# samuel-vitorino/sopro

Hardware: AMD Instinct MI355X
Metric: audio_seconds_per_second (higher is better)
Workload: dtype f32; 1 GPU; Sopro-135M synthesize, 32 utterances x 200 frames per GPU (BASELINE configs[1]), S=64 text tokens, 32 distinct 150-frame reference voice(s) per batch prepared outside the timed region, top_p=0.9 T=1.05 anti_loop (reference defaults), synthetic weights with EOS suppressed; batch_per_gpu=32, frames=200, voices_per_batch=32, parallelism=replicas x1 (utterance sharding, no collective), lanes_per_gpu=4

## Files before the change

include/sopro_hip.h:

```cpp
#ifndef SOPRO_HIP_H
#define SOPRO_HIP_H

#include <stdint.h>

#ifdef __cplusplus
extern "C" {
#endif

#define SOPRO_ABI_VERSION 42

const char* sopro_last_error(void);
int sopro_abi_version(void);
int sopro_build_flags(void);
int sopro_set_lds_floor(int bytes);
int sopro_set_host_wait(int blocking);
int sopro_device_info(int device, int* out4);

int sopro_capture_begin(void* stream);
int sopro_capture_end(void* stream, void** graph_exec_out);
int sopro_graph_launch(void* graph_exec, void* stream);
int sopro_graph_launch_n(void* graph_exec, void* stream, int32_t n);
int sopro_graph_destroy(void* graph_exec);
int sopro_stream_create_cu_range(int first_cu, int n_cus, void** stream_out);
int sopro_stream_create_cu_mask(const uint32_t* mask, int32_t words, void** stream_out);
int sopro_stream_destroy(void* stream);
int sopro_host_alloc(int64_t bytes, void** out);
int sopro_host_free(void* p);
int sopro_copy_to_host_async(void* dst_host, const void* src_dev, int64_t bytes, void* stream);

enum { SOPRO_PRO_NONE = 0, SOPRO_PRO_ELU = 1, SOPRO_PRO_ADDVEC = 2 };
enum { SOPRO_EPI_NONE = 0, SOPRO_EPI_GELU = 1, SOPRO_EPI_GLU = 2, SOPRO_EPI_RES = 3, SOPRO_EPI_TANH = 4,
       SOPRO_EPI_GLU_DW = 5 ,
       SOPRO_EPI_ROPE = 6  };

typedef struct sopro_gemm_args {
  const float* A; int64_t lda; int64_t a_seg_stride;
  const float* W; int64_t ldw;
  const float* bias;
  float* C; int64_t ldc; int64_t c_seg_stride;
  const float* R; int64_t ldr; int64_t r_seg_stride;
  const float* scale;
  const float* pro_vec;
  long long* dbg;
  int32_t M, N, K, rows_per_seg;
  int32_t prologue, epilogue;
} sopro_gemm_args;
int sopro_gemm_f32(const sopro_gemm_args* args, void* stream);
int sopro_gemm_set_tile_override(int cfg);

typedef struct sopro_gemm_split_ext {
  int32_t a_format;
  int32_t c_mode;
  float* C2; int64_t ldc2; int64_t c2_seg_stride;
  int32_t rms_norm; float rms_eps;
  int32_t ksplit;
  int32_t n_tickets;
  float* ws; int64_t ws_bytes;
  int32_t* tickets;
  int32_t group_m;
  float acc_scale;
  int32_t* range_events;
  const float* rope_cos; const float* rope_sin;
  int32_t rope_cols, rope_dh, rope_pos0, rope_rows_per_seg;
  const float* ln_stats;
  float* ln_stats_out;
} sopro_gemm_split_ext;
int sopro_gemm_bf16x3(const sopro_gemm_args* a, const void* packed_w, const sopro_gemm_split_ext* ext, void* stream);
int64_t sopro_packed_w_rows_bytes(int32_t N, int32_t K);
int sopro_pack_w_rows_bf16(const float* W, int64_t ldw, int32_t N, int32_t K, void* packed, void* stream);
int sopro_gemm_8p_takes(const sopro_gemm_args* a, const sopro_gemm_split_ext* ext);
int sopro_gemm_bf16x3_8p(const sopro_gemm_args* a, const void* w_rows, const sopro_gemm_split_ext* ext, void* stream);
int sopro_gemm_bf16x6(const sopro_gemm_args* a, const void* packed_w, const sopro_gemm_split_ext* ext, void* stream);
int sopro_gemm_bf16x1(const sopro_gemm_args* a, const void* packed_w, const sopro_gemm_split_ext* ext, void* stream);
int sopro_pack_w_bf16(const float* W, int64_t ldw, int32_t N, int32_t K, int32_t pieces, void* packed, void* stream);
int sopro_pack_w_f16x2(const float* W, int64_t ldw, int32_t N, int32_t K, float wscale, void* packed, void* stream);
float sopro_f16x3_a_scale(void);
int sopro_gemm_f16x3(const sopro_gemm_args* a, const void* packed_w, const sopro_gemm_split_ext* ext, void* stream);
int64_t sopro_packed_w_bytes(int32_t N, int32_t K, int32_t pieces);
int sopro_gemm_bf16_set_tile_override(int cfg);
int sopro_gemm_set_group_m(int g);

typedef struct sopro_skinny_args {
  const float* X; int64_t ldx;
  const float* W; int64_t ldw;
  const float* bias;
  float* Y; int64_t ldy;
  const float* R; int64_t ldr;
  const float* scale;
  float* ring;
  const float* dw_w;
  const float* dw_b;
  const int32_t* step;
  const float* Xp; int64_t xp_stride;
  int64_t y_part_stride;
  long long* dbg;
  float eps;
  int32_t B, N, K, epilogue;
  int32_t ring_len, ring_bcap, dil, ksize;
  int32_t np, ksplit, rms_norm;
  int32_t w_layout;
  const float* aux_W; const float* aux_bias; const float* aux_R; float* aux_Y;
  int64_t aux_ldy, aux_ldr, aux_y_part_stride;
  int32_t aux_tiles, aux_flags;
  int32_t ring_format;
  int32_t mt, nt;
} sopro_skinny_args;
int sopro_skinny_f32(const sopro_skinny_args* args, void* stream);
int sopro_pack_skinny_w(const float* W, int64_t ldw, int32_t N, int32_t K, int32_t glu, float* out, void* stream);
int64_t sopro_skinny_packed_floats(int32_t N, int32_t K, int32_t glu);
int sopro_pack_skinny_w_bf16(const float* W, int64_t ldw, int32_t N, int32_t K, int32_t glu, void* out, void* stream);

int sopro_fill2d_u32(void* p, int64_t pitch, int32_t rows, int32_t width, uint32_t value, void* stream);
int sopro_copy2d_u32(void* dst, int64_t dpitch, const void* src, int64_t spitch, int32_t rows, int32_t width, void* stream);
int sopro_nar_seed_i32(int32_t* tokens, int32_t Q, const int32_t* cb0, int64_t cb0_bstride, int32_t B, int32_t T, int32_t vmax, void* stream);
int sopro_cvt_f32_bf16(const float* src, void* dst, int64_t n, void* stream);
int sopro_cvt_bf16_f32(const void* src, float* dst, int64_t n, void* stream);
enum { SOPRO_NORM_RMS = 0, SOPRO_NORM_LN = 1 };
int sopro_norm_f32(const float* x, int64_t ldx, int64_t x_seg_stride , float* out, int64_t ldo, const float* w, const float* b,
                   const float* mul, const float* add, int32_t rows, int32_t rows_per_seg, int32_t C,
                   float eps, int32_t kind, void* stream);
int sopro_row_stats_f32(const float* x, int64_t ldx, int64_t x_seg_stride , int32_t rows, int32_t rows_per_seg, int32_t C,
                        float* stats, void* stream);
int sopro_rms_match_f32(const float* a, const float* x, float* out, int32_t rows, int32_t C, void* stream);
int sopro_tanh_affine_f32(const float* in, float* out, float c0, float c1, int64_t n, void* stream);
int sopro_add_pos_f32(const float* rowvec, const float* table, float* out, int32_t B, int32_t T, int32_t C,
                      int32_t pos0, void* stream);
int sopro_masked_mean_f32(const float* x, const int32_t* lens, float* out, int32_t B, int32_t T, int32_t C,
                          void* stream);

int sopro_stats_pool_f32(const float* h, const float* logit, const int32_t* lens, float* out, int32_t B, int32_t T,
                         int32_t C, void* stream);
int sopro_l2norm_f32(const float* x, float* out, int32_t rows, int32_t C, float eps, void* stream);

int sopro_dwconv_f32(const float* x, const float* w, const float* bias, const float* res, float* out,
                     const int32_t* lens, int32_t B, int32_t T, int32_t C, int32_t ksize, int32_t dil,
                     int32_t left, int32_t mode, void* stream);

int sopro_codebook_sum_f32(const int32_t* tok, int32_t ldt, const int32_t* col, const int32_t* off, const float* wq,
                           int32_t nq, const float* table, int64_t table_rows, const float* base, float alpha,
                           float beta, float* out, int64_t ldo, int64_t o_seg_stride, int32_t rows,
                           int32_t rows_per_seg, int32_t D, void* stream);
int sopro_text_embed_f32(const int32_t* ids, const int32_t* lens, const float* table, int64_t table_rows,
                         const float* pe, float* out, int32_t B, int32_t T, int32_t C, void* stream);
int sopro_argmax_rows_f32(const float* x, int64_t ldx, int32_t* out, int64_t ldo, int32_t inner, int32_t rows, int32_t N,
                          void* stream);
int sopro_argmax_partials_i32(const float* partials, int64_t ldp, int32_t* out, int64_t ldo, int32_t heads, int32_t per_head, int32_t V,
                              int32_t rows, void* stream);

int sopro_fir1_f32(const float* x, int64_t x_seg_stride, int32_t n_in, const float* w, const float* bias, float* out,
                   int64_t ldo, int64_t o_seg_stride, int32_t B, int32_t n_out, int32_t C, int32_t K, int32_t stride,
                   int32_t left, void* stream);
int sopro_rvq_assign_f32(const float* scores, int64_t lds, int32_t V, const float* table, float* res, int64_t ldr,
                         int32_t D, int32_t* codes, int64_t ldc, int32_t rows, void* stream);

typedef struct sopro_attn_args {
  const float* Q; int64_t ldq; int64_t q_bstride;
  const float* K; int64_t ldk; int64_t k_bstride;
  const float* V; int64_t ldv; int64_t v_bstride;
  float* O; int64_t ldo; int64_t o_bstride;
  const int32_t* klens;
// ... 106 lines not shown
} sopro_ar_block;
typedef struct sopro_ar_frame {
  sopro_ar_block blk[SOPRO_AR_MAX_LAYERS];
  const void* head_w; const float* head_b;
  float* x0;
  float* xa; float* xb;
  float* part;
  float* u;
  float* xp;
  float* qa;
  float* qpart;
  float* logits;
  const int32_t* klens;
  int32_t n_layers, B, D, S_cap, V1, H, ksize, w_layout;
  int32_t tile_glu, tile_ff1, tile_ff2, tile_head;
  float eps;
  int32_t k_unfold;
  int32_t store_format;
  sopro_ar_state st;
} sopro_ar_frame;
int sopro_ar_issue_frame(const sopro_ar_frame* frame, void* stream);

typedef struct sopro_engine sopro_engine;
typedef struct sopro_engine_cfg {
  int32_t d_model, codebook_size, num_codebooks, nar_head_dim, bos_row;
  int32_t n_layers_ar, ar_kernel, ar_dilations[16], ar_xattn[16] ;
  float ar_gate[16];
  int32_t n_layers_nar, nar_kernel, nar_dilations[16];
  int32_t n_stages, stage_first_cb[8], stage_n_cb[8];
  float nar_mix[8][2];
  float nar_prev_cb_weights[64];
  int32_t mimi_hidden, mimi_codebook_dim, mimi_heads, mimi_head_dim, mimi_layers, mimi_window, mimi_inter;
  int32_t mimi_n_ratios, mimi_ratios[8], mimi_num_filters, mimi_kernel, mimi_res_kernel, mimi_last_kernel, mimi_compress;
  int32_t mimi_n_semantic, mimi_rope_positions;
  float mimi_norm_eps, mimi_final_bias;
  int32_t precision;
  int32_t n_layers_text, ref_enc_layers, ref_xattn_layers, ref_xattn_heads, sv_student_dim, enc_kernel ;
} sopro_engine_cfg;
int sopro_engine_create(const sopro_engine_cfg* cfg, sopro_engine** out);
int sopro_engine_set_tensor(sopro_engine* e, const char* name, const void* dev_ptr, const int64_t* shape, int32_t ndim);
int sopro_engine_upload_tensor(sopro_engine* e, const char* name, const float* host_ptr, const int64_t* shape, int32_t ndim, void* stream);
int sopro_engine_finalize(sopro_engine* e, void* stream);
int sopro_ar_fold_text(const float* txt, const float* nkv_weight, const float* kv_w, const float* q_wT, const float* o_w, float* nkv, float* kvd,
                       float* kp, float* vp, int32_t B, int32_t S, int32_t S_cap, int32_t D, int32_t H, float eps, void* stream);
int sopro_ar_fold_text_uk(const float* txt, const float* nkv_weight, const float* kv_w, const float* o_w, float* nkv, float* kvd, float* kq, float* vp,
                          int32_t B, int32_t S, int32_t S_cap, int32_t D, int32_t H, float eps, void* stream);
int sopro_engine_destroy(sopro_engine* e);
int sopro_engine_set_ar_tiles(sopro_engine* e, int32_t glu, int32_t ff1, int32_t ff2, int32_t head);

typedef struct sopro_checkpoint sopro_checkpoint;
int sopro_checkpoint_open(const char* sopro_path, const char* mimi_path, sopro_checkpoint** out);
int sopro_checkpoint_close(sopro_checkpoint* ck);
int32_t sopro_checkpoint_count(const sopro_checkpoint* ck);
int sopro_checkpoint_tensor(const sopro_checkpoint* ck, int32_t i, const char** name, const float** data, int64_t* shape4, int32_t* ndim);
int sopro_checkpoint_engine_cfg(const sopro_checkpoint* ck, int32_t precision, sopro_engine_cfg* cfg);
int sopro_engine_from_checkpoint(const sopro_checkpoint* ck, int32_t precision, void* stream, sopro_engine** out);

int64_t sopro_cond_workspace_bytes(const sopro_engine* e, int32_t B, int32_t S, int32_t Tar);
int sopro_cond_prepare(sopro_engine* e, void* workspace, const int32_t* ids, const int32_t* lens, int32_t ragged, const float* film_mul, const float* film_add,
                       const float* const* ref_k, const float* const* ref_v, int64_t kv_bstride, const int32_t* kv_index, const int32_t* ref_klens,
                       int32_t B, int32_t S, int32_t Tar, int32_t Tr, float* txt_seq, float* txt_pool, float* cond_ar, void* stream);
int sopro_film_coeffs(sopro_engine* e, const float* sv, float style, int32_t n, float* scratch, float* mul, float* add, void* stream);
int64_t sopro_ref_workspace_bytes(const sopro_engine* e, int32_t T);
int sopro_ref_prepare(sopro_engine* e, void* workspace, const int32_t* tokens, int32_t T, float* sv, float* ref_seq, float* const* kv, void* stream);

int64_t sopro_ar_workspace_bytes(const sopro_engine* e, int32_t B, int32_t S, int32_t Tar);
int sopro_ar_begin(sopro_engine* e, void* workspace, int32_t B, const float* cond_ar, const float* txt_seq, const int32_t* text_lens,
                   int32_t S, int32_t Tar, const float params[8], uint64_t seed, uint32_t nonce, void* stream);
int sopro_ar_run_graph(sopro_engine* e, int32_t n_steps, void* stream);
int sopro_ar_tokens(sopro_engine* e, int32_t* hist, int32_t* first_eos, int32_t* n_stopped, void* stream);

int64_t sopro_nar_workspace_bytes(const sopro_engine* e, int32_t B, int32_t T);
int sopro_nar_refine(sopro_engine* e, void* workspace, const float* cond, int64_t cond_bstride, const int32_t* rvq1, const int32_t* lens,
                     int32_t B, int32_t T, int32_t* tokens, void* stream);
typedef struct sopro_nar_io {
  const float* cond; int64_t cond_bstride;
  const int32_t* cb0; int64_t cb0_bstride;
  const int32_t* lens;
  int32_t* tokens;
  int32_t* range_out;
  int32_t safe;
} sopro_nar_io;
int sopro_nar_refine_io(sopro_engine* e, void* workspace, const sopro_nar_io* io, int32_t B, int32_t T, void* stream);

int64_t sopro_mimi_encode_workspace_bytes(const sopro_engine* e, int32_t B, int32_t N);
int sopro_mimi_encode(sopro_engine* e, void* workspace, const float* wav, int32_t B, int32_t N, int32_t* codes, void* stream);

int64_t sopro_mimi_workspace_bytes(const sopro_engine* e, int32_t B, int32_t T);
int sopro_mimi_decode(sopro_engine* e, void* workspace, const int32_t* tokens, int32_t B, int32_t T, float* wav, void* stream);
int32_t sopro_mimi_chunk_rows(int32_t B, int32_t T);
int sopro_mimi_decode_parts(sopro_engine* e, void* workspace, const int32_t* tokens, int32_t B, int32_t T, float* wav, int32_t parts, void* stream);

typedef struct sopro_mimi_stream_state {
  float* kv;
  int32_t cap_rows;
  int32_t kv_len, pos, evict, half;
} sopro_mimi_stream_state;
int64_t sopro_mimi_stream_kv_bytes(const sopro_engine* e, int32_t cap_rows);
int sopro_mimi_stream_init(const sopro_engine* e, sopro_mimi_stream_state* st, void* kv, int32_t cap_rows);
int sopro_mimi_stream_trim(sopro_mimi_stream_state* st, int32_t n);
int sopro_mimi_decode_stream(sopro_engine* e, void* workspace, sopro_mimi_stream_state* st, const int32_t* tokens, int32_t T, float* wav,
                             void* stream);

#define SOPRO_MIMI_STREAM_BATCH_MAX_ROWS 64
typedef struct sopro_mimi_stream_batch {
  float* kv;
  int32_t rows_cap, rows;
  int32_t cap_rows, kv_len, pos, evict, half;
} sopro_mimi_stream_batch;
int64_t sopro_mimi_stream_batch_kv_bytes(const sopro_engine* e, int32_t rows, int32_t cap_rows);
int sopro_mimi_stream_batch_init(const sopro_engine* e, sopro_mimi_stream_batch* st, void* kv, int32_t rows, int32_t cap_rows);
int sopro_mimi_stream_batch_trim(sopro_mimi_stream_batch* st, int32_t n);
int sopro_mimi_stream_batch_keep(const sopro_engine* e, sopro_mimi_stream_batch* st, const int32_t* keep, int32_t n_keep, void* stream);
int sopro_mimi_decode_stream_batch(sopro_engine* e, void* workspace, sopro_mimi_stream_batch* st, const int32_t* tokens, int32_t T, float* wav,
                                   void* stream);

int64_t sopro_join_workspace_bytes(int32_t n_seg, int64_t max_len, int32_t hop);
int sopro_join_edges_f32(const float* wav, int64_t row_stride, const int32_t* lens, int32_t n_seg, int64_t max_len, int32_t hop, float rel,
                         int32_t keep, int32_t trim, void* workspace, int32_t* edges, void* stream);
int sopro_join_layout_i64(const int32_t* edges, const int32_t* gaps, int32_t n_seg, int64_t* offs, void* stream);
int sopro_join_mix_f32(const float* wav, int64_t row_stride, const int32_t* edges, const int64_t* offs, const float* tab, int32_t fade_len,
                       int32_t n_seg, float* out, int64_t out_cap, void* stream);

#define SOPRO_TSM_W 960
#define SOPRO_TSM_HS 480
#define SOPRO_TSM_R 240
#define SOPRO_TSM_TAIL 2048
int64_t sopro_tsm_out_len(int64_t in_len, int64_t step);
int64_t sopro_tsm_blocks(int64_t out_len);
int64_t sopro_tsm_chunk_out_cap(int64_t in_len);
int64_t sopro_tsm_state_bytes(int32_t rows);
int sopro_tsm_rows_f32(const float* in, int64_t in_stride, const int32_t* in_lens, int64_t in_cap, const int64_t* steps, int32_t rows, void* state,
                       int32_t flush, const float* tab, float* out, int64_t out_stride, int64_t out_cap, int32_t* out_lens, int32_t* deltas,
                       int32_t blocks_cap, void* stream);

#define SOPRO_PITCH_NT 64
#define SOPRO_PITCH_P 256
#define SOPRO_PITCH_TAIL 128
#define SOPRO_PITCH_TILE 2048
int64_t sopro_pitch_out_len(int64_t in_len, int64_t inc);
int64_t sopro_pitch_chunk_out_cap(int64_t in_len);
int64_t sopro_pitch_state_bytes(int32_t rows);
int sopro_pitch_rows_f32(const float* in, int64_t in_stride, const int32_t* in_lens, int64_t in_cap, const int64_t* incs, const int32_t* bank_idx,
                         const float* banks, int32_t n_banks, int32_t rows, void* state, int32_t flush, float* out, int64_t out_stride,
                         int64_t out_cap, int32_t* out_lens, void* stream);

#define SOPRO_WM_HS 480
#define SOPRO_WM_P 8192
#define SOPRO_WM_SHIFT 32
#define SOPRO_WM_TAIL 1536
#define SOPRO_WM_TILE 3840
int64_t sopro_wm_state_bytes(int32_t rows);
int64_t sopro_wm_chunk_out_cap(int64_t in_len);
int64_t sopro_wm_fold_ws_bytes(int32_t rows, int64_t in_cap);
int sopro_wm_embed_rows_f32(const float* in, int64_t in_stride, const int32_t* in_lens, int64_t in_cap, const int32_t* car_idx, const int8_t* cars,
                            int32_t n_cars, const float* alphas, int32_t rows, void* state, int32_t flush, const float* tab, float* out,
                            int64_t out_stride, int64_t out_cap, int32_t* out_lens, void* stream);
int sopro_wm_fold_rows_f32(const float* in, int64_t in_stride, const int32_t* in_lens, int64_t in_cap, int32_t rows, const float* tab, void* workspace,
                           float* f, void* stream);
int sopro_wm_corr_rows_f32(const float* f, const int8_t* dtab, int32_t n_keys, const int32_t* key_idx, int32_t rows, float* R, void* stream);
int sopro_wm_peak_rows_f32(const float* R, int32_t rows, int32_t* out, void* stream);

#define SOPRO_SIL_HOP 240
#define SOPRO_SIL_TAIL 4608
#define SOPRO_SIL_TILE 2048
#define SOPRO_SIL_PLAN_WORDS 64
// ... 20 lines not shown
```

sopro_amd/csrc/common.h:

```cpp
#pragma once
#ifdef SOPRO_DEV_SWITCHES
#define SOPRO_DEV_ENV(name) getenv(name)
#else
#define SOPRO_DEV_ENV(name) (static_cast<const char*>(nullptr))
#endif
#include <hip/hip_runtime.h>
#include <stdint.h>
#include <stdio.h>
#include <string.h>

#include "../../include/sopro_hip.h"

typedef float f32x4 __attribute__((ext_vector_type(4)));
typedef float f32x16 __attribute__((ext_vector_type(16)));

void sopro_set_error(const char* fmt, ...);
extern int g_sopro_lds_floor;

#define SOPRO_CHECK_ARG(cond, msg)                                  \
  do {                                                              \
    if (!(cond)) {                                                  \
      sopro_set_error("%s: bad argument: %s", __func__, msg);       \
      return -2;                                                    \
    }                                                               \
  } while (0)

#define SOPRO_HIP(call)                                                                   \
  do {                                                                                    \
    hipError_t e_ = (call);                                                               \
    if (e_ != hipSuccess) {                                                               \
      sopro_set_error("%s: %s failed: %s", __func__, #call, hipGetErrorString(e_));       \
      return -1;                                                                          \
    }                                                                                     \
  } while (0)

#define SOPRO_LAUNCH_CHECK()                                                              \
  do {                                                                                    \
    hipError_t e_ = hipGetLastError();                                                    \
    if (e_ != hipSuccess) {                                                               \
      sopro_set_error("%s: kernel launch failed: %s", __func__, hipGetErrorString(e_));   \
      return -1;                                                                          \
    }                                                                                     \
    return 0;                                                                             \
  } while (0)

static inline bool aligned16(const void* p) { return (reinterpret_cast<uintptr_t>(p) & 15u) == 0; }

#define SOPRO_SET_MAX_LDS_ONCE(kern, bytes)                                                                              \
  do {                                                                                                                   \
    static unsigned char done_[64] = {};                                                                                 \
    int dev_ = 0;                                                                                                        \
    SOPRO_HIP(hipGetDevice(&dev_));                                                                                      \
    if (!done_[dev_ & 63]) {                                                                                             \
      SOPRO_HIP(hipFuncSetAttribute(reinterpret_cast<const void*>(kern), hipFuncAttributeMaxDynamicSharedMemorySize, (int)(bytes))); \
      done_[dev_ & 63] = 1;                                                                                              \
    }                                                                                                                    \
  } while (0)

__device__ __forceinline__ float gelu_erf(float v) { return v * 0.5f * (1.0f + erff(v * 0.70710678118654752440f)); }
__device__ __forceinline__ float gelu_fast(float v) {
  const float x = fabsf(v) * 0.70710678118654752440f;
  const float t = __builtin_amdgcn_rcpf(fmaf(0.3275911f, x, 1.0f));
  float p = fmaf(1.061405429f, t, -1.453152027f);
  p = fmaf(p, t, 1.421413741f);
  p = fmaf(p, t, -0.284496736f);
  p = fmaf(p, t, 0.254829592f);
  p *= t;
  const float e = __builtin_amdgcn_exp2f(x * x * -1.44269504088896340736f);
  const float y = fmaf(-p, e, 1.0f);
  const float h = 0.5f * v;
  return fmaf(h, copysignf(y, v), h);
}
__device__ __forceinline__ float sigmoidf_(float v) { return 1.0f / (1.0f + expf(-v)); }
__device__ __forceinline__ float sigmoid_fast(float v) { return __builtin_amdgcn_rcpf(1.0f + __builtin_amdgcn_exp2f(-1.44269504088896340736f * v)); }
__device__ __forceinline__ float eluf_(float v) { return __builtin_amdgcn_fmed3f(v, __expf(v) - 1.0f, 0.0f); }

typedef __bf16 bf16x2_t __attribute__((ext_vector_type(2)));
typedef float f32x2_t __attribute__((ext_vector_type(2)));
__device__ __forceinline__ void split2_bf16(float x, float y, unsigned& hi, unsigned& lo) {
  const f32x2_t v = {x, y};
  const bf16x2_t h = __builtin_convertvector(v, bf16x2_t);
  hi = *reinterpret_cast<const unsigned*>(&h);
  const f32x2_t r = {x - __uint_as_float(hi << 16), y - __uint_as_float(hi & 0xffff0000u)};
  const bf16x2_t l = __builtin_convertvector(r, bf16x2_t);
  lo = *reinterpret_cast<const unsigned*>(&l);
}

#ifndef SOPRO_NT_BULK
#define SOPRO_NT_BULK 1
#endif
__device__ __forceinline__ bool bulk_nt(bool big) { return SOPRO_NT_BULK == 1 || (SOPRO_NT_BULK == 2 && big); }
typedef unsigned u32x4_t __attribute__((ext_vector_type(4)));
typedef unsigned u32x2_t __attribute__((ext_vector_type(2)));
__device__ __forceinline__ void bulk_store4(float* p, const float4& v, bool big) {
  if (bulk_nt(big)) __builtin_nontemporal_store((f32x4){v.x, v.y, v.z, v.w}, reinterpret_cast<f32x4*>(p));
  else *reinterpret_cast<float4*>(p) = v;
}
__device__ __forceinline__ void bulk_store1(float* p, float v, bool big) {
  if (bulk_nt(big)) __builtin_nontemporal_store(v, p);
  else *p = v;
}
__device__ __forceinline__ void bulk_store_u2(void* p, const uint2& v, bool big) {
  if (bulk_nt(big)) __builtin_nontemporal_store((u32x2_t){v.x, v.y}, reinterpret_cast<u32x2_t*>(p));
  else *reinterpret_cast<uint2*>(p) = v;
}
__device__ __forceinline__ void bulk_store_u1(void* p, unsigned v, bool big) {
  if (bulk_nt(big)) __builtin_nontemporal_store(v, reinterpret_cast<unsigned*>(p));
  else *reinterpret_cast<unsigned*>(p) = v;
}
__device__ __forceinline__ uint4 bulk_load16(const void* p, bool big) {
  if (bulk_nt(big)) {
    const u32x4_t v = __builtin_nontemporal_load(reinterpret_cast<const u32x4_t*>(p));
    return make_uint4(v.x, v.y, v.z, v.w);
  }
  return *reinterpret_cast<const uint4*>(p);
}
constexpr int64_t SOPRO_BIG_BYTES = (int64_t)64 << 20;

__device__ __forceinline__ int xcd_contiguous(int b, int n) {
  const int per = n >> 3, rem = n & 7;
  const int x = b & 7, i = b >> 3;
  return x * per + min(x, rem) + i;
}

__device__ __forceinline__ float wave_sum(float v) {
#pragma unroll
  for (int o = 32; o > 0; o >>= 1) v += __shfl_xor(v, o, 64);
  return v;
}
__device__ __forceinline__ float wave_max(float v) {
#pragma unroll
  for (int o = 32; o > 0; o >>= 1) v = fmaxf(v, __shfl_xor(v, o, 64));
  return v;
}

struct sopro_prof_scope {
  void* rec;
  hipStream_t s;
  sopro_prof_scope(const char* family, double flops, hipStream_t s);
  ~sopro_prof_scope();
  sopro_prof_scope(const sopro_prof_scope&) = delete;
  sopro_prof_scope& operator=(const sopro_prof_scope&) = delete;
};
```

sopro_amd/csrc/elementwise.hip:

```cpp
#include "common.h"

namespace {

constexpr int NORM_MAX_PER_LANE = 16;

__global__ __launch_bounds__(256) void norm_kernel(const float* __restrict__ x, int64_t ldx, int64_t x_seg_stride, float* __restrict__ out,
                                                   int64_t ldo, const float* __restrict__ w, const float* __restrict__ b,
                                                   const float* __restrict__ mul, const float* __restrict__ add, int rows,
                                                   int rows_per_seg, int C, float eps, int kind) {
  const int lane = threadIdx.x & 63;
  const int row = blockIdx.x * 4 + (threadIdx.x >> 6);
  if (row >= rows) return;
  const int seg = row / rows_per_seg;
  const float* xr = x + (int64_t)seg * x_seg_stride + (int64_t)(row - seg * rows_per_seg) * ldx;
  float v[NORM_MAX_PER_LANE];
  const int per = (C + 63) / 64;
  float s = 0.f;
#pragma unroll
  for (int j = 0; j < NORM_MAX_PER_LANE; ++j) {
    const int c = lane + j * 64;
    v[j] = (j < per && c < C) ? xr[c] : 0.f;
    s += v[j];
  }
  float mean = 0.f, var;
// ... 364 lines not shown
      v.x = eluf_(v.x); v.y = eluf_(v.y); v.z = eluf_(v.z); v.w = eluf_(v.w);
      s0 = v.x * w0.x + v.y * w0.y + v.z * w0.z + v.w * w0.w;
      s1 = v.x * w1.x + v.y * w1.y + v.z * w1.z + v.w * w1.w;
      s2 = v.x * w2.x + v.y * w2.y + v.z * w2.z + v.w * w2.w;
    }
#pragma unroll
    for (int o = 8; o > 0; o >>= 1) {
      s0 += __shfl_xor(s0, o, 64);
      s1 += __shfl_xor(s1, o, 64);
      s2 += __shfl_xor(s2, o, 64);
    }
    if (sub == 0) { d[0][rr] = s0; d[1][rr] = s1; d[2][rr] = s2; }
  }
  __syncthreads();
  const int n = n0 + threadIdx.x;
  if (n < T) wav[(int64_t)b * wav_seg_stride + n] = ((d[0][threadIdx.x] + d[1][threadIdx.x + 1]) + d[2][threadIdx.x + 2]) + bias;
}

__global__ __launch_bounds__(256) void stats_pool_kernel(const float* __restrict__ h, const float* __restrict__ logit,
                                                         const int* __restrict__ lens, float* __restrict__ out, int B, int T,
                                                         int C) {
  __shared__ float red[4];
  __shared__ float sh_max, sh_sum;
  const int b = blockIdx.x, tid = threadIdx.x, lane = tid & 63, wave = tid >> 6;
  const int len = lens ? min(lens[b], T) : T;
  const float* lg = logit + (int64_t)b * T;
  float m = -INFINITY;
  for (int t = tid; t < len; t += 256) m = fmaxf(m, lg[t]);
  m = wave_max(m);
  if (lane == 0) red[wave] = m;
  __syncthreads();
  if (tid == 0) sh_max = fmaxf(fmaxf(red[0], red[1]), fmaxf(red[2], red[3]));
  __syncthreads();
  const float mx = sh_max;
  float s = 0.f;
  for (int t = tid; t < len; t += 256) s += expf(lg[t] - mx);
  s = wave_sum(s);
  __syncthreads();
  if (lane == 0) red[wave] = s;
  __syncthreads();
  if (tid == 0) sh_sum = (red[0] + red[1]) + (red[2] + red[3]);
  __syncthreads();
  const float inv = 1.f / sh_sum;
  for (int c = tid; c < C; c += 256) {
    float mu = 0.f;
    for (int t = 0; t < len; ++t) mu += (expf(lg[t] - mx) * inv) * h[((int64_t)b * T + t) * C + c];
    float var = 0.f;
    for (int t = 0; t < len; ++t) {
      const float d = h[((int64_t)b * T + t) * C + c] - mu;
      var += (expf(lg[t] - mx) * inv) * d * d;
    }
    out[(int64_t)b * 2 * C + c] = mu;
    out[(int64_t)b * 2 * C + C + c] = sqrtf(fmaxf(var, 1e-6f));
  }
}

__global__ __launch_bounds__(256) void l2norm_kernel(const float* __restrict__ x, float* __restrict__ out, int rows, int C,
                                                     float eps) {
  const int lane = threadIdx.x & 63;
  const int row = blockIdx.x * 4 + (threadIdx.x >> 6);
  if (row >= rows) return;
  float s = 0.f;
  for (int c = lane; c < C; c += 64) s += x[(int64_t)row * C + c] * x[(int64_t)row * C + c];
  s = wave_sum(s);
  const float d = fmaxf(sqrtf(s), eps);
  for (int c = lane; c < C; c += 64) out[(int64_t)row * C + c] = x[(int64_t)row * C + c] / d;
}

inline unsigned nblk(int64_t n, int bs) { return (unsigned)((n + bs - 1) / bs); }


__global__ __launch_bounds__(256) void fill2d_kernel(unsigned* __restrict__ p, int64_t pitch, int rows, int width, unsigned v) {
  const int64_t i = (int64_t)blockIdx.x * blockDim.x + threadIdx.x;
  if (i >= (int64_t)rows * width) return;
  p[(i / width) * pitch + (i % width)] = v;
}
__global__ __launch_bounds__(256) void copy2d_kernel(unsigned* __restrict__ d, int64_t dpitch, const unsigned* __restrict__ s, int64_t spitch, int rows,
                                                     int width) {
  const int64_t i = (int64_t)blockIdx.x * blockDim.x + threadIdx.x;
  if (i >= (int64_t)rows * width) return;
  d[(i / width) * dpitch + (i % width)] = s[(i / width) * spitch + (i % width)];
}

__global__ __launch_bounds__(256) void nar_seed_kernel(int* __restrict__ tokens, int Q, const int* __restrict__ cb0, int64_t bstride, int B, int T, int vmax) {
  const int64_t i = (int64_t)blockIdx.x * blockDim.x + threadIdx.x;
  if (i >= (int64_t)B * T) return;
  const int b = (int)(i / T), t = (int)(i - (int64_t)b * T);
  tokens[i * Q] = min(max(cb0[(int64_t)b * bstride + t], 0), vmax);
}

__global__ __launch_bounds__(256) void cvt_f32_bf16_kernel(const float* __restrict__ src, uint2* __restrict__ dst, int64_t n4) {
  const int64_t i = (int64_t)blockIdx.x * blockDim.x + threadIdx.x;
  if (i >= n4) return;
  const float4 v = reinterpret_cast<const float4*>(src)[i];
  unsigned a, b, lo;
  split2_bf16(v.x, v.y, a, lo);
  split2_bf16(v.z, v.w, b, lo);
  dst[i] = make_uint2(a, b);
}
__global__ __launch_bounds__(256) void cvt_bf16_f32_kernel(const uint2* __restrict__ src, float* __restrict__ dst, int64_t n4) {
  const int64_t i = (int64_t)blockIdx.x * blockDim.x + threadIdx.x;
  if (i >= n4) return;
  const uint2 v = src[i];
  reinterpret_cast<float4*>(dst)[i] = make_float4(__uint_as_float(v.x << 16), __uint_as_float(v.x & 0xffff0000u), __uint_as_float(v.y << 16),
                                                  __uint_as_float(v.y & 0xffff0000u));
}

__global__ __launch_bounds__(256) void row_stats_kernel(const float* __restrict__ x, int64_t ldx, int64_t seg_stride, int rows, int rps, int C,
                                                        float* __restrict__ stats) {
  const int per_row = C >> 2;
  const int64_t i = (int64_t)blockIdx.x * blockDim.x + threadIdx.x;
  const int64_t r = i / per_row;
  if (r >= rows) return;
  const int c4 = (int)(i - r * per_row);
  const int64_t seg = r / rps, rr = r - seg * rps;
  const float4 v = *reinterpret_cast<const float4*>(x + seg * seg_stride + rr * ldx + c4 * 4);
  float s = (v.x + v.y) + (v.z + v.w);
  s += __shfl_xor(s, 1, 64); s += __shfl_xor(s, 2, 64); s += __shfl_xor(s, 4, 64); s += __shfl_xor(s, 8, 64);
  const float mu = s * (1.0f / 64.0f);
  const float dx = v.x - mu, dy = v.y - mu, dz = v.z - mu, dw = v.w - mu;
  float q = (dx * dx + dy * dy) + (dz * dz + dw * dw);
  q += __shfl_xor(q, 1, 64); q += __shfl_xor(q, 2, 64); q += __shfl_xor(q, 4, 64); q += __shfl_xor(q, 8, 64);
  if ((c4 & 15) == 0) *reinterpret_cast<float2*>(stats + (r * (C >> 6) + (c4 >> 4)) * 2) = make_float2(mu, q);
}

}

extern "C" {

int sopro_row_stats_f32(const float* x, int64_t ldx, int64_t x_seg_stride, int32_t rows, int32_t rows_per_seg, int32_t C, float* stats, void* stream) {
  SOPRO_CHECK_ARG(x && stats && rows > 0 && rows_per_seg > 0 && C > 0 && (C & 63) == 0, "x, stats non-NULL; rows > 0; C a multiple of 64");
  SOPRO_CHECK_ARG(aligned16(x) && (ldx & 3) == 0 && (x_seg_stride & 3) == 0 && (reinterpret_cast<uintptr_t>(stats) & 7u) == 0, "16-byte aligned rows, 8-byte aligned stats");
  hipLaunchKernelGGL(row_stats_kernel, dim3(nblk((int64_t)rows * (C >> 2), 256)), dim3(256), 0, (hipStream_t)stream, x, ldx,
                     x_seg_stride ? x_seg_stride : (int64_t)rows_per_seg * ldx, rows, rows_per_seg, C, stats);
  SOPRO_LAUNCH_CHECK();
}

int sopro_norm_f32(const float* x, int64_t ldx, int64_t x_seg_stride, float* out, int64_t ldo, const float* w, const float* b,
                   const float* mul, const float* add, int32_t rows, int32_t rows_per_seg, int32_t C, float eps,
                   int32_t kind, void* stream) {
  SOPRO_CHECK_ARG(x && out && w, "x, out, w must be non-NULL");
  SOPRO_CHECK_ARG(rows > 0 && C > 0 && C <= 64 * NORM_MAX_PER_LANE && rows_per_seg > 0, "rows > 0, 0 < C <= 1024");
  SOPRO_CHECK_ARG(kind == SOPRO_NORM_RMS || kind == SOPRO_NORM_LN, "unknown norm kind");
  hipLaunchKernelGGL(norm_kernel, dim3(nblk(rows, 4)), dim3(256), 0, (hipStream_t)stream, x, ldx,
                     x_seg_stride ? x_seg_stride : (int64_t)rows_per_seg * ldx, out, ldo, w, b, mul, add, rows, rows_per_seg, C, eps, kind);
  SOPRO_LAUNCH_CHECK();
}

int sopro_rms_match_f32(const float* a, const float* x, float* out, int32_t rows, int32_t C, void* stream) {
  SOPRO_CHECK_ARG(a && x && out && rows > 0 && C > 0, "bad pointers or sizes");
  hipLaunchKernelGGL(rms_match_kernel, dim3(nblk(rows, 4)), dim3(256), 0, (hipStream_t)stream, a, x, out, rows, C);
  SOPRO_LAUNCH_CHECK();
}

int sopro_tanh_affine_f32(const float* in, float* out, float c0, float c1, int64_t n, void* stream) {
  SOPRO_CHECK_ARG(in && out && n > 0, "bad pointers or sizes");
  hipLaunchKernelGGL(tanh_affine_kernel, dim3(nblk(n, 256)), dim3(256), 0, (hipStream_t)stream, in, out, c0, c1, n);
  SOPRO_LAUNCH_CHECK();
}

int sopro_add_pos_f32(const float* rowvec, const float* table, float* out, int32_t B, int32_t T, int32_t C, int32_t pos0,
                      void* stream) {
  SOPRO_CHECK_ARG(rowvec && table && out && B > 0 && T > 0 && C > 0 && pos0 >= 0, "bad pointers or sizes");
  hipLaunchKernelGGL(add_pos_kernel, dim3(nblk((int64_t)B * T * C, 256)), dim3(256), 0, (hipStream_t)stream, rowvec, table,
                     out, B, T, C, pos0);
  SOPRO_LAUNCH_CHECK();
// ... 41 lines not shown

int sopro_text_embed_f32(const int32_t* ids, const int32_t* lens, const float* table, int64_t table_rows, const float* pe,
                         float* out, int32_t B, int32_t T, int32_t C, void* stream) {
  SOPRO_CHECK_ARG(ids && table && pe && out && B > 0 && T > 0 && C > 0 && (C & 3) == 0, "bad pointers or sizes");
  hipLaunchKernelGGL(text_embed_kernel, dim3(nblk((int64_t)B * T * (C / 4), 256)), dim3(256), 0, (hipStream_t)stream, ids, lens,
                     table, table_rows, pe, out, B, T, C);
  SOPRO_LAUNCH_CHECK();
}

int sopro_argmax_rows_f32(const float* x, int64_t ldx, int32_t* out, int64_t ldo, int32_t inner, int32_t rows, int32_t N,
                          void* stream) {
  SOPRO_CHECK_ARG(x && out && rows > 0 && N > 0 && inner > 0, "bad pointers or sizes");
  hipLaunchKernelGGL(argmax_rows_kernel, dim3(nblk(rows, 4)), dim3(256), 0, (hipStream_t)stream, x, ldx, out, ldo, inner, rows, N);
  SOPRO_LAUNCH_CHECK();
}

int sopro_fir1_f32(const float* x, int64_t x_seg_stride, int32_t n_in, const float* w, const float* bias, float* out, int64_t ldo,
                   int64_t o_seg_stride, int32_t B, int32_t n_out, int32_t C, int32_t K, int32_t stride, int32_t left, void* stream) {
  SOPRO_CHECK_ARG(x && w && out, "NULL pointer");
  SOPRO_CHECK_ARG(B > 0 && B <= 65535 && n_in > 0 && n_out > 0 && C > 0 && K > 0 && stride > 0 && left >= 0 && ldo >= C, "bad sizes");
  hipLaunchKernelGGL(fir1_kernel, dim3(nblk((int64_t)n_out * C, 256), B), dim3(256), 0, (hipStream_t)stream, x, x_seg_stride, n_in, w,
                     bias, out, ldo, o_seg_stride, n_out, C, K, stride, left);
  SOPRO_LAUNCH_CHECK();
}

int sopro_argmax_partials_i32(const float* partials, int64_t ldp, int32_t* out, int64_t ldo, int32_t heads, int32_t per_head, int32_t V,
                              int32_t rows, void* stream) {
  SOPRO_CHECK_ARG(partials && out && rows > 0 && heads > 0 && per_head > 0 && V > 0 && ldp >= (int64_t)heads * per_head && ldo >= heads,
                  "bad pointers or sizes");
  SOPRO_CHECK_ARG((reinterpret_cast<uintptr_t>(partials) & 7u) == 0, "partials must be 8-byte aligned");
  const int64_t total = (int64_t)rows * heads;
  hipLaunchKernelGGL(argmax_partials_kernel, dim3(nblk(total * 8, 256)), dim3(256), 0, (hipStream_t)stream, partials, ldp, out, ldo, heads,
                     per_head, V, total);
  SOPRO_LAUNCH_CHECK();
}

int sopro_rvq_assign_f32(const float* scores, int64_t lds, int32_t V, const float* table, float* res, int64_t ldr, int32_t D,
                         int32_t* codes, int64_t ldc, int32_t rows, void* stream) {
  SOPRO_CHECK_ARG(scores && table && res && codes, "NULL pointer");
  SOPRO_CHECK_ARG(rows > 0 && V > 0 && D > 0 && lds >= V && ldr >= D && ldc > 0, "bad sizes");
  hipLaunchKernelGGL(rvq_assign_kernel, dim3(rows), dim3(256), 0, (hipStream_t)stream, scores, lds, V, table, res, ldr, D, codes, ldc);
  SOPRO_LAUNCH_CHECK();
}

int sopro_rope_f32(float* x, int64_t ldx, const float* cos_t, const float* sin_t, int32_t rows, int32_t rows_per_seg,
                   int32_t pos0, int32_t H, int32_t dh, void* stream) {
  SOPRO_CHECK_ARG(x && cos_t && sin_t && rows > 0 && rows_per_seg > 0 && H > 0 && dh > 0 && (dh & 1) == 0 && pos0 >= 0,
                  "bad pointers or sizes");
  hipLaunchKernelGGL(rope_kernel, dim3(nblk((int64_t)rows * H * (dh / 2), 256)), dim3(256), 0, (hipStream_t)stream, x, ldx, cos_t,
                     sin_t, rows, rows_per_seg, pos0, H, dh);
  SOPRO_LAUNCH_CHECK();
}

int sopro_upsample2_f32(const float* x, const float* w, float* y, int64_t y_seg_stride, int32_t B, int32_t T, int32_t C,
                        void* stream) {
  SOPRO_CHECK_ARG(x && w && y && B > 0 && T > 0 && C > 0, "bad pointers or sizes");
  hipLaunchKernelGGL(upsample2_kernel, dim3(nblk((int64_t)B * T * 2 * C, 256)), dim3(256), 0, (hipStream_t)stream, x, w, y,
                     y_seg_stride, B, T, C);
  SOPRO_LAUNCH_CHECK();
}

int sopro_final_conv_f32(const float* h, int64_t h_seg_stride, const float* w, float bias, float* wav,
                         int64_t wav_seg_stride, int32_t B, int32_t T, void* stream) {
  SOPRO_CHECK_ARG(h && w && wav && B > 0 && T > 0, "bad pointers or sizes");
  SOPRO_CHECK_ARG(aligned16(h) && aligned16(w) && (h_seg_stride & 3) == 0, "alignment");
  hipLaunchKernelGGL(final_conv_kernel, dim3(nblk(T, 256), B), dim3(256), 0, (hipStream_t)stream, h, h_seg_stride, w, bias, wav,
                     wav_seg_stride, B, T);
  SOPRO_LAUNCH_CHECK();
}

int sopro_stats_pool_f32(const float* h, const float* logit, const int32_t* lens, float* out, int32_t B, int32_t T, int32_t C,
                         void* stream) {
  SOPRO_CHECK_ARG(h && logit && out && B > 0 && T > 0 && C > 0, "bad pointers or sizes");
  hipLaunchKernelGGL(stats_pool_kernel, dim3(B), dim3(256), 0, (hipStream_t)stream, h, logit, lens, out, B, T, C);
  SOPRO_LAUNCH_CHECK();
}

int sopro_l2norm_f32(const float* x, float* out, int32_t rows, int32_t C, float eps, void* stream) {
  SOPRO_CHECK_ARG(x && out && rows > 0 && C > 0, "bad pointers or sizes");
  hipLaunchKernelGGL(l2norm_kernel, dim3(nblk(rows, 4)), dim3(256), 0, (hipStream_t)stream, x, out, rows, C, eps);
  SOPRO_LAUNCH_CHECK();
}

int sopro_fill2d_u32(void* p, int64_t pitch, int32_t rows, int32_t width, uint32_t value, void* stream) {
  SOPRO_CHECK_ARG(p && rows > 0 && width > 0 && pitch >= width, "bad pointers or sizes");
  hipLaunchKernelGGL(fill2d_kernel, dim3(nblk((int64_t)rows * width, 256)), dim3(256), 0, (hipStream_t)stream, reinterpret_cast<unsigned*>(p), pitch, rows,
                     width, value);
  SOPRO_LAUNCH_CHECK();
}

int sopro_copy2d_u32(void* dst, int64_t dpitch, const void* src, int64_t spitch, int32_t rows, int32_t width, void* stream) {
  SOPRO_CHECK_ARG(dst && src && rows > 0 && width > 0 && dpitch >= width && spitch >= width, "bad pointers or sizes");
  hipLaunchKernelGGL(copy2d_kernel, dim3(nblk((int64_t)rows * width, 256)), dim3(256), 0, (hipStream_t)stream, reinterpret_cast<unsigned*>(dst), dpitch,
                     reinterpret_cast<const unsigned*>(src), spitch, rows, width);
  SOPRO_LAUNCH_CHECK();
}

int sopro_nar_seed_i32(int32_t* tokens, int32_t Q, const int32_t* cb0, int64_t cb0_bstride, int32_t B, int32_t T, int32_t vmax, void* stream) {
  SOPRO_CHECK_ARG(tokens && cb0 && Q > 0 && B > 0 && T > 0 && cb0_bstride >= T && vmax >= 0, "bad pointers or sizes");
  hipLaunchKernelGGL(nar_seed_kernel, dim3(nblk((int64_t)B * T, 256)), dim3(256), 0, (hipStream_t)stream, tokens, Q, cb0, cb0_bstride, B, T, vmax);
  SOPRO_LAUNCH_CHECK();
}

int sopro_cvt_f32_bf16(const float* src, void* dst, int64_t n, void* stream) {
  SOPRO_CHECK_ARG(src && dst && n > 0 && (n & 3) == 0 && aligned16(src) && (reinterpret_cast<uintptr_t>(dst) & 7u) == 0, "n % 4 == 0, 16 / 8-byte aligned");
  hipLaunchKernelGGL(cvt_f32_bf16_kernel, dim3(nblk(n / 4, 256)), dim3(256), 0, (hipStream_t)stream, src, reinterpret_cast<uint2*>(dst), n / 4);
  SOPRO_LAUNCH_CHECK();
}

int sopro_cvt_bf16_f32(const void* src, float* dst, int64_t n, void* stream) {
  SOPRO_CHECK_ARG(src && dst && n > 0 && (n & 3) == 0 && aligned16(dst) && (reinterpret_cast<uintptr_t>(src) & 7u) == 0, "n % 4 == 0, 16 / 8-byte aligned");
  hipLaunchKernelGGL(cvt_bf16_f32_kernel, dim3(nblk(n / 4, 256)), dim3(256), 0, (hipStream_t)stream, reinterpret_cast<const uint2*>(src), dst, n / 4);
  SOPRO_LAUNCH_CHECK();
}

}

namespace {

__global__ __launch_bounds__(256) void stream_batch_append_kernel(float4* __restrict__ cur, float4* __restrict__ other, const float4* __restrict__ qkv,
                                                                  int hs4, int64_t bstride4, int n, int kv_len, int keep_from) {
  const int j = blockIdx.x, b = blockIdx.y;
  const int row4 = 2 * hs4;
  const float4* src;
  float4* dst;
  if (j < n) {
    src = qkv + ((int64_t)b * n + j) * 3 * hs4 + hs4;
    dst = cur + (int64_t)b * bstride4 + (int64_t)(kv_len + j) * row4;
  } else {
    const int i = j - n, p = keep_from + i;
    src = p < kv_len ? cur + (int64_t)b * bstride4 + (int64_t)p * row4 : qkv + ((int64_t)b * n + (p - kv_len)) * 3 * hs4 + hs4;
    dst = other + (int64_t)b * bstride4 + (int64_t)i * row4;
  }
  for (int c = threadIdx.x; c < row4; c += blockDim.x) dst[c] = src[c];
}

struct KeepMap {
  int32_t src[64];
};

__global__ __launch_bounds__(256) void stream_batch_gather_kernel(float4* __restrict__ kv, const KeepMap km, int row4, int64_t bstride4, int64_t half4,
                                                                  int half) {
  const int p = blockIdx.x, i = blockIdx.y, l = blockIdx.z;
  const float4* src = kv + (int64_t)(2 * l + half) * half4 + (int64_t)km.src[i] * bstride4 + (int64_t)p * row4;
  float4* dst = kv + (int64_t)(2 * l + (half ^ 1)) * half4 + (int64_t)i * bstride4 + (int64_t)p * row4;
  for (int c = threadIdx.x; c < row4; c += blockDim.x) dst[c] = src[c];
}

}

int sopro_stream_batch_append(float* cur, float* other, const float* qkv, int32_t hs, int32_t rows, int64_t bstride, int32_t n, int32_t kv_len,
                              int32_t nkeep, hipStream_t s) {
  SOPRO_CHECK_ARG(cur && other && qkv && hs > 0 && (hs & 3) == 0 && rows > 0 && n > 0 && kv_len >= 0 && nkeep >= 0 && nkeep <= kv_len + n &&
                      (int64_t)(kv_len + n) * 2 * hs <= bstride && (int64_t)nkeep * 2 * hs <= bstride && (bstride & 3) == 0,
                  "bad sizes");
  SOPRO_CHECK_ARG(aligned16(cur) && aligned16(other) && aligned16(qkv), "16-byte aligned rows");
  hipLaunchKernelGGL(stream_batch_append_kernel, dim3(n + nkeep, rows), dim3(256), 0, s, reinterpret_cast<float4*>(cur),
                     reinterpret_cast<float4*>(other), reinterpret_cast<const float4*>(qkv), hs / 4, bstride / 4, n, kv_len, kv_len + n - nkeep);
  SOPRO_LAUNCH_CHECK();
}

int sopro_stream_batch_gather(float* kv, const int32_t* keep, int32_t n_keep, int32_t layers, int32_t rows_cap, int64_t bstride, int32_t hs, int32_t half,
                              int32_t kv_len, hipStream_t s) {
  SOPRO_CHECK_ARG(kv && keep && n_keep > 0 && n_keep <= 64 && n_keep <= rows_cap && layers > 0 && hs > 0 && (hs & 3) == 0 && kv_len > 0 &&
                      (int64_t)kv_len * 2 * hs <= bstride && (bstride & 3) == 0 && (half == 0 || half == 1),
                  "bad sizes");
// ... 9 lines not shown
```

sopro_amd/csrc/gemm_bf16s.hip:

```cpp
#include "common.h"
#include "gemm_epilogue.h"

namespace {

constexpr int BK = 32;


typedef __bf16 bf16x8 __attribute__((ext_vector_type(8)));
typedef _Float16 f16x8 __attribute__((ext_vector_type(8)));
typedef _Float16 f16x2_t __attribute__((ext_vector_type(2)));

__device__ __forceinline__ bf16x8 as_frag(const uint4& v) { return *reinterpret_cast<const bf16x8*>(&v); }
__device__ __forceinline__ f16x8 as_frag16(const uint4& v) { return *reinterpret_cast<const f16x8*>(&v); }

constexpr float A16_SCALE = 8.0f;

template <int NPL, bool F16 = false>
__device__ __forceinline__ void split_pair(float x, float y, unsigned (&pc)[NPL]) {
#pragma unroll
  for (int p = 0; p < NPL; ++p) {
    const f32x2_t v = {x, y};
    if constexpr (F16) {
      const f16x2_t h = __builtin_convertvector(v, f16x2_t);
      pc[p] = *reinterpret_cast<const unsigned*>(&h);
      x -= (float)h[0];
      y -= (float)h[1];
    } else {
      const bf16x2_t h = __builtin_convertvector(v, bf16x2_t);
      pc[p] = *reinterpret_cast<const unsigned*>(&h);
      x -= __uint_as_float(pc[p] << 16);
      y -= __uint_as_float(pc[p] & 0xffff0000u);
    }
  }
}

template <int NPL, int WM, int WN, int TM, int TN, int EPI, int AMODE, int OUT, bool SK, bool F16 = false>
__global__ __launch_bounds__(WM* WN * 64) void gemm_bf16s_kernel(const sopro_gemm_args g, const uint4* __restrict__ Wp,
                                                                 int ksubs, const sopro_gemm_split_ext ext) {
  constexpr int AROW = NPL * 64 + 16;
  constexpr bool FOLD = F16;
  constexpr int NT = WM * WN * 64;
  constexpr int BM = WM * TM * 32;
  constexpr int BN = WN * TN * 32;
  constexpr int A_F4 = BM * 8 / NT;
  constexpr int RSTEP = NT / 8;
  extern __shared__ float4 smem4[];
  unsigned char* As = reinterpret_cast<unsigned char*>(smem4);

  const int tid = threadIdx.x, lane = tid & 63, wave = tid >> 6;
  const int wm = wave / WN, wn = wave % WN;
  const int ntn = (g.N + BN - 1) / BN;
  const int bid = xcd_contiguous((int)blockIdx.x, (int)gridDim.x);
  int mt = bid / ntn, nt = bid % ntn;
  if (ext.group_m > 1) {
    const int ntm_all = (g.M + BM - 1) / BM;
    const int per = ext.group_m * ntn;
    const int grp = bid / per, rem = bid - grp * per;
    const int first = grp * ext.group_m;
    const int gsz = min(ntm_all - first, ext.group_m);
    mt = first + rem % gsz;
    nt = rem / gsz;
  }
  const int m0 = mt * BM, n0 = nt * BN;
  const int lrow = tid >> 3, lc4 = tid & 7;
  const int rps = g.rows_per_seg;
  long long* dbg = g.dbg ? g.dbg + (int64_t)blockIdx.x * 8 : nullptr;
  if (dbg && tid == 0) dbg[0] = clock64();

  static_assert(AMODE != 5 || NPL == 1, "bf16 rows are a one-pass (bf16 mode) operand form");
  constexpr int AES = AMODE == 5 ? 2 : 4;
  const char* ap[A_F4];
#pragma unroll
  for (int i = 0; i < A_F4; ++i) {
    const int m = min(m0 + lrow + i * RSTEP, g.M - 1);
    const int seg = m / rps;
    const int r = m - seg * rps;
    ap[i] = reinterpret_cast<const char*>(g.A) + ((int64_t)seg * g.a_seg_stride + (int64_t)r * g.lda) * AES;
  }
  const int ntiles = (g.N + 31) >> 5;
  const uint4* bp[TN];
#pragma unroll
  for (int j = 0; j < TN; ++j) {
    const int t = min((n0 >> 5) + wn * TN + j, ntiles - 1);
    bp[j] = Wp + ((int64_t)t * ksubs * NPL) * 64 + lane;
  }
  int boff[TN];
#pragma unroll
  for (int j = 0; j < TN; ++j) {
    const int t = min((n0 >> 5) + wn * TN + j, ntiles - 1);
    boff[j] = (t * ksubs * NPL) * 64 + lane;
  }
  float biasv[TN];
#pragma unroll
  for (int j = 0; j < TN; ++j) {
    const int n = n0 + (wn * TN + j) * 32 + (lane & 31);
    biasv[j] = (g.bias && n < g.N) ? g.bias[n] : 0.f;
  }

  float4 raA[A_F4], raB[A_F4];
  float ssq[A_F4];
  float rsc[A_F4];
  float a16max = 0.f;
#pragma unroll
  for (int i = 0; i < A_F4; ++i) { ssq[i] = 0.f; rsc[i] = A16_SCALE; }
  float sapin[A_F4];
#pragma unroll
  for (int i = 0; i < A_F4; ++i) sapin[i] = A16_SCALE;
  float lmu[A_F4], lrs[A_F4];
  float4 pvA = make_float4(0.f, 0.f, 0.f, 0.f), pvB = pvA;
  const int KT = (g.K + BK - 1) / BK;
  const int klast = g.K - 4;

  auto gload = [&](int kt, float4 (&ra)[A_F4], float4& pv) {
    const int k = min(kt * BK + lc4 * 4, klast);
    if constexpr (AMODE == 5) {
#pragma unroll
      for (int i = 0; i < A_F4; ++i) {
        const uint2 v = *reinterpret_cast<const uint2*>(ap[i] + (int64_t)k * 2);
        ra[i].x = __uint_as_float(v.x);
        ra[i].y = __uint_as_float(v.y);
      }
    } else {
#pragma unroll
      for (int i = 0; i < A_F4; ++i) ra[i] = *reinterpret_cast<const float4*>(ap[i] + (int64_t)k * 4);
    }
    if (AMODE == 3) pv = *reinterpret_cast<const float4*>(g.pro_vec + k);
  };
  auto bload = [&](int kt, uint4 (&rb)[TN][2][NPL]) {
#pragma unroll
    for (int j = 0; j < TN; ++j)
#pragma unroll
      for (int s = 0; s < 2; ++s)
#pragma unroll
        for (int p = 0; p < NPL; ++p) rb[j][s][p] = bp[j][((int64_t)(kt * 2 + s) * NPL + p) * 64];
  };
  auto lstore_piece = [&](int buf, float4 (&ra)[A_F4], const float4& pv, int i, bool fresh, bool first) {
    if constexpr (FOLD) {
      if constexpr (AMODE == 4) asm volatile("" : "+v"(rsc[i]), "+v"(ssq[i]));
      else asm volatile("" : "+v"(sapin[i]));
    }
    if constexpr (AMODE == 5) {
      unsigned char* a = As + buf * BM * AROW + lrow * AROW + lc4 * 8;
      *reinterpret_cast<uint2*>(a + i * RSTEP * AROW) = make_uint2(__float_as_uint(ra[i].x), __float_as_uint(ra[i].y));
    } else if constexpr (AMODE == 2) {
      unsigned char* a = As + buf * BM * AROW + lrow * AROW + lc4 * 16;
      *reinterpret_cast<f32x4*>(a + i * RSTEP * AROW) = (f32x4){ra[i].x, ra[i].y, ra[i].z, ra[i].w};
    } else {
      if constexpr (AMODE == 1) {
        ra[i].x = eluf_(ra[i].x); ra[i].y = eluf_(ra[i].y); ra[i].z = eluf_(ra[i].z); ra[i].w = eluf_(ra[i].w);
      } else if constexpr (AMODE == 3) {
        ra[i].x += pv.x; ra[i].y += pv.y; ra[i].z += pv.z; ra[i].w += pv.w;
      } else if constexpr (AMODE == 6) {
        const f32x2_t r2 = {lrs[i], lrs[i]}, n2 = {lmu[i], lmu[i]};
        const f32x2_t lo2 = (f32x2_t){ra[i].x, ra[i].y} * r2 + n2, hi2 = (f32x2_t){ra[i].z, ra[i].w} * r2 + n2;
        ra[i].x = lo2[0]; ra[i].y = lo2[1]; ra[i].z = hi2[0]; ra[i].w = hi2[1];
      }
      if constexpr (AMODE == 4) {
        if (fresh) ssq[i] = fmaf(ra[i].x, ra[i].x, fmaf(ra[i].y, ra[i].y, fmaf(ra[i].z, ra[i].z, fmaf(ra[i].w, ra[i].w, ssq[i]))));
      }
      unsigned char* a = As + buf * BM * AROW + lrow * AROW + lc4 * 8;
      {
        unsigned c0[NPL], c1[NPL];
        if constexpr (F16) {
          const float F16MAX = 65504.0f;
          if constexpr (AMODE == 4) {
            if (first) {
              float mx = fmaxf(fmaxf(fabsf(ra[i].x), fabsf(ra[i].y)), fmaxf(fabsf(ra[i].z), fabsf(ra[i].w)));
              mx = fmaxf(mx, __shfl_xor(mx, 1, 64));
              mx = fmaxf(mx, __shfl_xor(mx, 2, 64));
              mx = fmaxf(mx, __shfl_xor(mx, 4, 64));
              const int ex = (int)((__float_as_uint(mx) >> 23) & 255u);
              rsc[i] = (ex == 0 || ex == 255) ? A16_SCALE : __uint_as_float((unsigned)min(max(261 - ex, 2), 252) << 23);
            }
          }
          const float sa = AMODE == 4 ? rsc[i] : sapin[i];
          const float vx = ra[i].x * sa, vy = ra[i].y * sa, vz = ra[i].z * sa, vw = ra[i].w * sa;
          a16max = fmaxf(a16max, fmaxf(fmaxf(fabsf(vx), fabsf(vy)), fmaxf(fabsf(vz), fabsf(vw))));
          split_pair<NPL, true>(__builtin_amdgcn_fmed3f(vx, -F16MAX, F16MAX), __builtin_amdgcn_fmed3f(vy, -F16MAX, F16MAX), c0);
          split_pair<NPL, true>(__builtin_amdgcn_fmed3f(vz, -F16MAX, F16MAX), __builtin_amdgcn_fmed3f(vw, -F16MAX, F16MAX), c1);
        } else {
          split_pair<NPL>(ra[i].x, ra[i].y, c0);
          split_pair<NPL>(ra[i].z, ra[i].w, c1);
        }
#pragma unroll
        for (int p = 0; p < NPL; ++p) *reinterpret_cast<uint2*>(a + i * RSTEP * AROW + p * 64) = make_uint2(c0[p], c1[p]);
      }
    }
  };
  auto lstore = [&](int buf, float4 (&ra)[A_F4], const float4& pv, bool fresh = true, bool first = false) {
#pragma unroll
    for (int i = 0; i < A_F4; ++i) lstore_piece(buf, ra, pv, i, fresh, first);
  };

  f32x16 acc[TM][TN];
#pragma unroll
  for (int i = 0; i < TM; ++i)
#pragma unroll
    for (int j = 0; j < TN; ++j)
#pragma unroll
      for (int r = 0; r < 16; ++r) acc[i][j][r] = 0.f;

  const int frow = lane & 31, fg = lane >> 5;
  constexpr int NPAIR = NPL == 1 ? 1 : (NPL == 2 ? 3 : 6);
  constexpr int PA[6] = {NPL == 1 ? 0 : (NPL == 2 ? 1 : 2), 0, NPL == 2 ? 0 : 1, 1, 0, 0};
  constexpr int PB[6] = {0, NPL == 2 ? 1 : 2, NPL == 2 ? 0 : 1, 0, 1, 0};
  auto compute = [&](int buf, const uint4 (&rb)[TN][2][NPL]) {
    const unsigned char* a = As + buf * BM * AROW + (wm * TM * 32 + frow) * AROW + fg * 16;
#pragma unroll
    for (int s = 0; s < 2; ++s) {
      uint4 af[TM][NPL];
#pragma unroll
      for (int i = 0; i < TM; ++i)
#pragma unroll
        for (int p = 0; p < NPL; ++p) af[i][p] = *reinterpret_cast<const uint4*>(a + i * 32 * AROW + p * 64 + s * 32);
#pragma unroll
      for (int q = 0; q < NPAIR; ++q)
#pragma unroll
        for (int i = 0; i < TM; ++i)
#pragma unroll
          for (int j = 0; j < TN; ++j)
            if constexpr (F16)
// ... 172 lines not shown
                acc[i][j][r] += v[u][0]; acc[i][j][r + 1] += v[u][1]; acc[i][j][r + 2] += v[u][2]; acc[i][j][r + 3] += v[u][3];
              }
            }
          }
    }
  }
  float cscale = 1.0f;
  if constexpr (F16) {
    cscale = AMODE == 4 ? ext.acc_scale * A16_SCALE : ext.acc_scale;
    if (ext.range_events && !(a16max <= 65504.0f)) atomicAdd(ext.range_events, 1);
  }
  const float* rs = nullptr;
  if constexpr (AMODE == 4) {
    float* rsl = reinterpret_cast<float*>(smem4) + BM * (BN + 4);
#pragma unroll
    for (int i = 0; i < A_F4; ++i) {
      float v = ssq[i];
      v += __shfl_xor(v, 1, 64);
      v += __shfl_xor(v, 2, 64);
      v += __shfl_xor(v, 4, 64);
      float r = rsqrtf(v / (float)g.K + ext.rms_eps);
      if constexpr (F16) r *= __uint_as_float(0x7f000000u - __float_as_uint(rsc[i])) * cscale;
      if (lc4 == 0) rsl[lrow + i * RSTEP] = r;
    }
    __syncthreads();
    rs = rsl;
  }
  gemm_store_tile<WM, WN, TM, TN, EPI, OUT>(g, reinterpret_cast<float*>(smem4), acc, biasv, m0, n0, &ext, rs, cscale);
  if (dbg && tid == 0) dbg[3] = clock64();
}

template <int NPL, bool F16 = false>
__global__ __launch_bounds__(256) void pack_w_kernel(const float* __restrict__ W, int64_t ldw, int N, int K, uint4* __restrict__ out,
                                                     int ksubs, int64_t total, float wscale = 1.0f) {
  const int64_t i = (int64_t)blockIdx.x * blockDim.x + threadIdx.x;
  if (i >= total) return;
  const int lane = (int)(i & 63);
  const int64_t pk = i >> 6;
  const int p = (int)(pk % NPL);
  const int64_t tk = pk / NPL;
  const int ks = (int)(tk % ksubs);
  const int t = (int)(tk / ksubs);
  const int n = t * 32 + (lane & 31);
  const int k0 = ks * 16 + (lane >> 5) * 8;
  unsigned w[4];
#pragma unroll
  for (int e = 0; e < 4; ++e) {
    const int k = k0 + 2 * e;
    const float x = (n < N && k < K) ? W[(int64_t)n * ldw + k] : 0.f;
    const float y = (n < N && k + 1 < K) ? W[(int64_t)n * ldw + k + 1] : 0.f;
    unsigned pc[NPL];
    if constexpr (F16) split_pair<NPL, true>(x * wscale, y * wscale, pc);
    else split_pair<NPL>(x, y, pc);
    w[e] = pc[p];
  }
  out[i] = make_uint4(w[0], w[1], w[2], w[3]);
}

template <int NPL, int WM, int WN, int TM, int TN, int EPI, int AMODE, int OUT, bool F16 = false>
int launch_one(const sopro_gemm_args& g, const uint4* wp, int ksubs, const sopro_gemm_split_ext& ext, hipStream_t s) {
  constexpr int BM = WM * TM * 32, BN = WN * TN * 32;
  constexpr size_t lds_main = (size_t)2 * BM * (NPL * 64 + 16), lds_epi = (size_t)BM * (BN + 4 + (AMODE == 4 ? 1 : 0)) * sizeof(float);
  constexpr size_t lds = lds_main > lds_epi ? lds_main : lds_epi;
  const int ks = ext.ksplit > 1 ? ext.ksplit : 1;
  auto kern = ks > 1 ? gemm_bf16s_kernel<NPL, WM, WN, TM, TN, EPI, AMODE, OUT, true, F16> : gemm_bf16s_kernel<NPL, WM, WN, TM, TN, EPI, AMODE, OUT, false, F16>;
  constexpr size_t lds_cap = lds > (size_t)96 * 1024 ? lds : (size_t)96 * 1024;
  if (ks > 1) SOPRO_SET_MAX_LDS_ONCE(kern, lds_cap);
  else SOPRO_SET_MAX_LDS_ONCE(kern, lds_cap);
  const size_t lds_req = lds > (size_t)g_sopro_lds_floor ? lds : (size_t)g_sopro_lds_floor;
  const int ntm = (g.M + BM - 1) / BM, ntn = (g.N + BN - 1) / BN;
  if (ks > 1) {
    const int64_t need = (int64_t)ks * ntm * ntn * BM * BN * (int64_t)sizeof(float);
    if (!ext.ws || !ext.tickets || ext.ws_bytes < need || ext.n_tickets < ntm * ntn) {
      sopro_set_error("split-K needs a %lld-byte workspace and %d tickets (got %lld, %d)", (long long)need, ntm * ntn,
                      (long long)ext.ws_bytes, ext.n_tickets);
      return -2;
    }
  }
  hipLaunchKernelGGL(kern, dim3(ntm * ntn, ks), dim3(WM * WN * 64), lds_req, s, g, wp, ksubs, ext);
  SOPRO_LAUNCH_CHECK();
}

inline int amode_of(const sopro_gemm_args& g, const sopro_gemm_split_ext& ext) {
  if (ext.a_format == 1) return 2;
  if (ext.a_format == 2) return 5;
  if (ext.rms_norm) return 4;
  if (ext.ln_stats) return 6;
  return g.prologue == SOPRO_PRO_ELU ? 1 : (g.prologue == SOPRO_PRO_ADDVEC ? 3 : 0);
}

template <int NPL, int WM, int WN, int TM, int TN>
int launch_cfg3(const sopro_gemm_args& g, const uint4* wp, int ksubs, const sopro_gemm_split_ext& ext, hipStream_t s) {
  const int key = g.epilogue * 100 + amode_of(g, ext) * 10 + ext.c_mode;
#define SOPRO_CASE(E, A, O) \
  case (E) * 100 + (A) * 10 + (O): return launch_one<NPL, WM, WN, TM, TN, ((E) == SOPRO_EPI_GELU ? SOPRO_EPI_GELU_FAST : (E)), A, O>(g, wp, ksubs, ext, s)
  switch (key) {
    SOPRO_CASE(SOPRO_EPI_NONE, 0, 0);
    SOPRO_CASE(SOPRO_EPI_GELU, 0, 0);
    SOPRO_CASE(SOPRO_EPI_RES, 0, 0);
    SOPRO_CASE(SOPRO_EPI_ROPE, 0, 0);
    SOPRO_CASE(SOPRO_EPI_NONE, 6, 0);
    SOPRO_CASE(SOPRO_EPI_GELU, 6, 0);
    SOPRO_CASE(SOPRO_EPI_ROPE, 6, 0);
    SOPRO_CASE(SOPRO_EPI_NONE, 1, 0);
    SOPRO_CASE(SOPRO_EPI_RES, 1, 0);
    SOPRO_CASE(SOPRO_EPI_NONE, 0, 3);
    SOPRO_CASE(SOPRO_EPI_NONE, 0, 4);
    SOPRO_CASE(SOPRO_EPI_RES, 0, 3);
    default: break;
  }
  if constexpr (NPL == 1) {
    switch (key) {
      SOPRO_CASE(SOPRO_EPI_NONE, 0, 7);
      SOPRO_CASE(SOPRO_EPI_NONE, 5, 8);
      SOPRO_CASE(SOPRO_EPI_NONE, 5, 7);
      SOPRO_CASE(SOPRO_EPI_RES, 5, 7);
      SOPRO_CASE(SOPRO_EPI_NONE, 5, 6);
      SOPRO_CASE(SOPRO_EPI_NONE, 5, 0);
      default: break;
    }
  }
  if constexpr (NPL == 2) {
    switch (key) {
      SOPRO_CASE(SOPRO_EPI_NONE, 0, 1);
      SOPRO_CASE(SOPRO_EPI_NONE, 0, 2);
      SOPRO_CASE(SOPRO_EPI_NONE, 2, 0);
      SOPRO_CASE(SOPRO_EPI_NONE, 2, 1);
      SOPRO_CASE(SOPRO_EPI_NONE, 2, 2);
      SOPRO_CASE(SOPRO_EPI_NONE, 2, 4);
      SOPRO_CASE(SOPRO_EPI_RES, 2, 1);
      default: break;
    }
  }
#undef SOPRO_CASE
  sopro_set_error("sopro_gemm_bf16x%d: (epilogue %d, prologue %d, a_format %d, c_mode %d) is not an available combination",
                  NPL == 2 ? 3 : NPL, g.epilogue, g.prologue, ext.a_format, ext.c_mode);
  return -2;
}

template <int NPL, int WM, int WN, int TM, int TN, bool F16 = false>
int launch_cfg6(const sopro_gemm_args& g, const uint4* wp, int ksubs, const sopro_gemm_split_ext& ext, hipStream_t s) {
  const int key = g.epilogue * 10 + amode_of(g, ext);
#define SOPRO_CASE(E, A) \
  case (E) * 10 + (A): return launch_one<NPL, WM, WN, TM, TN, (((E) == SOPRO_EPI_GELU && (F16 || NPL != 3)) ? SOPRO_EPI_GELU_FAST : (E)), A, 0, F16>(g, wp, ksubs, ext, s)
  switch (key) {
    SOPRO_CASE(SOPRO_EPI_NONE, 0);
    SOPRO_CASE(SOPRO_EPI_GELU, 0);
    SOPRO_CASE(SOPRO_EPI_RES, 0);
    SOPRO_CASE(SOPRO_EPI_NONE, 3);
    SOPRO_CASE(SOPRO_EPI_GELU, 4);
    SOPRO_CASE(SOPRO_EPI_NONE, 4);
    default: break;
  }
#undef SOPRO_CASE
  if constexpr (WN * TN * 32 >= 64) {
    constexpr int GLU_ = (F16 || NPL != 3) ? SOPRO_EPI_GLU_FAST : SOPRO_EPI_GLU;
    if (key == SOPRO_EPI_GLU * 10) return launch_one<NPL, WM, WN, TM, TN, GLU_, 0, 0, F16>(g, wp, ksubs, ext, s);
    if (key == SOPRO_EPI_GLU * 10 + 4) return launch_one<NPL, WM, WN, TM, TN, GLU_, 4, 0, F16>(g, wp, ksubs, ext, s);
  }
  sopro_set_error("sopro_gemm_%s: (epilogue %d, prologue %d) is not an available combination", F16 ? "f16x3" : (NPL == 3 ? "bf16x6" : "bf16x1"), g.epilogue, g.prologue);
  return -2;
}

template <int NPL, bool F16 = false>
int launch_argmax(sopro_gemm_args& g, const uint4* wp, int ksubs, const sopro_gemm_split_ext& ext, hipStream_t s) {
  SOPRO_CHECK_ARG(g.epilogue == SOPRO_EPI_NONE && g.prologue == SOPRO_PRO_NONE && !ext.rms_norm && ext.a_format == 0,
                  "arg-max output takes a plain contraction (no prologue / epilogue / fused norm)");
  SOPRO_CHECK_ARG(ext.C2 && ext.ldc2 >= (g.N + 63) / 64, "arg-max output: C2 = [M][ldc2 >= ceil(N / 64)] (value, index) pairs");
  static const bool tm1 = SOPRO_DEV_ENV("SOPRO_ARGMAX_TM") != nullptr && SOPRO_DEV_ENV("SOPRO_ARGMAX_TM")[0] == '1';
  static const bool tn1 = SOPRO_DEV_ENV("SOPRO_ARGMAX_TN") != nullptr && SOPRO_DEV_ENV("SOPRO_ARGMAX_TN")[0] == '1';
  if (g.M >= 8192 && g.N >= 2048 && (g.N & 127) == 0 && !tm1 && !tn1) return launch_one<NPL, 2, 2, 2, 2, SOPRO_EPI_NONE, 0, 5, F16>(g, wp, ksubs, ext, s);
  if (g.M >= 8192 && !tm1) return launch_one<NPL, 2, 2, 2, 1, SOPRO_EPI_NONE, 0, 5, F16>(g, wp, ksubs, ext, s);
  return launch_one<NPL, 2, 2, 1, 1, SOPRO_EPI_NONE, 0, 5, F16>(g, wp, ksubs, ext, s);
}

int check_rope(const sopro_gemm_args& g, const sopro_gemm_split_ext& ext) {
  if (g.epilogue != SOPRO_EPI_ROPE) return 0;
  const int dh = ext.rope_dh;
  SOPRO_CHECK_ARG(ext.rope_cos && ext.rope_sin && aligned16(ext.rope_cos) && aligned16(ext.rope_sin), "EPI_ROPE needs 16-byte aligned cos / sin tables");
  SOPRO_CHECK_ARG(dh >= 8 && dh <= 64 && (dh & (dh - 1)) == 0, "EPI_ROPE: rope_dh must be a power of two in 8..64 (heads must not straddle a 64-column tile)");
  SOPRO_CHECK_ARG(ext.rope_cols > 0 && ext.rope_cols <= g.N && ext.rope_cols % dh == 0, "EPI_ROPE: rope_cols must be whole heads within N");
  SOPRO_CHECK_ARG(ext.rope_rows_per_seg > 0 && ext.rope_pos0 >= 0, "EPI_ROPE: rope_rows_per_seg > 0, rope_pos0 >= 0");
  SOPRO_CHECK_ARG(ext.c_mode == 0 && ext.a_format == 0 && g.prologue == SOPRO_PRO_NONE && !ext.rms_norm, "EPI_ROPE is a plain fp32-rows form");
  SOPRO_CHECK_ARG((g.N & 3) == 0 && (g.ldc & 3) == 0 && (g.c_seg_stride & 3) == 0 && aligned16(g.C), "EPI_ROPE: 16-byte aligned output rows");
  return 0;
}

int check_ln(const sopro_gemm_args& g, const sopro_gemm_split_ext& ext) {
  if (ext.ln_stats) {
    SOPRO_CHECK_ARG((g.K & 63) == 0 && (reinterpret_cast<uintptr_t>(ext.ln_stats) & 7u) == 0, "fused LayerNorm: K % 64 == 0, 8-byte aligned ln_stats");
    SOPRO_CHECK_ARG(ext.a_format == 0 && g.prologue == SOPRO_PRO_NONE && !ext.rms_norm && ext.c_mode == 0, "fused LayerNorm takes plain fp32 rows (no prologue, c_mode 0)");
    SOPRO_CHECK_ARG(g.epilogue == SOPRO_EPI_NONE || g.epilogue == SOPRO_EPI_GELU || g.epilogue == SOPRO_EPI_ROPE, "fused LayerNorm: epilogue NONE, GELU or ROPE");
    SOPRO_CHECK_ARG(ext.rms_eps > 0.f, "fused LayerNorm: rms_eps carries the norm's eps (> 0)");
  }
  if (ext.ln_stats_out) {
    SOPRO_CHECK_ARG(g.epilogue == SOPRO_EPI_RES && ext.c_mode == 0 && (g.N & 63) == 0 && (reinterpret_cast<uintptr_t>(ext.ln_stats_out) & 7u) == 0,
                    "ln_stats_out: an EPI_RES contraction with fp32 output rows, N % 64 == 0, 8-byte aligned pairs");
    SOPRO_CHECK_ARG((g.ldc & 3) == 0 && (g.c_seg_stride & 3) == 0 && aligned16(g.C) && (g.ldr & 3) == 0 && (g.r_seg_stride & 3) == 0 && aligned16(g.R),
                    "ln_stats_out: 16-byte aligned output / residual rows");
  }
  return 0;
}

int check_common(sopro_gemm_args& g, sopro_gemm_split_ext& ext, const void* packed_w) {
  if (g.a_seg_stride == 0) g.a_seg_stride = (int64_t)g.rows_per_seg * g.lda;
  if (g.c_seg_stride == 0) g.c_seg_stride = (int64_t)g.rows_per_seg * g.ldc;
  if (g.r_seg_stride == 0) g.r_seg_stride = (int64_t)g.rows_per_seg * g.ldr;
  if (ext.c2_seg_stride == 0) ext.c2_seg_stride = (int64_t)g.rows_per_seg * ext.ldc2;
  SOPRO_CHECK_ARG(g.M > 0 && g.N > 0 && g.K > 0, "M, N, K must be positive");
  SOPRO_CHECK_ARG((g.K & 3) == 0, "K must be a multiple of 4");
  SOPRO_CHECK_ARG(g.rows_per_seg > 0, "rows_per_seg must be positive");
  SOPRO_CHECK_ARG(g.A && packed_w && (g.C || ext.c_mode == 5), "A, packed_w, C must be non-NULL");
  SOPRO_CHECK_ARG(aligned16(g.A) && aligned16(packed_w), "A and packed_w must be 16-byte aligned");
  SOPRO_CHECK_ARG((g.lda & 3) == 0 && (g.a_seg_stride & 3) == 0, "lda, a_seg_stride must be multiples of 4");
  SOPRO_CHECK_ARG(g.epilogue != SOPRO_EPI_RES || g.R != nullptr, "EPI_RES needs R");
  SOPRO_CHECK_ARG(g.prologue != SOPRO_PRO_ADDVEC || (g.pro_vec && aligned16(g.pro_vec)), "PRO_ADDVEC needs an aligned pro_vec");
  SOPRO_CHECK_ARG(g.epilogue != SOPRO_EPI_GLU || (g.N % 64) == 0, "EPI_GLU needs N % 64 == 0 (packed value/gate blocks)");
  SOPRO_CHECK_ARG(ext.ksplit >= 0 && ext.ksplit <= 64, "ksplit must be in 0..64");
  SOPRO_CHECK_ARG(ext.ksplit <= 1 || g.dbg == nullptr, "the clock-stamp probe is for unsplit launches");
  return 0;
}

}

static int g_group_m = 0;
extern "C" int sopro_gemm_set_group_m(int g) {
  g_group_m = g > 1 ? g : 0;
  return 0;
}

static bool eight_waves(const sopro_gemm_args& g) {
  static const bool on = SOPRO_DEV_ENV("SOPRO_GEMM_W8") != nullptr && SOPRO_DEV_ENV("SOPRO_GEMM_W8")[0] == '1';
  return on && g.N >= 512 && g.M >= 1024;
}

#ifdef SOPRO_DEV_SWITCHES
bool sopro_gemm_astat_takes(const sopro_gemm_args& g, const sopro_gemm_split_ext& ext);
int sopro_gemm_astat_bf16x3(const sopro_gemm_args& g, const void* packed_w, hipStream_t s);
#endif

static int g_tile_override = 0;
extern "C" int sopro_gemm_bf16_set_tile_override(int cfg) {
  g_tile_override = cfg;
  return 0;
}

extern "C" int64_t sopro_packed_w_bytes(int32_t N, int32_t K, int32_t pieces) {
  if (N <= 0 || K <= 0 || pieces < 1 || pieces > 3) return 0;
  return (int64_t)((N + 31) / 32) * ((K + 31) / 32 * 2) * pieces * 64 * 16;
}

extern "C" int sopro_pack_w_bf16(const float* W, int64_t ldw, int32_t N, int32_t K, int32_t pieces, void* packed, void* stream) {
  SOPRO_CHECK_ARG(W && packed && N > 0 && K > 0 && ldw >= K, "bad pointers or sizes");
// ... 90 lines not shown
  if (ext.c_mode == 5) return launch_argmax<1>(g, reinterpret_cast<const uint4*>(packed_w), (g.K + 31) / 32 * 2, ext, reinterpret_cast<hipStream_t>(stream));
  if (ext.c_mode >= 6) {
    SOPRO_CHECK_ARG((g.N & 3) == 0 && g.C && (reinterpret_cast<uintptr_t>(g.C) & 7u) == 0 && (g.ldc & 3) == 0 && (g.c_seg_stride & 3) == 0 && g.ldc >= g.N,
                    "bf16 output rows must be 8-byte aligned (N, ld, seg stride multiples of 4)");
    SOPRO_CHECK_ARG(ext.c_mode != 8 || (ext.C2 && (reinterpret_cast<uintptr_t>(ext.C2) & 7u) == 0 && (ext.ldc2 & 3) == 0 && (ext.c2_seg_stride & 3) == 0 && ext.ldc2 >= g.N),
                    "c_mode 8: C2 (the activated bf16 copy) must be given, 8-byte aligned rows");
    SOPRO_CHECK_ARG(g.epilogue != SOPRO_EPI_RES || ((reinterpret_cast<uintptr_t>(g.R) & 7u) == 0 && (g.ldr & 3) == 0 && (g.r_seg_stride & 3) == 0),
                    "bf16 skip operand rows must be 8-byte aligned");
  } else if (ext.c_mode != 0) {
    const bool second = ext.c_mode == 4;
    float* d = second ? ext.C2 : g.C;
    const int64_t ldd = second ? ext.ldc2 : g.ldc, dseg = second ? ext.c2_seg_stride : g.c_seg_stride;
    SOPRO_CHECK_ARG((g.N & 3) == 0 && d && aligned16(d) && (ldd & 3) == 0 && (dseg & 3) == 0 && ldd >= g.N,
                    "activated output rows must be 16-byte aligned (N, ld, seg stride multiples of 4)");
  }
  hipStream_t s = reinterpret_cast<hipStream_t>(stream);
  const uint4* wp = reinterpret_cast<const uint4*>(packed_w);
  const int ksubs = (g.K + 31) / 32 * 2;
  const int64_t t128 = (int64_t)((g.M + 127) / 128) * ((g.N + 127) / 128);
  const bool small = g.N <= 64 || g.M <= 64 || t128 < 256;
  const bool nar_like = ext.rms_norm || g.epilogue == SOPRO_EPI_GLU || g.prologue == SOPRO_PRO_ADDVEC;
  if (nar_like) {
    SOPRO_CHECK_ARG(ext.c_mode == 0 && (g.prologue == SOPRO_PRO_NONE || g.prologue == SOPRO_PRO_ADDVEC), "GLU / RMSNorm / ADDVEC forms write plain fp32");
    if (g.epilogue == SOPRO_EPI_GLU) return small ? launch_cfg6<1, 2, 2, 1, 2>(g, wp, ksubs, ext, s) : launch_cfg6<1, 2, 2, 2, 2>(g, wp, ksubs, ext, s);
    return small ? launch_cfg6<1, 2, 2, 1, 1>(g, wp, ksubs, ext, s) : launch_cfg6<1, 2, 2, 2, 2>(g, wp, ksubs, ext, s);
  }
  SOPRO_CHECK_ARG(g.prologue == SOPRO_PRO_NONE || g.prologue == SOPRO_PRO_ELU, "prologue must be NONE, ELU or ADDVEC");
  SOPRO_CHECK_ARG(g.epilogue == SOPRO_EPI_NONE || g.epilogue == SOPRO_EPI_GELU || g.epilogue == SOPRO_EPI_RES || g.epilogue == SOPRO_EPI_ROPE,
                  "epilogue must be NONE, GELU, RES, GLU or ROPE");
  if (int rc = check_rope(g, ext)) return rc;
  return small ? launch_cfg3<1, 2, 2, 1, 1>(g, wp, ksubs, ext, s) : launch_cfg3<1, 2, 2, 2, 2>(g, wp, ksubs, ext, s);
}

extern "C" int sopro_gemm_bf16x6(const sopro_gemm_args* a, const void* packed_w, const sopro_gemm_split_ext* x, void* stream) {
  SOPRO_CHECK_ARG(a != nullptr, "args is NULL");
  sopro_gemm_args g = *a;
  sopro_gemm_split_ext ext;
  memset(&ext, 0, sizeof(ext));
  if (x) ext = *x;
  if (ext.group_m == 0) ext.group_m = g_group_m;
  SOPRO_CHECK_ARG(ext.a_format == 0 && (ext.c_mode == 0 || ext.c_mode == 5),
                  "the six-pass path reads fp32 rows and writes fp32 rows, or arg-max partials (c_mode 5)");
  SOPRO_CHECK_ARG(!ext.rms_norm || ((g.K & 31) == 0 && ext.ksplit <= 1 && g.prologue == SOPRO_PRO_NONE && ext.rms_eps > 0.f),
                  "fused RMSNorm needs K % 32 == 0, no split-K, no prologue and eps > 0");
  if (int rc = check_common(g, ext, packed_w)) return rc;
  if (int rc = check_ln(g, ext)) return rc;
  SOPRO_CHECK_ARG(g.prologue == SOPRO_PRO_NONE || g.prologue == SOPRO_PRO_ADDVEC, "prologue must be NONE or ADDVEC");
  SOPRO_CHECK_ARG(g.epilogue == SOPRO_EPI_NONE || g.epilogue == SOPRO_EPI_GELU || g.epilogue == SOPRO_EPI_RES || g.epilogue == SOPRO_EPI_GLU,
                  "epilogue must be NONE, GELU, RES or GLU");
  hipStream_t s = reinterpret_cast<hipStream_t>(stream);
  const uint4* wp = reinterpret_cast<const uint4*>(packed_w);
  const int ksubs = (g.K + 31) / 32 * 2;
  if (ext.c_mode == 5) return launch_argmax<3>(g, wp, ksubs, ext, s);
  switch (g_tile_override) {
    case 1: return launch_cfg6<3, 2, 2, 2, 2>(g, wp, ksubs, ext, s);
    case 4: return launch_cfg6<3, 2, 2, 1, 2>(g, wp, ksubs, ext, s);
    case 5: if (g.epilogue != SOPRO_EPI_GLU) return launch_cfg6<3, 2, 2, 1, 1>(g, wp, ksubs, ext, s); break;
    default: break;
  }
  if (g.epilogue == SOPRO_EPI_GLU) return launch_cfg6<3, 2, 2, 1, 2>(g, wp, ksubs, ext, s);
  return launch_cfg6<3, 2, 2, 1, 1>(g, wp, ksubs, ext, s);
}

extern "C" int sopro_pack_w_f16x2(const float* W, int64_t ldw, int32_t N, int32_t K, float wscale, void* packed, void* stream) {
  SOPRO_CHECK_ARG(W && packed && N > 0 && K > 0 && ldw >= K, "bad pointers or sizes");
  SOPRO_CHECK_ARG(aligned16(packed), "packed must be 16-byte aligned");
  int ex = 0;
  SOPRO_CHECK_ARG(wscale > 0.f && frexpf(wscale, &ex) == 0.5f, "wscale must be a power of two (the scaling has to be exact)");
  const int ksubs = (K + 31) / 32 * 2;
  const int64_t total = (int64_t)((N + 31) / 32) * ksubs * 2 * 64;
  hipLaunchKernelGGL((pack_w_kernel<2, true>), dim3((unsigned)((total + 255) / 256)), dim3(256), 0, (hipStream_t)stream, W, ldw, N, K,
                     reinterpret_cast<uint4*>(packed), ksubs, total, wscale);
  SOPRO_LAUNCH_CHECK();
}

extern "C" float sopro_f16x3_a_scale(void) { return A16_SCALE; }

extern "C" int sopro_gemm_f16x3(const sopro_gemm_args* a, const void* packed_w, const sopro_gemm_split_ext* x, void* stream) {
  SOPRO_CHECK_ARG(a != nullptr && x != nullptr, "args / ext is NULL (ext carries acc_scale)");
  sopro_gemm_args g = *a;
  sopro_gemm_split_ext ext = *x;
  if (ext.group_m == 0) ext.group_m = g_group_m;
  SOPRO_CHECK_ARG(ext.acc_scale > 0.f, "acc_scale = 1 / (sopro_f16x3_a_scale() * the weight's pack scale) must be set");
  SOPRO_CHECK_ARG(ext.a_format == 0 && (ext.c_mode == 0 || ext.c_mode == 5),
                  "the f16 three-pass path reads fp32 rows and writes fp32 rows, or arg-max partials (c_mode 5)");
  SOPRO_CHECK_ARG(!ext.rms_norm || ((g.K & 31) == 0 && ext.ksplit <= 1 && g.prologue == SOPRO_PRO_NONE && ext.rms_eps > 0.f),
                  "fused RMSNorm needs K % 32 == 0, no split-K, no prologue and eps > 0");
  if (int rc = check_common(g, ext, packed_w)) return rc;
  if (int rc = check_ln(g, ext)) return rc;
  SOPRO_CHECK_ARG(g.prologue == SOPRO_PRO_NONE || g.prologue == SOPRO_PRO_ADDVEC, "prologue must be NONE or ADDVEC");
  SOPRO_CHECK_ARG(g.epilogue == SOPRO_EPI_NONE || g.epilogue == SOPRO_EPI_GELU || g.epilogue == SOPRO_EPI_RES || g.epilogue == SOPRO_EPI_GLU,
                  "epilogue must be NONE, GELU, RES or GLU");
  hipStream_t s = reinterpret_cast<hipStream_t>(stream);
  const uint4* wp = reinterpret_cast<const uint4*>(packed_w);
  const int ksubs = (g.K + 31) / 32 * 2;
  if (ext.c_mode == 5) return launch_argmax<2, true>(g, wp, ksubs, ext, s);
  static const int env_tile = SOPRO_DEV_ENV("SOPRO_F16X3_TILE") ? atoi(SOPRO_DEV_ENV("SOPRO_F16X3_TILE")) : 0;
  switch (g_tile_override ? g_tile_override : env_tile) {
    case 1: return launch_cfg6<2, 2, 2, 2, 2, true>(g, wp, ksubs, ext, s);
#ifdef SOPRO_DEV_SWITCHES
    case 3: return launch_cfg6<2, 1, 4, 4, 1, true>(g, wp, ksubs, ext, s);
#endif
    case 4: return launch_cfg6<2, 2, 2, 1, 2, true>(g, wp, ksubs, ext, s);
    case 5: return g.epilogue == SOPRO_EPI_GLU ? launch_cfg6<2, 2, 2, 1, 2, true>(g, wp, ksubs, ext, s) : launch_cfg6<2, 2, 2, 1, 1, true>(g, wp, ksubs, ext, s);
    default: break;
  }
  if (g.M >= 8192 && env_tile == 0) return launch_cfg6<2, 2, 2, 2, 2, true>(g, wp, ksubs, ext, s);
  if (g.epilogue == SOPRO_EPI_GLU) return launch_cfg6<2, 2, 2, 1, 2, true>(g, wp, ksubs, ext, s);
  return launch_cfg6<2, 2, 2, 1, 1, true>(g, wp, ksubs, ext, s);
}
```

sopro_amd/csrc/gemm_epilogue.h:

```cpp
#pragma once
#include "common.h"

constexpr int SOPRO_EPI_GELU_FAST = 100;
constexpr int SOPRO_EPI_GLU_FAST = 101;
template <int WM, int WN, int TM, int TN, int EPI, int OUT = 0>
__device__ __forceinline__ void gemm_store_tile(const sopro_gemm_args& g, float* __restrict__ Cs, f32x16 (&acc)[TM][TN],
                                                const float (&biasv)[TN], int m0, int n0,
                                                const sopro_gemm_split_ext* __restrict__ ext = nullptr,
                                                const float* __restrict__ rs = nullptr, float cscale = 1.0f) {
  constexpr int NT = WM * WN * 64;
  constexpr int BM = WM * TM * 32;
  constexpr int BN = WN * TN * 32;
  const int tid = threadIdx.x, lane = tid & 63, wave = tid >> 6;
  const int wm = wave / WN, wn = wave % WN;
  const int rps = g.rows_per_seg;
  const bool big = (int64_t)g.M * g.N * (OUT >= 6 ? 2 : 4) >= SOPRO_BIG_BYTES;
  constexpr int CLD = BN + 4;
  constexpr bool RES_AHEAD = EPI == SOPRO_EPI_RES && OUT < 5;
  constexpr int RA_TPR = BN / 4, RA_RPP = NT / RA_TPR, RA_NPASS = BM / RA_RPP;
  float4 rahead[RES_AHEAD ? RA_NPASS : 1];
  const bool whole_tile = m0 + BM <= g.M && n0 + BN <= g.N && (m0 / rps) == ((m0 + BM - 1) / rps);
  if constexpr (RES_AHEAD) {
    const int prow = tid / RA_TPR, ocol = n0 + (tid % RA_TPR) * 4;
    const bool rvec = ((g.N & 3) == 0) && ((g.ldr & 3) == 0) && ((g.r_seg_stride & 3) == 0) && ((reinterpret_cast<uintptr_t>(g.R) & 15u) == 0);
    int m = m0 + prow;
    int seg = m / rps, rr = m - seg * rps;
    if (whole_tile && rvec) {
      const float* rptr = g.R + (int64_t)seg * g.r_seg_stride + (int64_t)rr * g.ldr + ocol;
      const int64_t rstep = (int64_t)RA_RPP * g.ldr;
#pragma unroll
      for (int q = 0; q < RA_NPASS; ++q) rahead[q] = *reinterpret_cast<const float4*>(rptr + q * rstep);
    } else {
#pragma unroll
    for (int q = 0; q < RA_NPASS; ++q) {
      rahead[q] = make_float4(0.f, 0.f, 0.f, 0.f);
      if (ocol < g.N && m < g.M) {
        const float* rptr = g.R + (int64_t)seg * g.r_seg_stride + (int64_t)rr * g.ldr + ocol;
        if (rvec) {
          rahead[q] = *reinterpret_cast<const float4*>(rptr);
        } else {
          rahead[q].x = rptr[0];
          if (ocol + 1 < g.N) rahead[q].y = rptr[1];
          if (ocol + 2 < g.N) rahead[q].z = rptr[2];
          if (ocol + 3 < g.N) rahead[q].w = rptr[3];
        }
      }
      m += RA_RPP; rr += RA_RPP;
      while (rr >= rps) { rr -= rps; ++seg; }
    }
    }
  }
  {
    const int col = lane & 31;
#pragma unroll
    for (int i = 0; i < TM; ++i)
#pragma unroll
      for (int k = 0; k < 4; ++k) {
        const int row0 = (wm * TM + i) * 32 + 8 * k + 4 * (lane >> 5);
        float rs4[4] = {cscale, cscale, cscale, cscale};
        if (rs) {
          const float4 t = *reinterpret_cast<const float4*>(rs + row0);
          rs4[0] = t.x; rs4[1] = t.y; rs4[2] = t.z; rs4[3] = t.w;
        }
#pragma unroll
        for (int j = 0; j < TN; ++j)
#pragma unroll
          for (int e = 0; e < 4; ++e) {
            float p = acc[i][j][4 * k + e] * rs4[e];
            if (rs) asm("" : "+v"(p));
            Cs[(row0 + e) * CLD + (wn * TN + j) * 32 + col] = p + biasv[j];
          }
      }
  }
  __syncthreads();
#ifdef SOPRO_DEV_SWITCHES
  if (g.dbg && tid == 0) g.dbg[(int64_t)blockIdx.x * 8 + 4] = clock64();
#endif
  if constexpr (OUT == 5) {
    constexpr int TPR5 = NT / BM;
    constexpr int CPT = BN / TPR5;
    const int row = tid / TPR5, part = tid % TPR5;
    float best = -INFINITY;
    int bi = 0x7fffffff;
#pragma unroll 8
    for (int c = 0; c < CPT; ++c) {
      const int n = n0 + part * CPT + c;
      const float v = Cs[row * CLD + part * CPT + c];
      if (n < g.N && v > best) { best = v; bi = n; }
    }
    constexpr int GRP = CPT >= 64 ? 1 : 64 / CPT;
    static_assert(BN % 64 == 0 && (CPT >= 64 ? CPT == 64 : 64 % CPT == 0), "arg-max partials are per 64 columns");
#pragma unroll
    for (int o = 1; o < GRP; o <<= 1) {
      const float ov = __shfl_xor(best, o, 64);
      const int oi = __shfl_xor(bi, o, 64);
      if (ov > best || (ov == best && oi < bi)) { best = ov; bi = oi; }
    }
    if (part % GRP == 0 && m0 + row < g.M) {
      float* pp = ext->C2 + ((int64_t)(m0 + row) * ext->ldc2 + n0 / 64 + part / GRP) * 2;
      pp[0] = best;
      pp[1] = __int_as_float(bi);
    }
    return;
  }
  if constexpr (OUT >= 6) {
    constexpr bool hres = EPI == SOPRO_EPI_RES;
    static_assert(EPI == SOPRO_EPI_NONE || EPI == SOPRO_EPI_RES, "bf16 rows take EPI_NONE or EPI_RES");
    constexpr int HTPR = BN / 4, HRPP = NT / HTPR, HNPASS = BM / HRPP;
    const int prow = tid / HTPR, pc4 = tid % HTPR;
    const int ocol = n0 + pc4 * 4;
    const bool col_ok = ocol < g.N;
    float4 sc4 = make_float4(1.f, 1.f, 1.f, 1.f);
    if (hres && g.scale && col_ok) sc4 = make_float4(g.scale[ocol], g.scale[ocol + 1], g.scale[ocol + 2], g.scale[ocol + 3]);
    int m = m0 + prow;
    int seg = m / rps, rr = m - seg * rps;
    char* const rawb = reinterpret_cast<char*>(g.C);
    char* const actb = OUT == 8 ? reinterpret_cast<char*>(ext->C2) : rawb;
    const int64_t ldact = OUT == 8 ? ext->ldc2 : g.ldc, segact = OUT == 8 ? ext->c2_seg_stride : g.c_seg_stride;
    const char* const rb = reinterpret_cast<const char*>(g.R);
    auto at = [&](int64_t sg, int64_t r, int64_t ld, int64_t sstride) { return (sg * sstride + r * ld + ocol) * 2; };
    const float* csrc = Cs + prow * CLD + pc4 * 4;
    constexpr int HB = HNPASS < 8 ? HNPASS : 8;
#pragma unroll 1
    for (int p0 = 0; p0 < HNPASS; p0 += HB) {
      int64_t oraw[HB], oact[HB];
      bool okq[HB];
      uint2 rv[HB];
#pragma unroll
      for (int q = 0; q < HB; ++q) {
        okq[q] = col_ok && m < g.M;
        oraw[q] = at(seg, rr, g.ldc, g.c_seg_stride);
        oact[q] = at(seg, rr, ldact, segact);
        rv[q] = make_uint2(0u, 0u);
        if (hres && okq[q]) rv[q] = *reinterpret_cast<const uint2*>(rb + at(seg, rr, g.ldr, g.r_seg_stride));
        m += HRPP; rr += HRPP;
        while (rr >= rps) { rr -= rps; ++seg; }
      }
#pragma unroll
      for (int q = 0; q < HB; ++q) {
        if (!okq[q]) continue;
        float4 v = *reinterpret_cast<const float4*>(csrc + (p0 + q) * HRPP * CLD);
        if (hres) {
          v.x = __uint_as_float(rv[q].x << 16) + sc4.x * v.x; v.y = __uint_as_float(rv[q].x & 0xffff0000u) + sc4.y * v.y;
          v.z = __uint_as_float(rv[q].y << 16) + sc4.z * v.z; v.w = __uint_as_float(rv[q].y & 0xffff0000u) + sc4.w * v.w;
        }
        unsigned lo_;
        if (OUT != 7) {
          uint2 h;
          split2_bf16(v.x, v.y, h.x, lo_);
          split2_bf16(v.z, v.w, h.y, lo_);
          bulk_store_u2(rawb + oraw[q], h, big);
        }
        if (OUT != 6) {
          uint2 h;
          split2_bf16(eluf_(v.x), eluf_(v.y), h.x, lo_);
          split2_bf16(eluf_(v.z), eluf_(v.w), h.y, lo_);
          bulk_store_u2(actb + oact[q], h, big);
        }
      }
    }
    return;
  }
  constexpr bool glu = EPI == SOPRO_EPI_GLU || EPI == SOPRO_EPI_GLU_FAST;
  constexpr bool res = EPI == SOPRO_EPI_RES;
  if constexpr (glu && OUT == 0) {
    constexpr int GT = BN / 4, GRPP = NT / GT, GNP = BM / GRPP;
    const int prow = tid / GT, t = tid % GT;
    const int grp = t >> 4, u = t & 15;
    const int ocol = ((n0 + grp * 64) >> 6) * 32 + 2 * u;
    const bool col_ok = n0 + grp * 64 < g.N;
    const bool st2 = ((g.ldc & 1) == 0) && ((g.c_seg_stride & 1) == 0) && ((reinterpret_cast<uintptr_t>(g.C) & 7u) == 0);
    const float* csrc = Cs + prow * CLD + grp * 64 + 2 * u;
    auto piece = [&](int q, float* cp) {
      const float2 v = *reinterpret_cast<const float2*>(csrc + q * GRPP * CLD), gt = *reinterpret_cast<const float2*>(csrc + q * GRPP * CLD + 32);
      const float ox = v.x * (EPI == SOPRO_EPI_GLU_FAST ? sigmoid_fast(gt.x) : sigmoidf_(gt.x)), oy = v.y * (EPI == SOPRO_EPI_GLU_FAST ? sigmoid_fast(gt.y) : sigmoidf_(gt.y));
      if (st2) {
        bulk_store_u2(cp, make_uint2(__float_as_uint(ox), __float_as_uint(oy)), big);
      } else {
        cp[0] = ox;
        cp[1] = oy;
      }
    };
    if (!col_ok) return;
    if (m0 + BM <= g.M && (m0 / rps) == ((m0 + BM - 1) / rps)) {
      const int m = m0 + prow, seg = m / rps, rr = m - seg * rps;
      float* cptr = g.C + (int64_t)seg * g.c_seg_stride + (int64_t)rr * g.ldc + ocol;
      const int64_t cstep = (int64_t)GRPP * g.ldc;
#pragma unroll
      for (int q = 0; q < GNP; ++q) {
        piece(q, cptr + q * cstep);
#ifdef SOPRO_DEV_SWITCHES
        if (g.dbg && tid == 0 && q == GNP / 2 - 1) g.dbg[(int64_t)blockIdx.x * 8 + 5] = clock64();
#endif
      }
    } else {
#pragma unroll 1
      for (int q = 0; q < GNP; ++q) {
        const int m = m0 + prow + q * GRPP;
        if (m >= g.M) break;
        const int seg = m / rps, rr = m - seg * rps;
        piece(q, g.C + (int64_t)seg * g.c_seg_stride + (int64_t)rr * g.ldc + ocol);
      }
    }
    return;
  }
  constexpr int TPR = BN / 4;
  constexpr int RPP = NT / TPR;
  constexpr int NPASS = BM / RPP;
  const int prow = tid / TPR, pc4 = tid % TPR;
  const int n_out_total = glu ? g.N / 2 : g.N;
  const int ncol = n0 + pc4 * 4;
  const int ocol = glu ? (ncol >> 6) * 32 + (ncol & 31) : ncol;
  const bool col_ok = ocol < n_out_total && (!glu || ((pc4 * 4) & 32) == 0);
  const bool vec_ok = ((n_out_total & 3) == 0) && ((g.ldc & 3) == 0) && ((g.c_seg_stride & 3) == 0) &&
                      ((reinterpret_cast<uintptr_t>(g.C) & 15u) == 0) &&
                      (!res || (((g.ldr & 3) == 0) && ((g.r_seg_stride & 3) == 0) && ((reinterpret_cast<uintptr_t>(g.R) & 15u) == 0)));
  float4 sc4 = make_float4(1.f, 1.f, 1.f, 1.f);
  if (res && g.scale) {
    sc4.x = ncol + 0 < g.N ? g.scale[ncol + 0] : 1.f; sc4.y = ncol + 1 < g.N ? g.scale[ncol + 1] : 1.f;
    sc4.z = ncol + 2 < g.N ? g.scale[ncol + 2] : 1.f; sc4.w = ncol + 3 < g.N ? g.scale[ncol + 3] : 1.f;
  }
  int m = m0 + prow;
  int seg = m / rps, rr = m - seg * rps;
  float* cptr = g.C + (int64_t)seg * g.c_seg_stride + (int64_t)rr * g.ldc + ocol;
  constexpr bool second = OUT == 2 || OUT == 4;
  constexpr bool split_out = OUT == 1 || OUT == 2;
  float* const dbase = second ? ext->C2 : g.C;
  const int64_t ldd = second ? ext->ldc2 : g.ldc, dseg = second ? ext->c2_seg_stride : g.c_seg_stride;
  const int64_t dcol_bytes = split_out ? (int64_t)(ocol >> 5) * 128 + (ocol & 31) * 2 : (int64_t)ocol * 4;
  char* dptr = OUT != 0 ? reinterpret_cast<char*>(dbase + (int64_t)seg * dseg + (int64_t)rr * ldd) + dcol_bytes : nullptr;
  const int64_t dstep = (int64_t)RPP * ldd * 4;
  const int64_t cstep = (int64_t)RPP * g.ldc;
  const float* csrc = Cs + prow * CLD + pc4 * 4;
  constexpr int BATCH = NPASS < 8 ? NPASS : 8;
  static_assert(!RES_AHEAD || (RA_NPASS == NPASS && RA_RPP == RPP), "the residual pieces requested ahead are the store loop's");
  auto emit = [&](int pq, float* cpq, char* dpq, const float4& rvq) {
    {
      float4 v = *reinterpret_cast<const float4*>(csrc + pq * RPP * CLD);
      if (glu) {
        const float4 gt = *reinterpret_cast<const float4*>(csrc + pq * RPP * CLD + 32);
        v.x *= sigmoidf_(gt.x); v.y *= sigmoidf_(gt.y); v.z *= sigmoidf_(gt.z); v.w *= sigmoidf_(gt.w);
      } else if (EPI == SOPRO_EPI_GELU) {
        v.x = gelu_erf(v.x); v.y = gelu_erf(v.y); v.z = gelu_erf(v.z); v.w = gelu_erf(v.w);
      } else if (EPI == SOPRO_EPI_GELU_FAST) {
        v.x = gelu_fast(v.x); v.y = gelu_fast(v.y); v.z = gelu_fast(v.z); v.w = gelu_fast(v.w);
      } else if (EPI == SOPRO_EPI_TANH) {
        v.x = tanhf(v.x); v.y = tanhf(v.y); v.z = tanhf(v.z); v.w = tanhf(v.w);
      } else if (res) {
        v.x = rvq.x + sc4.x * v.x; v.y = rvq.y + sc4.y * v.y; v.z = rvq.z + sc4.z * v.z; v.w = rvq.w + sc4.w * v.w;
        if (OUT == 0 && ext && ext->ln_stats_out) {
          float s1 = (v.x + v.y) + (v.z + v.w);
          s1 += __shfl_xor(s1, 1, 64); s1 += __shfl_xor(s1, 2, 64); s1 += __shfl_xor(s1, 4, 64); s1 += __shfl_xor(s1, 8, 64);
          const float mu = s1 * (1.0f / 64.0f);
          const float dx = v.x - mu, dy = v.y - mu, dz = v.z - mu, dw = v.w - mu;
          float s2 = (dx * dx + dy * dy) + (dz * dz + dw * dw);
          s2 += __shfl_xor(s2, 1, 64); s2 += __shfl_xor(s2, 2, 64); s2 += __shfl_xor(s2, 4, 64); s2 += __shfl_xor(s2, 8, 64);
          if ((pc4 & 15) == 0) {
            const int64_t mq = m0 + prow + pq * RPP;
            *reinterpret_cast<float2*>(ext->ln_stats_out + (mq * (g.N >> 6) + (ncol >> 6)) * 2) = make_float2(mu, s2);
          }
        }
      } else if (EPI == SOPRO_EPI_ROPE) {
        if (ncol < ext->rope_cols) {
          const int half = ext->rope_dh >> 1, e = ncol & (ext->rope_dh - 1);
          const bool lowh = e < half;
          const float4 pv = *reinterpret_cast<const float4*>(csrc + pq * RPP * CLD + (lowh ? half : -half));
          const int mq = m0 + prow + pq * RPP;
          const int64_t ti = (int64_t)(ext->rope_pos0 + mq % ext->rope_rows_per_seg) * half + (e & (half - 1));
          const float4 c4 = *reinterpret_cast<const float4*>(ext->rope_cos + ti), s4 = *reinterpret_cast<const float4*>(ext->rope_sin + ti);
          if (lowh) { v.x = v.x * c4.x - pv.x * s4.x; v.y = v.y * c4.y - pv.y * s4.y; v.z = v.z * c4.z - pv.z * s4.z; v.w = v.w * c4.w - pv.w * s4.w; }
          else { v.x = v.x * c4.x + pv.x * s4.x; v.y = v.y * c4.y + pv.y * s4.y; v.z = v.z * c4.z + pv.z * s4.z; v.w = v.w * c4.w + pv.w * s4.w; }
        }
      }
      if (split_out) {
        uint2 h, l;
        split2_bf16(eluf_(v.x), eluf_(v.y), h.x, l.x);
        split2_bf16(eluf_(v.z), eluf_(v.w), h.y, l.y);
        *reinterpret_cast<uint2*>(dpq) = h;
        *reinterpret_cast<uint2*>(dpq + 64) = l;
        if (OUT == 1) return;
      } else if (OUT != 0) {
        bulk_store4(reinterpret_cast<float*>(dpq), make_float4(eluf_(v.x), eluf_(v.y), eluf_(v.z), eluf_(v.w)), big);
        if (OUT == 3) return;
      }
      if (vec_ok) {
        bulk_store4(cpq, v, big);
      } else {
        cpq[0] = v.x;
        if (ocol + 1 < n_out_total) cpq[1] = v.y;
        if (ocol + 2 < n_out_total) cpq[2] = v.z;
        if (ocol + 3 < n_out_total) cpq[3] = v.w;
      }
    }
  };
  if (whole_tile && vec_ok) {
    if (col_ok) {
#pragma unroll
      for (int q = 0; q < NPASS; ++q) {
        emit(q, cptr + q * cstep, OUT != 0 ? dptr + q * dstep : nullptr, rahead[RES_AHEAD ? q : 0]);
#ifdef SOPRO_DEV_SWITCHES
        if (g.dbg && tid == 0 && q == BATCH - 1) g.dbg[(int64_t)blockIdx.x * 8 + 5] = clock64();
#endif
      }
    }
    return;
  }
  auto batch = [&](int p0, const float4* rvb) {
    float* cp[BATCH];
    char* dp[BATCH];
    float4 rv[BATCH];
#pragma unroll
    for (int q = 0; q < BATCH; ++q) {
      const bool ok = col_ok && m < g.M;
      cp[q] = ok ? cptr : nullptr;
      dp[q] = dptr;
      rv[q] = res ? rvb[q] : make_float4(0.f, 0.f, 0.f, 0.f);
      m += RPP; rr += RPP; cptr += cstep;
      if (OUT != 0) dptr += dstep;
      if (rr >= rps) {
        do { rr -= rps; ++seg; } while (rr >= rps);
        cptr = g.C + (int64_t)seg * g.c_seg_stride + (int64_t)rr * g.ldc + ocol;
        if (OUT != 0) dptr = reinterpret_cast<char*>(dbase + (int64_t)seg * dseg + (int64_t)rr * ldd) + dcol_bytes;
      }
    }
#pragma unroll
    for (int q = 0; q < BATCH; ++q) {
      if (!cp[q]) continue;
      emit(p0 + q, cp[q], dp[q], rv[q]);
    }
  };
  if constexpr (RES_AHEAD) {
#pragma unroll
    for (int b = 0; b < NPASS / BATCH; ++b) {
      batch(b * BATCH, rahead + b * BATCH);
#ifdef SOPRO_DEV_SWITCHES
      if (g.dbg && tid == 0 && b == 0) g.dbg[(int64_t)blockIdx.x * 8 + 5] = clock64();
#endif
    }
  } else {
#pragma unroll 1
    for (int p0 = 0; p0 < NPASS; p0 += BATCH) {
      batch(p0, nullptr);
#ifdef SOPRO_DEV_SWITCHES
      if (g.dbg && tid == 0 && p0 == 0) g.dbg[(int64_t)blockIdx.x * 8 + 5] = clock64();
#endif
    }
  }
}
```

sopro_amd/csrc/stages.hip:

```cpp
#include <stdlib.h>

#include <algorithm>
#include <map>
#include <string>
#include <vector>

#include "common.h"

int sopro_stream_batch_append(float* cur, float* other, const float* qkv, int32_t hs, int32_t rows, int64_t bstride, int32_t n, int32_t kv_len,
                              int32_t nkeep, hipStream_t s);
int sopro_stream_batch_gather(float* kv, const int32_t* keep, int32_t n_keep, int32_t layers, int32_t rows_cap, int64_t bstride, int32_t hs, int32_t half,
                              int32_t kv_len, hipStream_t s);

namespace {

struct Ten {
  const void* p = nullptr;
  int64_t shape[4] = {0, 0, 0, 0};
  int ndim = 0;
  const float* f() const { return reinterpret_cast<const float*>(p); }
};

struct Wt {
  const float* f32 = nullptr;
// ... 169 lines not shown
  SOPRO_HIP(hipMemcpy(hv.data(), v->p, (size_t)K * 4, hipMemcpyDeviceToHost));
  for (int n = 0; n < N; ++n) {
    double acc = 0.0;
    for (int k = 0; k < K; ++k) acc += (double)hw[(size_t)n * K + k] * hv[k];
    ho[n] = (float)acc;
  }
  float* d;
  STG(dev_upload(e, ho, &d));
  Ten o;
  o.p = d; o.shape[0] = N; o.ndim = 1;
  e->t[out_key] = o;
  return 0;
}

int plain(sopro_engine* e, const std::string& key) {
  const Ten* t;
  STG(need(e, key, &t));
  Wt w;
  w.f32 = t->f();
  e->w[key] = w;
  return 0;
}

constexpr size_t SPLITK_WS_BYTES = (size_t)32 << 20;
constexpr int SPLITK_TICKETS = 1024;
struct SplitK {
  float* ws = nullptr;
  int32_t* tickets = nullptr;
};

int auto_ksplit(int M, int N, int K, int pieces, int epi) {
  int bm, bn;
  if (pieces == 3) {
    bm = 64; bn = epi == SOPRO_EPI_GLU ? 128 : 64;
  } else if (pieces == 1) {
    const bool small = N <= 64 || M <= 64 || (int64_t)((M + 127) / 128) * ((N + 127) / 128) < 256;
    if (small) { bm = 64; bn = epi == SOPRO_EPI_GLU ? 128 : 64; } else { bm = bn = 128; }
  } else {
    if (N <= 64 || M <= 64) bm = bn = 64; else bm = bn = 128;
  }
  const int64_t tiles = (int64_t)((M + bm - 1) / bm) * ((N + bn - 1) / bn);
  const int kt = (K + 31) / 32;
  if (tiles >= 96 || kt < 32 || tiles > SPLITK_TICKETS) return 1;
  int ks = (int)lrint(sqrt(2.5 * kt));
  if (ks > 16) ks = 16;
  if (ks > 512 / (int)tiles) ks = 512 / (int)tiles;
  if (ks < 1) ks = 1;
  while (ks > 1 && (size_t)ks * tiles * bm * bn * 4 > SPLITK_WS_BYTES) --ks;
  return ks;
}

struct G {
  int M = 0, N = 0, K = 0;
  int64_t lda = -1, ldc = -1, ldr = -1, ldw = -1;
  const float *bias = nullptr, *R = nullptr, *scale = nullptr, *pro_vec = nullptr;
  int epi = SOPRO_EPI_NONE, pro = SOPRO_PRO_NONE, rows_per_seg = -1;
  int64_t a_seg = 0, c_seg = 0, r_seg = 0;
  int c_mode = 0;
  int a_fmt = 0;
  float* C2 = nullptr;
  int64_t ldc2 = -1, c2_seg = 0;
  float rms_eps = 0.f;
  const SplitK* sk = nullptr;
  int32_t* range_events = nullptr;
  const float *rope_cos = nullptr, *rope_sin = nullptr;
  int rope_cols = 0, rope_dh = 0, rope_pos0 = 0, rope_rps = 0;
  const float* ln_stats = nullptr;
  float* ln_stats_out = nullptr;
  float ln_eps = 0.f;
};

int attend(const sopro_attn_args& a, hipStream_t s, int split_passes = 0) {
  double pairs = (double)a.Tq * a.Tk;
  if (a.causal) {
    pairs = 0;
    for (int q = 0; q < a.Tq; ++q) {
      const int hi = std::min(a.Tk - 1, a.q_pos0 + q - a.k_pos0), lo = std::max(0, a.q_pos0 + q - a.window + 1 - a.k_pos0);
      pairs += std::max(0, hi - lo + 1);
    }
  }
  sopro_prof_scope prof(split_passes ? "attention_split_kernel" : "attention_kernel", 4.0 * a.dh * pairs * a.B * a.H, s);
  if (split_passes) return sopro_attention_split_bf16(&a, split_passes, s);
  return sopro_attention_f32(&a, s);
}

int gemm(hipStream_t s, const float* A, const Wt& w, const float* w_f32_override, float* C, const G& o) {
  const int n_out = o.epi == SOPRO_EPI_GLU ? o.N / 2 : o.N;
  sopro_gemm_args g;
  memset(&g, 0, sizeof(g));
  g.A = A;
  g.lda = o.lda < 0 ? o.K : o.lda;
  g.a_seg_stride = o.a_seg;
  g.W = w_f32_override ? w_f32_override : w.f32;
  g.ldw = o.ldw < 0 ? o.K : o.ldw;
  g.bias = o.bias;
  g.C = C;
  g.ldc = o.ldc < 0 ? n_out : o.ldc;
  g.c_seg_stride = o.c_seg;
  g.R = o.R;
  g.ldr = o.ldr < 0 ? n_out : o.ldr;
  g.r_seg_stride = o.r_seg;
  g.scale = o.scale;
  g.pro_vec = o.pro_vec;
  g.M = o.M; g.N = o.N; g.K = o.K;
  g.rows_per_seg = o.rows_per_seg < 0 ? o.M : o.rows_per_seg;
  g.prologue = o.pro; g.epilogue = o.epi;
  const bool split = !w_f32_override && w.packed;
  sopro_prof_scope prof(!split ? "gemm_f32_kernel" : w.f16 ? "gemm_f16x3_kernel" : w.pieces == 3 ? "gemm_bf16x6_kernel"
                        : w.pieces == 1 ? "gemm_bf16x1_kernel" : "gemm_bf16x3_kernel", 2.0 * o.M * o.N * o.K, s);
  if (split) {
    sopro_gemm_split_ext x;
    memset(&x, 0, sizeof(x));
    x.c_mode = o.c_mode;
    x.a_format = o.a_fmt;
    x.C2 = o.C2;
    x.ldc2 = o.ldc2 < 0 ? n_out : o.ldc2;
    x.c2_seg_stride = o.c2_seg;
    if (o.rms_eps > 0.f) { x.rms_norm = 1; x.rms_eps = o.rms_eps; }
    x.rope_cos = o.rope_cos; x.rope_sin = o.rope_sin; x.rope_cols = o.rope_cols; x.rope_dh = o.rope_dh; x.rope_pos0 = o.rope_pos0;
    x.rope_rows_per_seg = o.rope_rps;
    x.ln_stats = o.ln_stats; x.ln_stats_out = o.ln_stats_out;
    if (o.ln_stats) x.rms_eps = o.ln_eps;
    static const bool no_splitk = getenv("SOPRO_NO_SPLITK") && getenv("SOPRO_NO_SPLITK")[0] == '1';
    if (!no_splitk && o.sk && o.sk->ws && o.rms_eps <= 0.f && o.c_mode != 5) {
      const int ks = auto_ksplit(o.M, o.N, o.K, w.f16 ? 3 : w.pieces, o.epi);
      if (ks > 1) {
        x.ksplit = ks; x.n_tickets = SPLITK_TICKETS; x.ws = o.sk->ws; x.ws_bytes = (int64_t)SPLITK_WS_BYTES; x.tickets = o.sk->tickets;
      }
    }
    if (w.f16) {
      x.acc_scale = w.acc_scale;
      x.range_events = o.range_events;
      return sopro_gemm_f16x3(&g, w.packed, &x, s);
    }
    if (w.pieces == 3) return sopro_gemm_bf16x6(&g, w.packed, &x, s);
    if (w.pieces == 1) return sopro_gemm_bf16x1(&g, w.packed, &x, s);
    if (w.rows) {
      sopro_gemm_split_ext x8 = x;
      x8.ksplit = 0;
      if (sopro_gemm_8p_takes(&g, &x8)) return sopro_gemm_bf16x3_8p(&g, w.rows, &x8, s);
    }
    return sopro_gemm_bf16x3(&g, w.packed, &x, s);
  }
  if (!g.W) {
    sopro_set_error("stage API: a contraction has neither an fp32 nor a packed weight");
    return -2;
  }
  return sopro_gemm_f32(&g, s);
}

int norm(hipStream_t s, const float* x, float* out, const float* w, int rows, int C, float eps, int kind = SOPRO_NORM_RMS,
         const float* b = nullptr, const float* mul = nullptr, const float* add = nullptr, int rows_per_seg = -1, int64_t x_seg = 0) {
  return sopro_norm_f32(x, C, x_seg, out, C, w, b, mul, add, rows, rows_per_seg < 0 ? rows : rows_per_seg, C, eps, kind, s);
}

}

extern "C" {

int sopro_engine_create(const sopro_engine_cfg* cfg, sopro_engine** out) {
  SOPRO_CHECK_ARG(cfg && out, "NULL argument");
  SOPRO_CHECK_ARG(cfg->d_model == 384 && cfg->n_layers_ar >= 1 && cfg->n_layers_ar <= 16 && cfg->n_layers_nar >= 1 && cfg->n_layers_nar <= 16,
                  "d_model must be 384 (kernel family), 1..16 layers");
  SOPRO_CHECK_ARG(cfg->n_stages >= 1 && cfg->n_stages <= 8 && cfg->num_codebooks <= 64 && cfg->mimi_n_ratios >= 1 && cfg->mimi_n_ratios <= 8,
                  "1..8 NAR stages, <= 64 codebooks, 1..8 decoder ratios");
  sopro_engine* e = new sopro_engine();
  e->c = *cfg;
  *out = e;
  return 0;
}

int sopro_engine_set_tensor(sopro_engine* e, const char* name, const void* dev_ptr, const int64_t* shape, int32_t ndim) {
  SOPRO_CHECK_ARG(e && name && dev_ptr && shape && ndim >= 1 && ndim <= 4, "bad arguments");
  SOPRO_CHECK_ARG(!e->final, "the engine is finalized");
  Ten t;
  t.p = dev_ptr;
  t.ndim = ndim;
  for (int i = 0; i < ndim; ++i) t.shape[i] = shape[i];
  e->t[name] = t;
  return 0;
}

int sopro_engine_upload_tensor(sopro_engine* e, const char* name, const float* host_ptr, const int64_t* shape, int32_t ndim, void* stream) {
  SOPRO_CHECK_ARG(e && name && host_ptr && shape && ndim >= 1 && ndim <= 4, "bad arguments");
  SOPRO_CHECK_ARG(!e->final, "the engine is finalized");
  size_t n = 1;
  for (int i = 0; i < ndim; ++i) {
    SOPRO_CHECK_ARG(shape[i] > 0, "empty dimension");
    n *= (size_t)shape[i];
  }
  float* d = nullptr;
  STG(dev_alloc(e, n, &d));
  (void)stream;
  SOPRO_HIP(hipMemcpy(d, host_ptr, n * sizeof(float), hipMemcpyHostToDevice));
  return sopro_engine_set_tensor(e, name, d, shape, ndim);
}

int sopro_engine_set_ar_tiles(sopro_engine* e, int32_t glu, int32_t ff1, int32_t ff2, int32_t head) {
  SOPRO_CHECK_ARG(e != nullptr, "engine is NULL");
  e->ar_tiles[0] = glu; e->ar_tiles[1] = ff1; e->ar_tiles[2] = ff2; e->ar_tiles[3] = head;
  if (e->ar.graph) {
    (void)sopro_graph_destroy(e->ar.graph);
    e->ar.graph = nullptr;
  }
  return 0;
}

int sopro_engine_destroy(sopro_engine* e) {
  if (!e) return 0;
  if (e->ar.graph) (void)sopro_graph_destroy(e->ar.graph);
  for (void* p : e->owned) (void)hipFree(p);
// ... 500 lines not shown
                           vdst, B, S, p.S_cap, D, H, RMS_EPS, s));
    if (c.precision == 1) {
      STG(sopro_cvt_f32_bf16(kdst, p.kp[i], (int64_t)B * H * p.S_cap * D, s));
      STG(sopro_cvt_f32_bf16(vdst, p.vp[i], (int64_t)B * H * p.S_cap * D, s));
    }
  }
  for (int i = 0; i < c.n_layers_ar; ++i) {
    const int64_t n = (int64_t)((c.ar_kernel - 1) * c.ar_dilations[i] + 1) * B * D;
    STG(sopro_fill2d_u32(p.rings[i], n, 1, (int32_t)n, 0u, s));
  }
  STG(sopro_fill2d_u32(p.hist, (int64_t)B * Tar, 1, B * Tar, 0u, s));
  for (int k = 0; k < 8; ++k) {
    uint32_t u;
    memcpy(&u, &params[k], 4);
    STG(sopro_fill2d_u32(p.params + k, 1, 1, 1, u, s));
  }
  STG(sopro_fill2d_u32(p.nonce, B, 1, B, nonce, s));
  STG(sopro_fill2d_u32(p.key, 1, 1, 1, (uint32_t)seed, s));
  STG(sopro_fill2d_u32(p.key + 1, 1, 1, 1, (uint32_t)(seed >> 32), s));
  sopro_ar_state& st = p.st;
  memset(&st, 0, sizeof(st));
  st.x_cur = p.x[0]; st.cond = p.cond; st.emb = F(e, "cb_embed"); st.hist = p.hist;
  st.step = p.ctr; st.row_step = p.row_step; st.n_stopped = p.ctr + 2;
  st.first_eos = p.first_eos; st.stop_t = p.stop_t; st.recent = p.recent; st.params = p.params; st.nonce = p.nonce;
  st.key = p.key; st.seed = 0; st.B = B; st.D = D; st.Tar = Tar; st.max_steps = Tar; st.V = c.codebook_size; st.bos_row = c.bos_row;
  STG(sopro_ar_init(&st, s));
  if (p.graph && (p.graph_B != B || p.graph_S_cap != p.S_cap || p.graph_Tar != Tar || p.graph_ws != workspace)) {
    STG(sopro_graph_destroy(p.graph));
    p.graph = nullptr;
  }
  return 0;
}

int sopro_ar_run_graph(sopro_engine* e, int32_t n_steps, void* stream) {
  SOPRO_CHECK_ARG(e && e->ar.ws && n_steps >= 0 && stream, "sopro_ar_begin first; a non-default stream is needed for graph capture");
  ArPlan& p = e->ar;
  if (!p.graph) {
    STG(sopro_capture_begin(stream));
    const int rc = ar_issue_step(e, (hipStream_t)stream);
    void* g = nullptr;
    const int rc2 = sopro_capture_end(stream, &g);
    if (rc != 0) return rc;
    if (rc2 != 0) return rc2;
    p.graph = g; p.graph_B = p.B; p.graph_S_cap = p.S_cap; p.graph_Tar = p.Tar; p.graph_ws = p.ws;
  }
  for (int i = 0; i < n_steps; ++i) STG(sopro_graph_launch(p.graph, stream));
  return 0;
}

int sopro_ar_tokens(sopro_engine* e, int32_t* hist, int32_t* first_eos, int32_t* n_stopped, void* stream) {
  SOPRO_CHECK_ARG(e && e->ar.ws, "sopro_ar_begin first");
  hipStream_t s = (hipStream_t)stream;
  const ArPlan& p = e->ar;
  if (hist) STG(sopro_copy2d_u32(hist, (int64_t)p.B * p.Tar, p.hist, (int64_t)p.B * p.Tar, 1, p.B * p.Tar, s));
  if (first_eos) STG(sopro_copy2d_u32(first_eos, p.B, p.first_eos, p.B, 1, p.B, s));
  if (n_stopped) STG(sopro_copy2d_u32(n_stopped, 1, p.ctr + 2, 1, 1, 1, s));
  return 0;
}

struct NarWs { float *xa, *xb, *h, *x1, *u, *z, *part, *cond; int32_t *lens, *range; SplitK sk; };
static size_t nar_carve(const sopro_engine* e, NarWs& w, void* ws, int B, int T) {
  const sopro_engine_cfg& c = e->c;
  const size_t M = (size_t)B * T, D = c.d_model;
  int nh_max = 0;
  for (int i = 0; i < c.n_stages; ++i) nh_max = c.stage_n_cb[i] > nh_max ? c.stage_n_cb[i] : nh_max;
  Carver cv(ws);
  w.xa = cv.take<float>(M * D); w.xb = cv.take<float>(M * D); w.h = cv.take<float>(M * D); w.x1 = cv.take<float>(M * D);
  w.u = cv.take<float>(M * 4 * D); w.z = cv.take<float>(M * c.nar_head_dim);
  w.part = cv.take<float>(M * nh_max * (c.codebook_size / 64) * 2);
  w.cond = cv.take<float>(M * D);
  w.lens = cv.take<int32_t>(B);
  w.range = cv.take<int32_t>(4);
  w.sk.tickets = cv.take<int32_t>(SPLITK_TICKETS);
  w.sk.ws = M <= 1024 ? cv.take<float>(SPLITK_WS_BYTES / 4) : nullptr;
  return cv.off;
}

int64_t sopro_nar_workspace_bytes(const sopro_engine* e, int32_t B, int32_t T) {
  if (!e || B <= 0 || T <= 0) return 0;
  NarWs w;
  return (int64_t)nar_carve(e, w, nullptr, B, T);
}

static int ssm_block_bufs(sopro_engine* e, hipStream_t s, float* h, float* x1, float* u, const SplitK* sk, const float* x, float* out,
                          const std::string& p, int B, int T, int ksize, int dil, const int32_t* lens, const char* sfx, int32_t* range) {
  const int D = e->c.d_model, M = B * T;
  const int total = (ksize - 1) * dil, left = total / 2;
  G g; g.M = M; g.N = 2 * D; g.K = D; g.bias = F(e, p + ".glu.b"); g.epi = SOPRO_EPI_GLU; g.rms_eps = RMS_EPS; g.range_events = range;
  STG(gemm(s, x, WT(e, p + ".glu.wn" + sfx), nullptr, h, g));
  STG(sopro_dwconv_f32(h, F(e, p + ".dw.w"), F(e, p + ".dw.b"), x, x1, lens, B, T, D, ksize, dil, left, 1, s));
  G f1; f1.M = M; f1.N = 4 * D; f1.K = D; f1.bias = F(e, p + ".ff1.b"); f1.epi = SOPRO_EPI_GELU; f1.rms_eps = RMS_EPS; f1.range_events = range;
  STG(gemm(s, x1, WT(e, p + ".ff1.wn" + sfx), nullptr, u, f1));
  G f2; f2.M = M; f2.N = D; f2.K = 4 * D; f2.bias = F(e, p + ".ff2.b"); f2.epi = SOPRO_EPI_RES; f2.R = x1; f2.sk = sk; f2.range_events = range;
  return gemm(s, u, WT(e, p + ".ff2.w" + sfx), nullptr, out, f2);
}
static int ssm_block_seq(sopro_engine* e, hipStream_t s, const NarWs& w, const float* x, float* out, const std::string& p, int B, int T,
                         int ksize, int dil, const int32_t* lens, const char* sfx) {
  return ssm_block_bufs(e, s, w.h, w.x1, w.u, &w.sk, x, out, p, B, T, ksize, dil, lens, sfx, w.range);
}

int sopro_nar_refine_io(sopro_engine* e, void* workspace, const sopro_nar_io* io, int32_t B, int32_t T, void* stream) {
  SOPRO_CHECK_ARG(e && e->final && e->has_nar && workspace && io && io->cond && io->cb0 && io->tokens && B > 0 && T > 0,
                  "bad arguments (finalize the engine with the NAR tensors first)");
  hipStream_t s = (hipStream_t)stream;
  const sopro_engine_cfg& c = e->c;
  const int D = c.d_model, V = c.codebook_size, Q = c.num_codebooks, HD = c.nar_head_dim, M = B * T;
  SOPRO_CHECK_ARG(V % 64 == 0, "codebook_size must be a multiple of 64 (arg-max partials per 64 columns)");
  SOPRO_CHECK_ARG(io->cond_bstride >= (int64_t)T * D && io->cb0_bstride >= T, "cond / cb0 blocks shorter than T rows");
  const bool safe = io->safe != 0 && c.precision == 0;
  const char* sfx = safe ? NAR_SAFE : "";
  int32_t* tokens = io->tokens;
  NarWs w;
  nar_carve(e, w, workspace, B, T);
  if (w.sk.ws) STG(sopro_fill2d_u32(w.sk.tickets, SPLITK_TICKETS, 1, SPLITK_TICKETS, 0u, s));
  STG(sopro_fill2d_u32(w.range, 4, 1, 4, 0u, s));
  int nh_max = 0;
  for (int i = 0; i < c.n_stages; ++i) nh_max = c.stage_n_cb[i] > nh_max ? c.stage_n_cb[i] : nh_max;
  const float* cnd = io->cond;
  if (io->cond_bstride != (int64_t)T * D) {
    STG(sopro_copy2d_u32(w.cond, (int64_t)T * D, io->cond, io->cond_bstride, B, T * D, s));
    cnd = w.cond;
  }
  STG(sopro_nar_seed_i32(tokens, Q, io->cb0, io->cb0_bstride, B, T, V - 1, s));
  const int32_t* lens_d = nullptr;
  if (io->lens) {
    STG(sopro_copy2d_u32(w.lens, B, io->lens, B, 1, B, s));
    lens_d = w.lens;
  }
  const char* stage_names[8] = {"B", "C", "D", "E", "F", "G", "H", "I"};
  for (int sid = 0; sid < c.n_stages; ++sid) {
    float *xa = w.xa, *xb = w.xb;
    STG(sopro_codebook_sum_f32(tokens, Q, e->nar_cols[sid], e->nar_offs[sid], e->nar_cw[sid], e->nar_known[sid], F(e, "cb_embed"),
                               e->t["cb_embed"].shape[0], cnd, c.nar_mix[sid][0], c.nar_mix[sid][1], xa, D, 0, M, M, D, s));
    STG(norm(s, xa, xb, F(e, "nar.adapter.norm.weight"), M, D, RMS_EPS, SOPRO_NORM_RMS, nullptr, e->ad_mul[sid], e->ad_add[sid], M));
    std::swap(xa, xb);
    for (int i = 0; i < c.n_layers_nar; ++i) {
      STG(ssm_block_seq(e, s, w, xa, xb, "nar.blocks." + std::to_string(i), B, T, c.nar_kernel, c.nar_dilations[i], lens_d, sfx));
      std::swap(xa, xb);
    }
    STG(norm(s, xa, xb, F(e, "nar.norm.weight"), M, D, RMS_EPS));
    G pz; pz.M = M; pz.N = HD; pz.K = D; pz.bias = F(e, "nar.pre.b"); pz.range_events = w.range;
    STG(gemm(s, xb, WT(e, std::string("nar.pre.w") + sfx), nullptr, w.z, pz));
    const int nh = c.stage_n_cb[sid];
    const std::string hk = std::string("nar.heads.") + stage_names[sid];
    G hg; hg.M = M; hg.N = nh * V; hg.K = HD; hg.bias = F(e, hk + ".b"); hg.c_mode = 5; hg.C2 = w.part; hg.ldc2 = (int64_t)nh_max * (V / 64);
    hg.range_events = w.range;
    STG(gemm(s, w.z, WT(e, hk + ".w" + sfx), nullptr, nullptr, hg));
    STG(sopro_argmax_partials_i32(w.part, (int64_t)nh_max * (V / 64), tokens + c.stage_first_cb[sid], Q, nh, V / 64, V, M, s));
  }
  if (io->range_out) STG(sopro_copy2d_u32(io->range_out, 1, w.range, 1, 1, 1, s));
  return 0;
}

int sopro_nar_refine(sopro_engine* e, void* workspace, const float* cond, int64_t cond_bstride, const int32_t* rvq1, const int32_t* lens,
                     int32_t B, int32_t T, int32_t* tokens, void* stream) {
  sopro_nar_io io;
  memset(&io, 0, sizeof(io));
  io.cond = cond; io.cond_bstride = cond_bstride; io.cb0 = rvq1; io.cb0_bstride = T; io.lens = lens; io.tokens = tokens;
  return sopro_nar_refine_io(e, workspace, &io, B, T, stream);
}

struct MimiWs {
  int32_t* tok;
  float *emb, *q, *X, *y, *qkv, *ao, *hd, *e0, *hraw[8], *hact[8], *y1[8];
  float* lnst;
  SplitK sk;
};
static bool mimi_half(const sopro_engine* e) {
  static const bool off = getenv("SOPRO_MIMI_BF16") != nullptr && getenv("SOPRO_MIMI_BF16")[0] == '0';
  return e->c.precision == 1 && !off;
}

static bool seanet_fused(int B, int rows) {
  static const bool off = SOPRO_DEV_ENV("SOPRO_SEANET_FUSE") != nullptr && SOPRO_DEV_ENV("SOPRO_SEANET_FUSE")[0] == '0';
  return !off && (int64_t)B * rows >= 512 * 1024;
}

static size_t mimi_carve(const sopro_engine* e, MimiWs& w, void* ws, int B, int T) {
  const sopro_engine_cfg& c = e->c;
  const bool half = mimi_half(e);
  auto act = [&](Carver& cv_, size_t n) { return half ? reinterpret_cast<float*>(cv_.take<uint16_t>(n)) : cv_.take<float>(n); };
  const size_t HS = c.mimi_hidden, CD = c.mimi_codebook_dim, N2 = 2 * (size_t)T, PADX = c.mimi_kernel - 1;
  Carver cv(ws);
  w.tok = cv.take<int32_t>((size_t)B * T * c.num_codebooks);
  w.sk.tickets = cv.take<int32_t>(SPLITK_TICKETS);
  w.sk.ws = (size_t)B * N2 <= 512 ? cv.take<float>(SPLITK_WS_BYTES / 4) : nullptr;
  w.emb = cv.take<float>((size_t)B * T * 2 * CD);
  w.q = cv.take<float>((size_t)B * T * HS);
  w.X = cv.take<float>((size_t)B * (PADX + N2) * HS);
  w.y = cv.take<float>((size_t)B * N2 * HS);
  w.qkv = cv.take<float>((size_t)B * N2 * 3 * HS);
  w.ao = cv.take<float>((size_t)B * N2 * HS);
  w.hd = cv.take<float>((size_t)B * N2 * c.mimi_inter);
  w.lnst = cv.take<float>((size_t)B * N2 * ((HS + 63) / 64) * 2);
  size_t ch = (size_t)c.mimi_num_filters << c.mimi_n_ratios, rows = N2;
  w.e0 = act(cv, (size_t)B * (1 + rows) * ch);
  for (int si = 0; si < c.mimi_n_ratios; ++si) {
    const size_t co = ch / 2, orow = rows * c.mimi_ratios[si];
    const bool on_cu = si + 1 == c.mimi_n_ratios && ch == 128 && c.mimi_ratios[si] == 4 && seanet_fused(B, (int)rows);
    w.hraw[si] = on_cu ? nullptr : act(cv, (size_t)B * (2 + orow) * co);
    w.hact[si] = si + 1 < c.mimi_n_ratios ? act(cv, (size_t)B * (2 + orow) * co) : nullptr;
    w.y1[si] = si + 1 < c.mimi_n_ratios ? act(cv, (size_t)B * orow * (co / c.mimi_compress)) : nullptr;
    ch = co; rows = orow;
  }
  return cv.off;
}

int64_t sopro_mimi_workspace_bytes(const sopro_engine* e, int32_t B, int32_t T) {
  if (!e || B <= 0 || T <= 0) return 0;
  MimiWs w;
  return (int64_t)mimi_carve(e, w, nullptr, sopro_mimi_chunk_rows(B, T), T);
}

static int transformer_stack(sopro_engine* e, hipStream_t s, const char* pre, float* X, int PADX, int64_t xs, float* y, float* qkv, float* ao,
                             float* hd, const SplitK* sk, int B, int n, int past, sopro_mimi_stream_state* sst, int attn_split = 0,
                             float* lnst = nullptr, sopro_mimi_stream_batch* sbt = nullptr) {
  const sopro_engine_cfg& c = e->c;
  const int HS = c.mimi_hidden, H = c.mimi_heads, dh = c.mimi_head_dim;
  struct { float *X, *y, *qkv, *ao, *hd; SplitK sk; } w{X, y, qkv, ao, hd, sk ? *sk : SplitK()};
  static const bool ln_off = SOPRO_DEV_ENV("SOPRO_LN_FUSE") != nullptr && SOPRO_DEV_ENV("SOPRO_LN_FUSE")[0] == '0';
  const bool fused_ln = !ln_off && lnst != nullptr && WT(e, std::string(pre) + ".0.qkv.w#ln").packed != nullptr;
  if (fused_ln) STG(sopro_row_stats_f32(w.X + (size_t)PADX * HS, HS, xs, B * n, n, HS, lnst, s));
  for (int l = 0; l < c.mimi_layers; ++l) {
    const std::string p = std::string(pre) + "." + std::to_string(l);
    if (!fused_ln)
      STG(norm(s, w.X + (size_t)PADX * HS, w.y, F(e, p + ".ln1.w"), B * n, HS, c.mimi_norm_eps, SOPRO_NORM_LN, F(e, p + ".ln1.b"), nullptr, nullptr, n, xs));
    G qg; qg.sk = &w.sk; qg.M = B * n; qg.N = 3 * HS; qg.K = HS;
    if (fused_ln) {
      qg.ln_stats = lnst; qg.ln_eps = c.mimi_norm_eps; qg.bias = F(e, p + ".qkv.lnb"); qg.a_seg = xs; qg.rows_per_seg = n;
      qg.c_seg = (int64_t)n * 3 * HS;
// ... 465 lines not shown
```

sopro_amd/hip.py:

```python
from __future__ import annotations

import ctypes as C
import gc
import os
import threading
from typing import List, Optional, Tuple

import torch

_HERE = os.path.dirname(os.path.abspath(__file__))
LIB_PATH = os.path.join(_HERE, "libsopro_hip.so")
ABI_VERSION = 42
DEV_MODE = os.environ.get("SOPRO_DEV", "0") == "1"


def dev_env(name: str, default: str) -> str:
    return os.environ.get(name, default) if DEV_MODE else default


DEFAULT_GROUP_M = 8
PRO_NONE, PRO_ELU, PRO_ADDVEC = 0, 1, 2
EPI_ROPE = 6
EPI_NONE, EPI_GELU, EPI_GLU, EPI_RES, EPI_TANH, EPI_GLU_DW = 0, 1, 2, 3, 4, 5
NORM_RMS, NORM_LN = 0, 1
# ... 40 lines not shown
                ("np", _i32), ("B", _i32), ("H", _i32), ("D", _i32), ("S_cap", _i32),
                ("Qp", _p), ("qp_stride", _i64), ("nqp", _i32), ("k_unfolded", _i32), ("kv_format", _i32)]


class ArState(C.Structure):
    _fields_ = [("x_cur", _p), ("cond", _p), ("emb", _p), ("hist", _p), ("step", _p), ("row_step", _p),
                ("first_eos", _p), ("stop_t", _p), ("n_stopped", _p), ("recent", _p), ("params", _p), ("seed", C.c_uint64),
                ("B", _i32), ("D", _i32), ("Tar", _i32), ("max_steps", _i32), ("V", _i32), ("bos_row", _i32),
                ("start", _p), ("row_max", _p), ("row_params", _p), ("nonce", _p), ("row_id", _p), ("key", _p), ("dbg", _p)]


AR_MAX_LAYERS = 16


class ArBlock(C.Structure):
    _fields_ = [("glu_w", _p), ("glu_b", _p), ("dw_w", _p), ("dw_b", _p), ("ff1_w", _p), ("ff1_b", _p), ("ff2_w", _p), ("ff2_b", _p),
                ("ring", _p), ("kp", _p), ("vp", _p), ("dil", _i32), ("xattn", _i32), ("gate", _f32), ("pad_", _i32),
                ("qa_w", _p), ("qu_w", _p), ("q_b", _p)]


class ArFrame(C.Structure):
    _fields_ = [("blk", ArBlock * AR_MAX_LAYERS), ("head_w", _p), ("head_b", _p), ("x0", _p), ("xa", _p), ("xb", _p), ("part", _p),
                ("u", _p), ("xp", _p), ("qa", _p), ("qpart", _p), ("logits", _p), ("klens", _p),
                ("n_layers", _i32), ("B", _i32), ("D", _i32), ("S_cap", _i32), ("V1", _i32), ("H", _i32), ("ksize", _i32), ("w_layout", _i32),
                ("tile_glu", _i32), ("tile_ff1", _i32), ("tile_ff2", _i32), ("tile_head", _i32), ("eps", _f32), ("k_unfold", _i32), ("store_format", _i32),
                ("st", ArState)]


class EngineCfg(C.Structure):
    _fields_ = [("d_model", _i32), ("codebook_size", _i32), ("num_codebooks", _i32), ("nar_head_dim", _i32), ("bos_row", _i32),
                ("n_layers_ar", _i32), ("ar_kernel", _i32), ("ar_dilations", _i32 * 16), ("ar_xattn", _i32 * 16), ("ar_gate", _f32 * 16),
                ("n_layers_nar", _i32), ("nar_kernel", _i32), ("nar_dilations", _i32 * 16),
                ("n_stages", _i32), ("stage_first_cb", _i32 * 8), ("stage_n_cb", _i32 * 8), ("nar_mix", (_f32 * 2) * 8),
                ("nar_prev_cb_weights", _f32 * 64),
                ("mimi_hidden", _i32), ("mimi_codebook_dim", _i32), ("mimi_heads", _i32), ("mimi_head_dim", _i32), ("mimi_layers", _i32),
                ("mimi_window", _i32), ("mimi_inter", _i32), ("mimi_n_ratios", _i32), ("mimi_ratios", _i32 * 8), ("mimi_num_filters", _i32),
                ("mimi_kernel", _i32), ("mimi_res_kernel", _i32), ("mimi_last_kernel", _i32), ("mimi_compress", _i32),
                ("mimi_n_semantic", _i32), ("mimi_rope_positions", _i32), ("mimi_norm_eps", _f32), ("mimi_final_bias", _f32), ("precision", _i32),
                ("n_layers_text", _i32), ("ref_enc_layers", _i32), ("ref_xattn_layers", _i32), ("ref_xattn_heads", _i32), ("sv_student_dim", _i32),
                ("enc_kernel", _i32)]


class NarIO(C.Structure):
    _fields_ = [("cond", _p), ("cond_bstride", _i64), ("cb0", _p), ("cb0_bstride", _i64), ("lens", _p), ("tokens", _p), ("range_out", _p),
                ("safe", _i32)]


class MimiStreamState(C.Structure):
    _fields_ = [("kv", _p), ("cap_rows", _i32), ("kv_len", _i32), ("pos", _i32), ("evict", _i32), ("half", _i32)]


class MimiStreamBatch(C.Structure):
    _fields_ = [("kv", _p), ("rows_cap", _i32), ("rows", _i32), ("cap_rows", _i32), ("kv_len", _i32), ("pos", _i32), ("evict", _i32),
                ("half", _i32)]


SYMBOLS = {
    "sopro_last_error": (C.c_char_p, []),
    "sopro_abi_version": (C.c_int, []),
    "sopro_build_flags": (C.c_int, []),
    "sopro_graph_launch_n": (C.c_int, [_p, _p, _i32]),
    "sopro_host_alloc": (C.c_int, [_i64, C.POINTER(_p)]),
    "sopro_host_free": (C.c_int, [_p]),
    "sopro_copy_to_host_async": (C.c_int, [_p, _p, _i64, _p]),
    "sopro_set_lds_floor": (C.c_int, [C.c_int]),
    "sopro_set_host_wait": (C.c_int, [C.c_int]),
    "sopro_device_info": (C.c_int, [C.c_int, C.POINTER(C.c_int)]),
    "sopro_capture_begin": (C.c_int, [_p]),
    "sopro_capture_end": (C.c_int, [_p, C.POINTER(_p)]),
    "sopro_graph_launch": (C.c_int, [_p, _p]),
    "sopro_graph_destroy": (C.c_int, [_p]),
    "sopro_stream_create_cu_range": (C.c_int, [C.c_int, C.c_int, C.POINTER(_p)]),
    "sopro_stream_create_cu_mask": (C.c_int, [_p, _i32, _p]),
    "sopro_stream_destroy": (C.c_int, [_p]),
    "sopro_gemm_f32": (C.c_int, [C.POINTER(GemmArgs), _p]),
    "sopro_gemm_bf16x3": (C.c_int, [_p, _p, _p, _p]),
    "sopro_gemm_bf16x6": (C.c_int, [_p, _p, _p, _p]),
    "sopro_gemm_bf16x1": (C.c_int, [_p, _p, _p, _p]),
    "sopro_pack_w_bf16": (C.c_int, [_p, _i64, _i32, _i32, _i32, _p, _p]),
    "sopro_fill2d_u32": (C.c_int, [_p, _i64, _i32, _i32, C.c_uint32, _p]),
    "sopro_copy2d_u32": (C.c_int, [_p, _i64, _p, _i64, _i32, _i32, _p]),
    "sopro_pack_w_f16x2": (C.c_int, [_p, _i64, _i32, _i32, _f32, _p, _p]),
    "sopro_f16x3_a_scale": (C.c_float, []),
    "sopro_gemm_f16x3": (C.c_int, [_p, _p, _p, _p]),
    "sopro_packed_w_bytes": (C.c_int64, [_i32, _i32, _i32]),
    "sopro_packed_w_rows_bytes": (C.c_int64, [_i32, _i32]),
    "sopro_pack_w_rows_bf16": (C.c_int, [_p, _i64, _i32, _i32, _p, _p]),
    "sopro_gemm_8p_takes": (C.c_int, [_p, _p]),
    "sopro_gemm_bf16x3_8p": (C.c_int, [_p, _p, _p, _p]),
    "sopro_gemm_bf16_set_tile_override": (C.c_int, [C.c_int]),
    "sopro_gemm_set_group_m": (C.c_int, [C.c_int]),
    "sopro_seanet_tail_set_tiles": (C.c_int, [C.c_int]),
    "sopro_seanet_res_set_tiles": (C.c_int, [C.c_int]),
    "sopro_seanet_res128_bf16": (C.c_int, [_p, _i64, _p, _p, _p, _p, _p, _i64, _i32, _i32, _p]),
    "sopro_seanet_up128_bf16": (C.c_int, [_p, _i64, _p, _p, _p, _i64, _i32, _i32, _p]),
    "sopro_seanet_tail_bf16": (C.c_int, [_p, _i64, _p, _p, _p, _p, _p, _f32, _p, _i64, _i32, _i32, _p]),
    "sopro_seanet_up_set_tiles": (C.c_int, [C.c_int]),
    "sopro_seanet_uptail_set_tiles": (C.c_int, [C.c_int]),
    "sopro_seanet_uptail_f32": (C.c_int, [_p, _i64, _p, _p, _p, _p, _p, _p, _p, _f32, _p, _i64, _i32, _i32, _i32, _p]),
    "sopro_seanet_uptail_bf16": (C.c_int, [_p, _i64, _p, _p, _p, _p, _p, _p, _p, _f32, _p, _i64, _i32, _i32, _p]),
    "sopro_seanet_up128_f32": (C.c_int, [_p, _i64, _p, _p, _p, _i64, _i32, _i32, _i32, _p]),
    "sopro_seanet_res128_f32": (C.c_int, [_p, _i64, _p, _p, _p, _p, _p, _i64, _i32, _i32, _p]),
    "sopro_gemm_set_tile_override": (C.c_int, [C.c_int]),
    "sopro_pack_skinny_w": (C.c_int, [_p, _i64, _i32, _i32, _i32, _p, _p]),
    "sopro_pack_skinny_w_bf16": (C.c_int, [_p, _i64, _i32, _i32, _i32, _p, _p]),
    "sopro_skinny_packed_floats": (_i64, [_i32, _i32, _i32]),
    "sopro_skinny_f32": (C.c_int, [C.POINTER(SkinnyArgs), _p]),
    "sopro_row_stats_f32": (C.c_int, [_p, _i64, _i64, _i32, _i32, _i32, _p, _p]),
    "sopro_norm_f32": (C.c_int, [_p, _i64, _i64, _p, _i64, _p, _p, _p, _p, _i32, _i32, _i32, _f32, _i32, _p]),
    "sopro_rms_match_f32": (C.c_int, [_p, _p, _p, _i32, _i32, _p]),
    "sopro_tanh_affine_f32": (C.c_int, [_p, _p, _f32, _f32, _i64, _p]),
    "sopro_add_pos_f32": (C.c_int, [_p, _p, _p, _i32, _i32, _i32, _i32, _p]),
    "sopro_masked_mean_f32": (C.c_int, [_p, _p, _p, _i32, _i32, _i32, _p]),
    "sopro_stats_pool_f32": (C.c_int, [_p, _p, _p, _p, _i32, _i32, _i32, _p]),
    "sopro_l2norm_f32": (C.c_int, [_p, _p, _i32, _i32, _f32, _p]),
    "sopro_dwconv_f32": (C.c_int, [_p, _p, _p, _p, _p, _p, _i32, _i32, _i32, _i32, _i32, _i32, _i32, _p]),
    "sopro_codebook_sum_f32": (C.c_int, [_p, _i32, _p, _p, _p, _i32, _p, _i64, _p, _f32, _f32, _p, _i64, _i64, _i32, _i32, _i32, _p]),
    "sopro_text_embed_f32": (C.c_int, [_p, _p, _p, _i64, _p, _p, _i32, _i32, _i32, _p]),
    "sopro_argmax_rows_f32": (C.c_int, [_p, _i64, _p, _i64, _i32, _i32, _i32, _p]),
    "sopro_argmax_partials_i32": (C.c_int, [_p, _i64, _p, _i64, _i32, _i32, _i32, _i32, _p]),
    "sopro_fir1_f32": (C.c_int, [_p, _i64, _i32, _p, _p, _p, _i64, _i64, _i32, _i32, _i32, _i32, _i32, _i32, _p]),
    "sopro_rvq_assign_f32": (C.c_int, [_p, _i64, _i32, _p, _p, _i64, _i32, _p, _i64, _i32, _p]),
    "sopro_attention_f32": (C.c_int, [C.POINTER(AttnArgs), _p]),
    "sopro_attention_split_bf16": (C.c_int, [C.POINTER(AttnArgs), C.c_int32, _p]),
    "sopro_attn_decode_f32": (C.c_int, [C.POINTER(AttnArgs), _p]),
    "sopro_xattn_step_f32": (C.c_int, [C.POINTER(XattnArgs), _p]),
    "sopro_rope_f32": (C.c_int, [_p, _i64, _p, _p, _i32, _i32, _i32, _i32, _i32, _p]),
    "sopro_upsample2_f32": (C.c_int, [_p, _p, _p, _i64, _i32, _i32, _i32, _p]),
    "sopro_final_conv_f32": (C.c_int, [_p, _i64, _p, _f32, _p, _i64, _i32, _i32, _p]),
    "sopro_seanet_tail_f32": (C.c_int, [_p, _i64, _p, _p, _p, _p, _p, _f32, _p, _i64, _i32, _i32, _p]),
    "sopro_seanet_res128_p_f32": (C.c_int, [_p, _i64, _p, _p, _p, _p, _p, _i64, _i32, _i32, _i32, _p]),
    "sopro_seanet_tail_p_f32": (C.c_int, [_p, _i64, _p, _p, _p, _p, _p, _f32, _p, _i64, _i32, _i32, _i32, _p]),
    "sopro_engine_create": (C.c_int, [C.POINTER(EngineCfg), C.POINTER(_p)]),
    "sopro_engine_set_tensor": (C.c_int, [_p, C.c_char_p, _p, C.POINTER(_i64), _i32]),
    "sopro_engine_finalize": (C.c_int, [_p, _p]),
    "sopro_engine_destroy": (C.c_int, [_p]),
    "sopro_ar_workspace_bytes": (_i64, [_p, _i32, _i32, _i32]),
    "sopro_ar_begin": (C.c_int, [_p, _p, _i32, _p, _p, _p, _i32, _i32, C.POINTER(_f32), C.c_uint64, C.c_uint32, _p]),
    "sopro_ar_run_graph": (C.c_int, [_p, _i32, _p]),
    "sopro_ar_tokens": (C.c_int, [_p, _p, _p, _p, _p]),
    "sopro_nar_workspace_bytes": (_i64, [_p, _i32, _i32]),
    "sopro_nar_refine": (C.c_int, [_p, _p, _p, _i64, _p, _p, _i32, _i32, _p, _p]),
    "sopro_nar_refine_io": (C.c_int, [_p, _p, C.POINTER(NarIO), _i32, _i32, _p]),
    "sopro_nar_seed_i32": (C.c_int, [_p, _i32, _p, _i64, _i32, _i32, _i32, _p]),
    "sopro_mimi_workspace_bytes": (_i64, [_p, _i32, _i32]),
    "sopro_mimi_decode": (C.c_int, [_p, _p, _p, _i32, _i32, _p, _p]),
    "sopro_mimi_chunk_rows": (_i32, [_i32, _i32]),
    "sopro_mimi_decode_parts": (C.c_int, [_p, _p, _p, _i32, _i32, _p, _i32, _p]),
    "sopro_mimi_stream_kv_bytes": (_i64, [_p, _i32]),
    "sopro_mimi_stream_init": (C.c_int, [_p, C.POINTER(MimiStreamState), _p, _i32]),
    "sopro_mimi_stream_trim": (C.c_int, [C.POINTER(MimiStreamState), _i32]),
    "sopro_mimi_decode_stream": (C.c_int, [_p, _p, C.POINTER(MimiStreamState), _p, _i32, _p, _p]),
    "sopro_mimi_stream_batch_kv_bytes": (_i64, [_p, _i32, _i32]),
    "sopro_mimi_stream_batch_init": (C.c_int, [_p, C.POINTER(MimiStreamBatch), _p, _i32, _i32]),
    "sopro_mimi_stream_batch_trim": (C.c_int, [C.POINTER(MimiStreamBatch), _i32]),
    "sopro_mimi_stream_batch_keep": (C.c_int, [_p, C.POINTER(MimiStreamBatch), C.POINTER(_i32), _i32, _p]),
    "sopro_mimi_decode_stream_batch": (C.c_int, [_p, _p, C.POINTER(MimiStreamBatch), _p, _i32, _p, _p]),
    "sopro_ar_init": (C.c_int, [C.POINTER(ArState), _p]),
    "sopro_ar_sample": (C.c_int, [C.POINTER(ArState), _p, _i64, _p]),
    "sopro_ar_admit": (C.c_int, [C.POINTER(ArState), _i32, _p]),
    "sopro_ar_issue_frame": (C.c_int, [C.POINTER(ArFrame), _p]),
    "sopro_ar_fold_text": (C.c_int, [_p, _p, _p, _p, _p, _p, _p, _p, _p, _i32, _i32, _i32, _i32, _i32, _f32, _p]),
    "sopro_ar_fold_text_uk": (C.c_int, [_p, _p, _p, _p, _p, _p, _p, _p, _i32, _i32, _i32, _i32, _i32, _f32, _p]),
    "sopro_engine_upload_tensor": (C.c_int, [_p, C.c_char_p, _p, C.POINTER(_i64), _i32, _p]),
    "sopro_checkpoint_open": (C.c_int, [C.c_char_p, C.c_char_p, C.POINTER(_p)]),
    "sopro_checkpoint_close": (C.c_int, [_p]),
# ... 135 lines not shown

def set_profiler(p: Optional[Profiler]) -> None:
    global _prof
    _prof = p
    load().sopro_prof_enable(1 if p is not None else 0)


def _check(rc: int, what: str) -> None:
    if rc != 0:
        raise SoproHipError(f"{what} failed ({rc}): {load().sopro_last_error().decode()}")


def _stream() -> int:
    return torch.cuda.current_stream().cuda_stream


def ptr(t: Optional[torch.Tensor], dtype: torch.dtype = torch.float32) -> Optional[int]:
    if t is None:
        return None
    if not t.is_cuda:
        raise SoproHipError("tensor is not on a HIP device: the Sopro hot path has no CPU fallback")
    if t.dtype != dtype:
        raise SoproHipError(f"expected {dtype}, got {t.dtype}")
    return t.data_ptr()


def gemm(A: torch.Tensor, W, Cout: torch.Tensor, *, M: int, N: int, K: int, lda: Optional[int] = None,
         ldc: Optional[int] = None, bias: Optional[torch.Tensor] = None, epilogue: int = EPI_NONE,
         prologue: int = PRO_NONE, R: Optional[torch.Tensor] = None, ldr: Optional[int] = None,
         scale: Optional[torch.Tensor] = None, pro_vec: Optional[torch.Tensor] = None, rows_per_seg: Optional[int] = None,
         a_seg_stride: int = 0, c_seg_stride: int = 0, r_seg_stride: int = 0, a_off: int = 0, c_off: int = 0,
         r_off: int = 0, ldw: Optional[int] = None, dbg: Optional[torch.Tensor] = None, a_split: bool = False, c_mode: int = 0,
         C2: Optional[torch.Tensor] = None, ldc2: Optional[int] = None, c2_seg_stride: int = 0,
         c2_off: int = 0, rms_eps: float = 0.0, range_events: Optional[torch.Tensor] = None, rope: Optional[tuple] = None,
         ln_stats: Optional[torch.Tensor] = None, ln_eps: float = 0.0, ln_stats_out: Optional[torch.Tensor] = None,
         long_k: Optional[bool] = None) -> None:
    n_out = N // 2 if epilogue == EPI_GLU else N
    g = GemmArgs()
    a16 = A.dtype == torch.bfloat16
    c16 = c_mode in (6, 7, 8)
    cdt = torch.bfloat16 if c16 else torch.float32
    g.A = ptr(A, A.dtype if a16 else torch.float32) + (2 if a16 else 4) * a_off
    g.lda = K if lda is None else lda
    g.a_seg_stride = a_seg_stride
    packed = isinstance(W, PackedW)
    if packed and (W.N != N or W.K != K):
        raise SoproHipError(f"packed weight is [{W.N}, {W.K}], the call wants [{N}, {K}]")
    g.W = None if packed else ptr(W)
    g.ldw = K if ldw is None else ldw
    g.bias = ptr(bias)
    g.C = (ptr(Cout, cdt) + (2 if c16 else 4) * c_off) if Cout is not None else None
    g.ldc = n_out if ldc is None else ldc
    g.c_seg_stride = c_seg_stride
    g.R = (ptr(R, cdt) + (2 if c16 else 4) * r_off) if R is not None else None
    g.ldr = (n_out if ldr is None else ldr)
    g.r_seg_stride = r_seg_stride
    g.scale = ptr(scale)
    g.pro_vec = ptr(pro_vec)
    g.dbg = ptr(dbg, torch.int64)
    g.M, g.N, g.K = M, N, K
    g.rows_per_seg = M if rows_per_seg is None else rows_per_seg
    g.prologue, g.epilogue = prologue, epilogue
    e0 = _prof.begin() if _prof is not None else None
    x = None
    if packed:
        x = SplitExt()
        if rope is not None:
            x.rope_cos, x.rope_sin = ptr(rope[0]), ptr(rope[1])
            x.rope_cols, x.rope_dh, x.rope_pos0, x.rope_rows_per_seg = int(rope[2]), int(rope[3]), int(rope[4]), int(rope[5])
        if ln_stats is not None:
            x.ln_stats, x.rms_eps = ptr(ln_stats), float(ln_eps)
        x.ln_stats_out = ptr(ln_stats_out)
        if rms_eps > 0.0:
            if W.pieces == 2 and not W.f16:
                raise SoproHipError("fused RMSNorm is a six-pass (pieces = 3), f16 three-pass or one-pass (pieces = 1) feature")
            x.rms_norm, x.rms_eps = 1, float(rms_eps)
        ks = _auto_ksplit(M, N, K, 3 if W.f16 else W.pieces, epilogue) if (dbg is None and _splitk_enabled and rms_eps <= 0.0) else 1
        if ks > 1:
            ws, tk = _splitk_buffers()
            x.ksplit, x.n_tickets, x.ws, x.ws_bytes, x.tickets = ks, int(tk.numel()), ptr(ws), int(ws.numel()) * 4, ptr(tk, torch.int32)
    if (a16 or c16) and not (packed and W.pieces == 1 and not W.f16):
        raise SoproHipError("bf16 rows (a_format 2, c_mode 6 / 7 / 8) belong to the one-pass (pieces = 1) path")
    if packed and W.f16:
        if a_split or c_mode not in (0, 5):
            raise SoproHipError("split-form operands belong to the bf16 three-pass (pieces = 2) path")
        if c_mode == 5:
            x.c_mode, x.C2, x.ldc2 = 5, ptr(C2) + 4 * c2_off, (-(-N // 64) if ldc2 is None else ldc2)
        x.acc_scale = W.acc_scale
        x.range_events = ptr(range_events, torch.int32)
        _check(load().sopro_gemm_f16x3(C.byref(g), ptr(W.data, torch.int32), C.byref(x), _stream()), "sopro_gemm_f16x3")
    elif packed and W.pieces == 1:
        if a_split or c_mode in (1, 2):
            raise SoproHipError("split-form operands belong to the three-pass (pieces = 2) path")
        x.c_mode = c_mode
        x.a_format = 2 if a16 else 0
        x.C2 = (ptr(C2, cdt) + (2 if c16 else 4) * c2_off) if C2 is not None else None
        x.ldc2, x.c2_seg_stride = (n_out if ldc2 is None else ldc2), c2_seg_stride
        _check(load().sopro_gemm_bf16x1(C.byref(g), ptr(W.data, torch.int32), C.byref(x), _stream()), "sopro_gemm_bf16x1")
    elif packed and W.pieces == 3:
        if a_split or c_mode not in (0, 5):
            raise SoproHipError("split-form operands belong to the three-pass (pieces = 2) path")
        if c_mode == 5:
            x.c_mode, x.C2, x.ldc2 = 5, ptr(C2) + 4 * c2_off, (-(-N // 64) if ldc2 is None else ldc2)
        _check(load().sopro_gemm_bf16x6(C.byref(g), ptr(W.data, torch.int32), C.byref(x), _stream()), "sopro_gemm_bf16x6")
    elif packed:
        if a16 or c16:
            raise SoproHipError("bf16 rows (a_format 2, c_mode 6 / 7 / 8) belong to the one-pass (pieces = 1) path")
        x.a_format, x.c_mode = int(bool(a_split)), c_mode
        x.C2 = (ptr(C2) + 4 * c2_off) if C2 is not None else None
        x.ldc2, x.c2_seg_stride = (n_out if ldc2 is None else ldc2), c2_seg_stride
        use_8p = long_k if long_k is not None else (W.rows is not None and bool(load().sopro_gemm_8p_takes(C.byref(g), C.byref(x))))
        if use_8p:
            if W.rows is None:
                raise SoproHipError("the long-K form needs the weight's split-form rows (pack_w_bf16x3(W, rows=True))")
            x.ksplit = 0
            _check(load().sopro_gemm_bf16x3_8p(C.byref(g), W.rows.data_ptr(), C.byref(x), _stream()), "sopro_gemm_bf16x3_8p")
        else:
            _check(load().sopro_gemm_bf16x3(C.byref(g), ptr(W.data, torch.int32), C.byref(x), _stream()), "sopro_gemm_bf16x3")
    elif a_split or c_mode:
        raise SoproHipError("split-plane operands need a PackedW weight (the fp32 kernel reads and writes fp32 rows)")
    else:
        _check(load().sopro_gemm_f32(C.byref(g), _stream()), "sopro_gemm_f32")
    if e0 is not None:
        fam = "gemm_f32_kernel" if not packed else ("gemm_f16x3_kernel" if W.f16 else {1: "gemm_bf16x1_kernel", 2: "gemm_bf16x3_kernel", 3: "gemm_bf16x6_kernel"}[W.pieces])
        _prof.end(fam, 2.0 * M * N * K, e0)


_splitk_enabled = os.environ.get("SOPRO_NO_SPLITK", "0") != "1"
_splitk_pool: dict = {}
_SPLITK_WS_BYTES = 32 << 20
_SPLITK_TICKETS = 1024


def _auto_ksplit(M: int, N: int, K: int, pieces: int, epilogue: int) -> int:
    if pieces == 3:
        bm, bn = (64, 128) if epilogue == EPI_GLU else (64, 64)
    elif pieces == 1:
        small = N <= 64 or M <= 64 or (-(-M // 128) * -(-N // 128)) < 256
        bm, bn = ((64, 128) if epilogue == EPI_GLU else (64, 64)) if small else (128, 128)
    else:
        bm, bn = (64, 64) if (N <= 64 or M <= 64) else (128, 128)
    tiles = -(-M // bm) * -(-N // bn)
    kt = -(-K // 32)
    if tiles >= 96 or kt < 32 or tiles > _SPLITK_TICKETS:
        return 1
    ks = max(1, min(16, int(round((2.5 * kt) ** 0.5)), 512 // tiles))
    while ks > 1 and ks * tiles * bm * bn * 4 > _SPLITK_WS_BYTES:
        ks -= 1
    return ks


def _splitk_buffers():
    key = _stream()
    bufs = _splitk_pool.get(key)
    if bufs is None:
        dev = torch.cuda.current_device()
        bufs = (torch.empty(_SPLITK_WS_BYTES // 4, dtype=torch.float32, device=f"cuda:{dev}"),
                torch.zeros(_SPLITK_TICKETS, dtype=torch.int32, device=f"cuda:{dev}"))
        _splitk_pool[key] = bufs
    return bufs


class PackedW:

    __slots__ = ("data", "N", "K", "pieces", "f16", "acc_scale", "rows")

    def __init__(self, data: torch.Tensor, N: int, K: int, pieces: int, f16: bool = False, acc_scale: float = 1.0):
        self.data, self.N, self.K, self.pieces, self.f16, self.acc_scale = data, N, K, pieces, f16, acc_scale
        self.rows = None

# ... 224 lines not shown
    if e0 is not None:
        pairs = float(Tq) * Tk if not causal else float(sum(max(0, min(Tk - 1, q_pos0 + q - k_pos0) - max(0, q_pos0 + q - window + 1 - k_pos0) + 1) for q in range(Tq)))
        _prof.end("attention_kernel", 4.0 * dh * pairs * B * H, e0)


def xattn_step(X: torch.Tensor, Y: torch.Tensor, norm_w: Optional[torch.Tensor], Kp: torch.Tensor, Vp: torch.Tensor, klens: Optional[torch.Tensor], *,
               B: int, H: int, D: int, S_cap: int, gate: float, scale: float, eps: float, Xp: Optional[torch.Tensor] = None, np_: int = 0,
               xp_stride: int = 0, y_part_stride: int = 0, Qp: Optional[torch.Tensor] = None, nqp: int = 0, qp_stride: int = 0) -> None:
    a = XattnArgs()
    if Qp is not None:
        a.Qp, a.nqp, a.qp_stride, a.k_unfolded = ptr(Qp), int(nqp), int(qp_stride), 1
    a.X, a.ldx, a.Xp, a.xp_stride, a.np = ptr(X), D, ptr(Xp), xp_stride, np_
    kv16 = Kp.dtype == torch.bfloat16
    a.norm_w, a.Kp, a.Vp, a.klens = ptr(norm_w), ptr(Kp, Kp.dtype), ptr(Vp, Kp.dtype), ptr(klens, torch.int32)
    a.kv_format = 1 if kv16 else 0
    a.Y, a.y_part_stride = ptr(Y), y_part_stride
    a.eps, a.gate, a.scale = eps, gate, scale
    a.B, a.H, a.D, a.S_cap = B, H, D, S_cap
    _check(load().sopro_xattn_step_f32(C.byref(a), _stream()), "sopro_xattn_step_f32")


def rope(x: torch.Tensor, cos_t: torch.Tensor, sin_t: torch.Tensor, *, rows: int, rows_per_seg: int, pos0: int, H: int,
         dh: int, ldx: int, x_off: int = 0) -> None:
    _check(load().sopro_rope_f32(ptr(x) + 4 * x_off, ldx, ptr(cos_t), ptr(sin_t), rows, rows_per_seg, pos0, H, dh, _stream()),
           "sopro_rope_f32")


def upsample2(x: torch.Tensor, w: torch.Tensor, y: torch.Tensor, *, B: int, T: int, C_: int, y_seg_stride: int,
              y_off: int = 0) -> None:
    _check(load().sopro_upsample2_f32(ptr(x), ptr(w), ptr(y) + 4 * y_off, y_seg_stride, B, T, C_, _stream()), "sopro_upsample2_f32")


def final_conv(h: torch.Tensor, w: torch.Tensor, bias: float, wav: torch.Tensor, *, B: int, T: int, h_seg_stride: int,
               wav_seg_stride: int) -> None:
    _check(load().sopro_final_conv_f32(ptr(h), h_seg_stride, ptr(w), bias, ptr(wav), wav_seg_stride, B, T, _stream()),
           "sopro_final_conv_f32")


def seanet_tail(h: torch.Tensor, w1: torch.Tensor, b1: torch.Tensor, w2: torch.Tensor, b2: torch.Tensor, wf: torch.Tensor,
                bf: float, wav: torch.Tensor, *, B: int, T: int, h_seg_stride: int, wav_seg_stride: int) -> None:
    _check(load().sopro_seanet_tail_f32(ptr(h), h_seg_stride, ptr(w1), ptr(b1), ptr(w2), ptr(b2), ptr(wf), bf, ptr(wav),
                                        wav_seg_stride, B, T, _stream()), "sopro_seanet_tail_f32")


def seanet_res128(h: torch.Tensor, w1: torch.Tensor, b1: torch.Tensor, w2: torch.Tensor, b2: torch.Tensor, out: torch.Tensor, *, B: int,
                  T: int, h_seg_stride: int, out_seg_stride: int) -> None:
    _check(load().sopro_seanet_res128_f32(ptr(h), h_seg_stride, ptr(w1), ptr(b1), ptr(w2), ptr(b2), ptr(out), out_seg_stride, B, T,
                                          _stream()), "sopro_seanet_res128_f32")


def seanet_up128(x: torch.Tensor, w: torch.Tensor, bias: torch.Tensor, out: torch.Tensor, *, B: int, T: int, x_seg_stride: int,
                 out_seg_stride: int, x_off: int = 0, out_off: int = 0, passes: int = 3) -> None:
    _check(load().sopro_seanet_up128_f32(ptr(x) + 4 * x_off, x_seg_stride, ptr(w), ptr(bias), ptr(out) + 4 * out_off, out_seg_stride, B, T,
                                         passes, _stream()), "sopro_seanet_up128_f32")


def seanet_res128_bf16(h: torch.Tensor, w1: torch.Tensor, b1: torch.Tensor, w2: torch.Tensor, b2: torch.Tensor, out: torch.Tensor, *, B: int,
                       T: int, h_seg_stride: int, out_seg_stride: int) -> None:
    _check(load().sopro_seanet_res128_bf16(ptr(h, torch.bfloat16), h_seg_stride, ptr(w1), ptr(b1), ptr(w2), ptr(b2), ptr(out, torch.bfloat16),
                                           out_seg_stride, B, T, _stream()), "sopro_seanet_res128_bf16")


def seanet_up128_bf16(x: torch.Tensor, w: torch.Tensor, bias: torch.Tensor, out: torch.Tensor, *, B: int, T: int, x_seg_stride: int,
                      out_seg_stride: int, x_off: int = 0, out_off: int = 0) -> None:
    _check(load().sopro_seanet_up128_bf16(ptr(x, torch.bfloat16) + 2 * x_off, x_seg_stride, ptr(w), ptr(bias), ptr(out, torch.bfloat16) + 2 * out_off,
                                          out_seg_stride, B, T, _stream()), "sopro_seanet_up128_bf16")


def seanet_tail_bf16(h: torch.Tensor, w1: torch.Tensor, b1: torch.Tensor, w2: torch.Tensor, b2: torch.Tensor, wf: torch.Tensor,
                     bf: float, wav: torch.Tensor, *, B: int, T: int, h_seg_stride: int, wav_seg_stride: int) -> None:
    _check(load().sopro_seanet_tail_bf16(ptr(h, torch.bfloat16), h_seg_stride, ptr(w1), ptr(b1), ptr(w2), ptr(b2), ptr(wf), bf, ptr(wav),
                                         wav_seg_stride, B, T, _stream()), "sopro_seanet_tail_bf16")


def seanet_uptail(x: torch.Tensor, wu: torch.Tensor, bu: torch.Tensor, w1: torch.Tensor, b1: torch.Tensor, w2: torch.Tensor, b2: torch.Tensor,
                  wf: torch.Tensor, bf: float, wav: torch.Tensor, *, B: int, T: int, x_seg_stride: int, wav_seg_stride: int, x_off: int = 0,
                  passes: int = 3) -> None:
    if x.dtype == torch.bfloat16:
        _check(load().sopro_seanet_uptail_bf16(ptr(x, torch.bfloat16) + 2 * x_off, x_seg_stride, ptr(wu), ptr(bu), ptr(w1), ptr(b1), ptr(w2), ptr(b2),
                                               ptr(wf), bf, ptr(wav), wav_seg_stride, B, T, _stream()), "sopro_seanet_uptail_bf16")
    else:
        _check(load().sopro_seanet_uptail_f32(ptr(x) + 4 * x_off, x_seg_stride, ptr(wu), ptr(bu), ptr(w1), ptr(b1), ptr(w2), ptr(b2), ptr(wf), bf,
                                              ptr(wav), wav_seg_stride, B, T, passes, _stream()), "sopro_seanet_uptail_f32")


def fill_u32(t: torch.Tensor, value: int = 0) -> None:
    n = t.numel() * t.element_size() // 4
    if not t.is_contiguous() or t.numel() * t.element_size() % 4 or n <= 0:
        raise SoproHipError("fill_u32: a contiguous tensor of whole 32-bit words")
    rows = 1
    while n // rows > (1 << 30):
        rows *= 2
    if n % rows:
        raise SoproHipError("fill_u32: tensor too large for one launch")
    _check(load().sopro_fill2d_u32(t.data_ptr(), n // rows, rows, n // rows, int(value) & 0xFFFFFFFF, _stream()), "sopro_fill2d_u32")


def copy_u32(dst: torch.Tensor, src: torch.Tensor) -> None:
    n = dst.numel() * dst.element_size() // 4
    if not (dst.is_contiguous() and src.is_contiguous()) or n * 4 != src.numel() * src.element_size() or n <= 0 or n > (1 << 30):
        raise SoproHipError("copy_u32: contiguous tensors of the same size (< 4 GiB)")
    _check(load().sopro_copy2d_u32(dst.data_ptr(), n, src.data_ptr(), n, 1, n, _stream()), "sopro_copy2d_u32")


def set_lds_floor(nbytes: int) -> None:
    _check(load().sopro_set_lds_floor(int(nbytes)), "sopro_set_lds_floor")


def ar_init(st: ArState) -> None:
    _check(load().sopro_ar_init(C.byref(st), _stream()), "sopro_ar_init")


def ar_admit(st: ArState, row: int) -> None:
    _check(load().sopro_ar_admit(C.byref(st), int(row), _stream()), "sopro_ar_admit")


def ar_sample(st: ArState, logits: torch.Tensor, ld: int) -> None:
    _check(load().sopro_ar_sample(C.byref(st), ptr(logits), ld, _stream()), "sopro_ar_sample")


def ar_issue_frame(frame: ArFrame) -> None:
    _check(load().sopro_ar_issue_frame(C.byref(frame), _stream()), "sopro_ar_issue_frame")


def ar_fold_text(txt: torch.Tensor, nkv_weight: torch.Tensor, kv_w: torch.Tensor, q_wT: torch.Tensor, o_w: torch.Tensor, nkv: torch.Tensor,
                 kvd: torch.Tensor, kp: torch.Tensor, vp: torch.Tensor, *, B: int, S: int, S_cap: int, D: int, H: int, eps: float,
                 out_off: int = 0) -> None:
    _check(load().sopro_ar_fold_text(ptr(txt), ptr(nkv_weight), ptr(kv_w), ptr(q_wT), ptr(o_w), ptr(nkv), ptr(kvd), ptr(kp) + 4 * out_off,
                                     ptr(vp) + 4 * out_off, B, S, S_cap, D, H, eps, _stream()), "sopro_ar_fold_text")


def ar_fold_text_uk(txt: torch.Tensor, nkv_weight: torch.Tensor, kv_w: torch.Tensor, o_w: torch.Tensor, nkv: torch.Tensor, kvd: torch.Tensor,
                    kq: torch.Tensor, vp: torch.Tensor, *, B: int, S: int, S_cap: int, D: int, H: int, eps: float, k_off: int = 0, v_off: int = 0) -> None:
    _check(load().sopro_ar_fold_text_uk(ptr(txt), ptr(nkv_weight), ptr(kv_w), ptr(o_w), ptr(nkv), ptr(kvd), ptr(kq) + 4 * k_off, ptr(vp) + 4 * v_off,
                                        B, S, S_cap, D, H, eps, _stream()), "sopro_ar_fold_text_uk")


def cvt_f32_bf16(src: torch.Tensor, dst: torch.Tensor, n: Optional[int] = None, dst_off: int = 0) -> None:
    n = int(src.numel() if n is None else n)
    _check(load().sopro_cvt_f32_bf16(ptr(src), ptr(dst, torch.bfloat16) + 2 * dst_off, n, _stream()), "sopro_cvt_f32_bf16")


def cvt_bf16_f32(src: torch.Tensor, dst: torch.Tensor, n: Optional[int] = None) -> None:
    n = int(src.numel() if n is None else n)
    _check(load().sopro_cvt_bf16_f32(ptr(src, torch.bfloat16), ptr(dst), n, _stream()), "sopro_cvt_bf16_f32")


_fade_tabs: dict = {}


def fade_table(fade_len: int, device) -> Optional[torch.Tensor]:
    import numpy as np

    fade_len = int(fade_len)
    if fade_len <= 0:
        return None
    key = (fade_len, str(device))
    t = _fade_tabs.get(key)
    if t is None:
        tab = (0.5 - 0.5 * np.cos(np.pi * (np.arange(fade_len, dtype=np.float64) + 0.5) / fade_len)).astype(np.float32)
        t = _fade_tabs[key] = torch.from_numpy(tab).to(device)
    return t


def _lens_list(lens) -> List[int]:
    return [int(v) for v in (lens.tolist() if isinstance(lens, torch.Tensor) else lens)]
# ... 860 lines not shown
```

Before: 27510 audio-s/s.

## Pass NAR intermediates between f16 GEMMs in pre-split fp16 hi/lo form

Adds a c_mode 9 epilogue to the f16 three-pass GEMM. It writes its output already split into scaled fp16 hi/lo halves, and an a_format 3 path lets the next GEMM read that split form directly. In the NAR refiner this is enabled by default only for the nar.pre -> heads chain (flow mask 2), so the consumer skips re-splitting fp32 rows and moves less A traffic. The FF1 -> FF2 chain in the SSM blocks is also wired but stays off by default. The cost is extra range-check reductions in the epilogue and more kernel template instantiations.

```diff
diff --git a/include/sopro_hip.h b/include/sopro_hip.h
--- a/include/sopro_hip.h
+++ b/include/sopro_hip.h
@@ -76,6 +76,7 @@
 int sopro_pack_w_f16x2(const float* W, int64_t ldw, int32_t N, int32_t K, float wscale, void* packed, void* stream);
 float sopro_f16x3_a_scale(void);
 int sopro_gemm_f16x3(const sopro_gemm_args* a, const void* packed_w, const sopro_gemm_split_ext* ext, void* stream);
+int sopro_split_rows_f16(const float* src, int64_t ld, void* dst, int32_t rows, int32_t cols, int32_t* range_events, void* stream);
 int64_t sopro_packed_w_bytes(int32_t N, int32_t K, int32_t pieces);
 int sopro_gemm_bf16_set_tile_override(int cfg);
 int sopro_gemm_set_group_m(int g);
@@ -348,6 +349,7 @@
   int32_t safe;
 } sopro_nar_io;
 int sopro_nar_refine_io(sopro_engine* e, void* workspace, const sopro_nar_io* io, int32_t B, int32_t T, void* stream);
+int sopro_nar_set_split_flow(int32_t mask);
 
 int64_t sopro_mimi_encode_workspace_bytes(const sopro_engine* e, int32_t B, int32_t N);
 int sopro_mimi_encode(sopro_engine* e, void* workspace, const float* wav, int32_t B, int32_t N, int32_t* codes, void* stream);
diff --git a/sopro_amd/csrc/common.h b/sopro_amd/csrc/common.h
--- a/sopro_amd/csrc/common.h
+++ b/sopro_amd/csrc/common.h
@@ -86,6 +86,19 @@
   lo = *reinterpret_cast<const unsigned*>(&l);
 }
 
+constexpr float SOPRO_A16_SCALE = 8.0f;
+typedef _Float16 f16x2_t __attribute__((ext_vector_type(2)));
+__device__ __forceinline__ void split2_f16_scaled(float x, float y, unsigned& hi, unsigned& lo, float& amax) {
+  const float F16MAX = 65504.0f;
+  const float vx = x * SOPRO_A16_SCALE, vy = y * SOPRO_A16_SCALE;
+  amax = fmaxf(amax, fmaxf(fabsf(vx), fabsf(vy)));
+  const float cx = __builtin_amdgcn_fmed3f(vx, -F16MAX, F16MAX), cy = __builtin_amdgcn_fmed3f(vy, -F16MAX, F16MAX);
+  const f16x2_t h = __builtin_convertvector((f32x2_t){cx, cy}, f16x2_t);
+  hi = *reinterpret_cast<const unsigned*>(&h);
+  const f16x2_t l = __builtin_convertvector((f32x2_t){cx - (float)h[0], cy - (float)h[1]}, f16x2_t);
+  lo = *reinterpret_cast<const unsigned*>(&l);
+}
+
 #ifndef SOPRO_NT_BULK
 #define SOPRO_NT_BULK 1
 #endif
diff --git a/sopro_amd/csrc/elementwise.hip b/sopro_amd/csrc/elementwise.hip
--- a/sopro_amd/csrc/elementwise.hip
+++ b/sopro_amd/csrc/elementwise.hip
@@ -470,6 +470,24 @@
   d[(i / width) * dpitch + (i % width)] = s[(i / width) * spitch + (i % width)];
 }
 
+__global__ __launch_bounds__(256) void split_rows_f16_kernel(const float* __restrict__ src, int64_t ld, char* __restrict__ dst, int rows, int cols4,
+                                                             int* __restrict__ range) {
+  const int64_t i = (int64_t)blockIdx.x * blockDim.x + threadIdx.x;
+  float amax = 0.f;
+  if (i < (int64_t)rows * cols4) {
+    const int64_t r = i / cols4;
+    const int c = (int)(i - r * cols4) * 4;
+    const float4 v = *reinterpret_cast<const float4*>(src + r * ld + c);
+    uint2 h, l;
+    split2_f16_scaled(v.x, v.y, h.x, l.x, amax);
+    split2_f16_scaled(v.z, v.w, h.y, l.y, amax);
+    char* d = dst + (r * ld) * 4 + (int64_t)(c >> 5) * 128 + (c & 31) * 2;
+    *reinterpret_cast<uint2*>(d) = h;
+    *reinterpret_cast<uint2*>(d + 64) = l;
+  }
+  if (range && __syncthreads_or(!(amax <= 65504.0f)) && threadIdx.x == 0) atomicAdd(range, 1);
+}
+
 __global__ __launch_bounds__(256) void nar_seed_kernel(int* __restrict__ tokens, int Q, const int* __restrict__ cb0, int64_t bstride, int B, int T, int vmax) {
   const int64_t i = (int64_t)blockIdx.x * blockDim.x + threadIdx.x;
   if (i >= (int64_t)B * T) return;
@@ -677,6 +695,16 @@
   SOPRO_LAUNCH_CHECK();
 }
 
+int sopro_split_rows_f16(const float* src, int64_t ld, void* dst, int32_t rows, int32_t cols, int32_t* range_events, void* stream) {
+  SOPRO_CHECK_ARG(src && dst && rows > 0 && cols > 0 && ld >= cols, "bad pointers or sizes");
+  SOPRO_CHECK_ARG((cols & 31) == 0 && (ld & 31) == 0, "cols and ld must be multiples of 32 (whole 128-byte groups)");
+  SOPRO_CHECK_ARG(aligned16(src) && (reinterpret_cast<uintptr_t>(dst) & 127u) == 0, "src 16-byte, dst 128-byte aligned");
+  SOPRO_CHECK_ARG(static_cast<const void*>(src) != dst, "not an in-place operation (a group's halves overwrite other threads' inputs)");
+  hipLaunchKernelGGL(split_rows_f16_kernel, dim3(nblk((int64_t)rows * (cols >> 2), 256)), dim3(256), 0, (hipStream_t)stream, src, ld,
+                     reinterpret_cast<char*>(dst), rows, cols >> 2, range_events);
+  SOPRO_LAUNCH_CHECK();
+}
+
 int sopro_fill2d_u32(void* p, int64_t pitch, int32_t rows, int32_t width, uint32_t value, void* stream) {
   SOPRO_CHECK_ARG(p && rows > 0 && width > 0 && pitch >= width, "bad pointers or sizes");
   hipLaunchKernelGGL(fill2d_kernel, dim3(nblk((int64_t)rows * width, 256)), dim3(256), 0, (hipStream_t)stream, reinterpret_cast<unsigned*>(p), pitch, rows,
diff --git a/sopro_amd/csrc/gemm_bf16s.hip b/sopro_amd/csrc/gemm_bf16s.hip
--- a/sopro_amd/csrc/gemm_bf16s.hip
+++ b/sopro_amd/csrc/gemm_bf16s.hip
@@ -8,12 +8,11 @@
 
 typedef __bf16 bf16x8 __attribute__((ext_vector_type(8)));
 typedef _Float16 f16x8 __attribute__((ext_vector_type(8)));
-typedef _Float16 f16x2_t __attribute__((ext_vector_type(2)));
 
 __device__ __forceinline__ bf16x8 as_frag(const uint4& v) { return *reinterpret_cast<const bf16x8*>(&v); }
 __device__ __forceinline__ f16x8 as_frag16(const uint4& v) { return *reinterpret_cast<const f16x8*>(&v); }
 
-constexpr float A16_SCALE = 8.0f;
+constexpr float A16_SCALE = SOPRO_A16_SCALE;
 
 template <int NPL, bool F16 = false>
 __device__ __forceinline__ void split_pair(float x, float y, unsigned (&pc)[NPL]) {
@@ -137,6 +136,7 @@
   auto lstore_piece = [&](int buf, float4 (&ra)[A_F4], const float4& pv, int i, bool fresh, bool first) {
     if constexpr (FOLD) {
       if constexpr (AMODE == 4) asm volatile("" : "+v"(rsc[i]), "+v"(ssq[i]));
+      else if constexpr (AMODE == 2) asm volatile("" : "+v"(ra[i].x), "+v"(ra[i].y), "+v"(ra[i].z), "+v"(ra[i].w));
       else asm volatile("" : "+v"(sapin[i]));
     }
     if constexpr (AMODE == 5) {
@@ -475,7 +475,7 @@
 }
 
 inline int amode_of(const sopro_gemm_args& g, const sopro_gemm_split_ext& ext) {
-  if (ext.a_format == 1) return 2;
+  if (ext.a_format == 1 || ext.a_format == 3) return 2;
   if (ext.a_format == 2) return 5;
   if (ext.rms_norm) return 4;
   if (ext.ln_stats) return 6;
@@ -536,7 +536,7 @@
   const int key = g.epilogue * 10 + amode_of(g, ext);
 #define SOPRO_CASE(E, A) \
   case (E) * 10 + (A): return launch_one<NPL, WM, WN, TM, TN, (((E) == SOPRO_EPI_GELU && (F16 || NPL != 3)) ? SOPRO_EPI_GELU_FAST : (E)), A, 0, F16>(g, wp, ksubs, ext, s)
-  switch (key) {
+  switch (ext.c_mode == 0 ? key : -1) {
     SOPRO_CASE(SOPRO_EPI_NONE, 0);
     SOPRO_CASE(SOPRO_EPI_GELU, 0);
     SOPRO_CASE(SOPRO_EPI_RES, 0);
@@ -546,6 +546,19 @@
     default: break;
   }
 #undef SOPRO_CASE
+  if constexpr (F16) {
+#define SOPRO_CASE9(E, A, O) \
+  case (O) * 1000 + (E) * 10 + (A): return launch_one<NPL, WM, WN, TM, TN, ((E) == SOPRO_EPI_GELU ? SOPRO_EPI_GELU_FAST : (E)), A, O, true>(g, wp, ksubs, ext, s)
+    switch (ext.c_mode * 1000 + key) {
+      SOPRO_CASE9(SOPRO_EPI_NONE, 2, 0);
+      SOPRO_CASE9(SOPRO_EPI_RES, 2, 0);
+      SOPRO_CASE9(SOPRO_EPI_NONE, 0, 9);
+      SOPRO_CASE9(SOPRO_EPI_GELU, 0, 9);
+      SOPRO_CASE9(SOPRO_EPI_GELU, 4, 9);
+      default: break;
+    }
+#undef SOPRO_CASE9
+  }
   if constexpr (WN * TN * 32 >= 64) {
     constexpr int GLU_ = (F16 || NPL != 3) ? SOPRO_EPI_GLU_FAST : SOPRO_EPI_GLU;
     if (key == SOPRO_EPI_GLU * 10) return launch_one<NPL, WM, WN, TM, TN, GLU_, 0, 0, F16>(g, wp, ksubs, ext, s);
@@ -557,11 +570,18 @@
 
 template <int NPL, bool F16 = false>
 int launch_argmax(sopro_gemm_args& g, const uint4* wp, int ksubs, const sopro_gemm_split_ext& ext, hipStream_t s) {
-  SOPRO_CHECK_ARG(g.epilogue == SOPRO_EPI_NONE && g.prologue == SOPRO_PRO_NONE && !ext.rms_norm && ext.a_format == 0,
+  SOPRO_CHECK_ARG(g.epilogue == SOPRO_EPI_NONE && g.prologue == SOPRO_PRO_NONE && !ext.rms_norm && (ext.a_format == 0 || (F16 && ext.a_format == 3)),
                   "arg-max output takes a plain contraction (no prologue / epilogue / fused norm)");
   SOPRO_CHECK_ARG(ext.C2 && ext.ldc2 >= (g.N + 63) / 64, "arg-max output: C2 = [M][ldc2 >= ceil(N / 64)] (value, index) pairs");
   static const bool tm1 = SOPRO_DEV_ENV("SOPRO_ARGMAX_TM") != nullptr && SOPRO_DEV_ENV("SOPRO_ARGMAX_TM")[0] == '1';
   static const bool tn1 = SOPRO_DEV_ENV("SOPRO_ARGMAX_TN") != nullptr && SOPRO_DEV_ENV("SOPRO_ARGMAX_TN")[0] == '1';
+  if constexpr (F16) {
+    if (ext.a_format == 3) {
+      if (g.M >= 8192 && g.N >= 2048 && (g.N & 127) == 0 && !tm1 && !tn1) return launch_one<NPL, 2, 2, 2, 2, SOPRO_EPI_NONE, 2, 5, F16>(g, wp, ksubs, ext, s);
+      if (g.M >= 8192 && !tm1) return launch_one<NPL, 2, 2, 2, 1, SOPRO_EPI_NONE, 2, 5, F16>(g, wp, ksubs, ext, s);
+      return launch_one<NPL, 2, 2, 1, 1, SOPRO_EPI_NONE, 2, 5, F16>(g, wp, ksubs, ext, s);
+    }
+  }
   if (g.M >= 8192 && g.N >= 2048 && (g.N & 127) == 0 && !tm1 && !tn1) return launch_one<NPL, 2, 2, 2, 2, SOPRO_EPI_NONE, 0, 5, F16>(g, wp, ksubs, ext, s);
   if (g.M >= 8192 && !tm1) return launch_one<NPL, 2, 2, 2, 1, SOPRO_EPI_NONE, 0, 5, F16>(g, wp, ksubs, ext, s);
   return launch_one<NPL, 2, 2, 1, 1, SOPRO_EPI_NONE, 0, 5, F16>(g, wp, ksubs, ext, s);
@@ -818,10 +838,25 @@
   sopro_gemm_split_ext ext = *x;
   if (ext.group_m == 0) ext.group_m = g_group_m;
   SOPRO_CHECK_ARG(ext.acc_scale > 0.f, "acc_scale = 1 / (sopro_f16x3_a_scale() * the weight's pack scale) must be set");
-  SOPRO_CHECK_ARG(ext.a_format == 0 && (ext.c_mode == 0 || ext.c_mode == 5),
-                  "the f16 three-pass path reads fp32 rows and writes fp32 rows, or arg-max partials (c_mode 5)");
+  SOPRO_CHECK_ARG((ext.a_format == 0 || ext.a_format == 3) && (ext.c_mode == 0 || ext.c_mode == 5 || ext.c_mode == 9),
+                  "the f16 three-pass path reads fp32 rows (a_format 0) or split-form fp16 rows (3) and writes fp32 rows (c_mode 0), arg-max partials (5) "
+                  "or split-form fp16 rows (9)");
   SOPRO_CHECK_ARG(!ext.rms_norm || ((g.K & 31) == 0 && ext.ksplit <= 1 && g.prologue == SOPRO_PRO_NONE && ext.rms_eps > 0.f),
                   "fused RMSNorm needs K % 32 == 0, no split-K, no prologue and eps > 0");
+  if (ext.a_format == 3) {
+    SOPRO_CHECK_ARG(!ext.rms_norm && !ext.ln_stats && g.prologue == SOPRO_PRO_NONE, "split-form fp16 A (a_format 3) takes the plain forms: no fused RMSNorm / LayerNorm, no prologue");
+    SOPRO_CHECK_ARG(g.epilogue == SOPRO_EPI_NONE || g.epilogue == SOPRO_EPI_RES, "split-form fp16 A (a_format 3): epilogue NONE or RES (or c_mode 5)");
+    SOPRO_CHECK_ARG(ext.c_mode != 9, "split-form fp16 A (a_format 3) writes fp32 rows or arg-max partials");
+    SOPRO_CHECK_ARG((g.K & 31) == 0 && (g.lda & 31) == 0 && (g.a_seg_stride & 31) == 0 && (reinterpret_cast<uintptr_t>(g.A) & 127u) == 0,
+                    "split-form A: K, lda, a_seg_stride multiples of 32 and a 128-byte aligned base");
+  }
+  if (ext.c_mode == 9) {
+    SOPRO_CHECK_ARG(g.epilogue == SOPRO_EPI_NONE || g.epilogue == SOPRO_EPI_GELU, "split-form fp16 output (c_mode 9): epilogue NONE or GELU");
+    SOPRO_CHECK_ARG(g.prologue == SOPRO_PRO_NONE && !ext.ln_stats, "split-form fp16 output (c_mode 9): no prologue, no fused LayerNorm");
+    SOPRO_CHECK_ARG((g.N & 31) == 0, "split-form fp16 output (c_mode 9): N % 32 == 0");
+    SOPRO_CHECK_ARG(g.C && (reinterpret_cast<uintptr_t>(g.C) & 127u) == 0 && (g.ldc & 31) == 0 && (g.c_seg_stride & 31) == 0 && g.ldc >= g.N,
+                    "split-form output rows must start on 128-byte boundaries (ld, seg stride multiples of 32)");
+  }
   if (int rc = check_common(g, ext, packed_w)) return rc;
   if (int rc = check_ln(g, ext)) return rc;
   SOPRO_CHECK_ARG(g.prologue == SOPRO_PRO_NONE || g.prologue == SOPRO_PRO_ADDVEC, "prologue must be NONE or ADDVEC");
diff --git a/sopro_amd/csrc/gemm_epilogue.h b/sopro_amd/csrc/gemm_epilogue.h
--- a/sopro_amd/csrc/gemm_epilogue.h
+++ b/sopro_amd/csrc/gemm_epilogue.h
@@ -14,7 +14,7 @@
   const int tid = threadIdx.x, lane = tid & 63, wave = tid >> 6;
   const int wm = wave / WN, wn = wave % WN;
   const int rps = g.rows_per_seg;
-  const bool big = (int64_t)g.M * g.N * (OUT >= 6 ? 2 : 4) >= SOPRO_BIG_BYTES;
+  const bool big = (int64_t)g.M * g.N * (OUT >= 6 && OUT <= 8 ? 2 : 4) >= SOPRO_BIG_BYTES;
   constexpr int CLD = BN + 4;
   constexpr bool RES_AHEAD = EPI == SOPRO_EPI_RES && OUT < 5;
   constexpr int RA_TPR = BN / 4, RA_RPP = NT / RA_TPR, RA_NPASS = BM / RA_RPP;
@@ -103,7 +103,7 @@
     }
     return;
   }
-  if constexpr (OUT >= 6) {
+  if constexpr (OUT >= 6 && OUT <= 8) {
     constexpr bool hres = EPI == SOPRO_EPI_RES;
     static_assert(EPI == SOPRO_EPI_NONE || EPI == SOPRO_EPI_RES, "bf16 rows take EPI_NONE or EPI_RES");
     constexpr int HTPR = BN / 4, HRPP = NT / HTPR, HNPASS = BM / HRPP;
@@ -224,7 +224,14 @@
   int seg = m / rps, rr = m - seg * rps;
   float* cptr = g.C + (int64_t)seg * g.c_seg_stride + (int64_t)rr * g.ldc + ocol;
   constexpr bool second = OUT == 2 || OUT == 4;
-  constexpr bool split_out = OUT == 1 || OUT == 2;
+  constexpr bool split_out = OUT == 1 || OUT == 2 || OUT == 9;
+  static_assert(OUT != 9 || EPI == SOPRO_EPI_NONE || EPI == SOPRO_EPI_GELU_FAST, "split-form fp16 rows take EPI_NONE or the f16 kernel's GELU");
+  float s16max = 0.f;
+  auto range_note = [&]() {
+    if constexpr (OUT == 9) {
+      if (ext->range_events && __syncthreads_or(!(s16max <= 65504.0f)) && tid == 0) atomicAdd(ext->range_events, 1);
+    }
+  };
   float* const dbase = second ? ext->C2 : g.C;
   const int64_t ldd = second ? ext->ldc2 : g.ldc, dseg = second ? ext->c2_seg_stride : g.c_seg_stride;
   const int64_t dcol_bytes = split_out ? (int64_t)(ocol >> 5) * 128 + (ocol & 31) * 2 : (int64_t)ocol * 4;
@@ -272,7 +279,14 @@
           else { v.x = v.x * c4.x + pv.x * s4.x; v.y = v.y * c4.y + pv.y * s4.y; v.z = v.z * c4.z + pv.z * s4.z; v.w = v.w * c4.w + pv.w * s4.w; }
         }
       }
-      if (split_out) {
+      if constexpr (OUT == 9) {
+        uint2 h, l;
+        split2_f16_scaled(v.x, v.y, h.x, l.x, s16max);
+        split2_f16_scaled(v.z, v.w, h.y, l.y, s16max);
+        bulk_store_u2(dpq, h, big);
+        bulk_store_u2(dpq + 64, l, big);
+        return;
+      } else if (split_out) {
         uint2 h, l;
         split2_bf16(eluf_(v.x), eluf_(v.y), h.x, l.x);
         split2_bf16(eluf_(v.z), eluf_(v.w), h.y, l.y);
@@ -303,6 +317,7 @@
 #endif
       }
     }
+    range_note();
     return;
   }
   auto batch = [&](int p0, const float4* rvb) {
@@ -346,4 +361,5 @@
 #endif
     }
   }
+  range_note();
 }
diff --git a/sopro_amd/csrc/stages.hip b/sopro_amd/csrc/stages.hip
--- a/sopro_amd/csrc/stages.hip
+++ b/sopro_amd/csrc/stages.hip
@@ -275,6 +275,12 @@
   sopro_prof_scope prof(split_passes ? "attention_split_kernel" : "attention_kernel", 4.0 * a.dh * pairs * a.B * a.H, s);
   if (split_passes) return sopro_attention_split_bf16(&a, split_passes, s);
   return sopro_attention_f32(&a, s);
+}
+
+int ksplit_of(const G& o, const Wt& w) {
+  static const bool no_splitk = getenv("SOPRO_NO_SPLITK") && getenv("SOPRO_NO_SPLITK")[0] == '1';
+  if (no_splitk || !o.sk || !o.sk->ws || o.rms_eps > 0.f || o.c_mode == 5) return 1;
+  return auto_ksplit(o.M, o.N, o.K, w.f16 ? 3 : w.pieces, o.epi);
 }
 
 int gemm(hipStream_t s, const float* A, const Wt& w, const float* w_f32_override, float* C, const G& o) {
@@ -314,12 +320,8 @@
     x.rope_rows_per_seg = o.rope_rps;
     x.ln_stats = o.ln_stats; x.ln_stats_out = o.ln_stats_out;
     if (o.ln_stats) x.rms_eps = o.ln_eps;
-    static const bool no_splitk = getenv("SOPRO_NO_SPLITK") && getenv("SOPRO_NO_SPLITK")[0] == '1';
-    if (!no_splitk && o.sk && o.sk->ws && o.rms_eps <= 0.f && o.c_mode != 5) {
-      const int ks = auto_ksplit(o.M, o.N, o.K, w.f16 ? 3 : w.pieces, o.epi);
-      if (ks > 1) {
-        x.ksplit = ks; x.n_tickets = SPLITK_TICKETS; x.ws = o.sk->ws; x.ws_bytes = (int64_t)SPLITK_WS_BYTES; x.tickets = o.sk->tickets;
-      }
+    if (const int ks = ksplit_of(o, w); ks > 1) {
+      x.ksplit = ks; x.n_tickets = SPLITK_TICKETS; x.ws = o.sk->ws; x.ws_bytes = (int64_t)SPLITK_WS_BYTES; x.tickets = o.sk->tickets;
     }
     if (w.f16) {
       x.acc_scale = w.acc_scale;
@@ -986,6 +988,22 @@
   return (int64_t)nar_carve(e, w, nullptr, B, T);
 }
 
+constexpr int NAR_SPLIT_FLOW_DEFAULT = 2;
+static int g_nar_split_flow = -1;
+static int nar_split_flow() {
+  if (g_nar_split_flow < 0) {
+    const char* v = SOPRO_DEV_ENV("SOPRO_NAR_SPLIT_FLOW");
+    g_nar_split_flow = v ? (atoi(v) & 3) : NAR_SPLIT_FLOW_DEFAULT;
+  }
+  return g_nar_split_flow;
+}
+int sopro_nar_set_split_flow(int32_t mask) {
+  SOPRO_CHECK_ARG(mask >= -1 && mask <= 3, "mask: bit 0 = FF1 -> FF2, bit 1 = nar.pre -> heads; -1 = the default");
+  g_nar_split_flow = mask < 0 ? NAR_SPLIT_FLOW_DEFAULT : mask;
+  return 0;
+}
+static bool rows128(const void* p, int64_t ld) { return (reinterpret_cast<uintptr_t>(p) & 127u) == 0 && (ld & 31) == 0; }
+
 static int ssm_block_bufs(sopro_engine* e, hipStream_t s, float* h, float* x1, float* u, const SplitK* sk, const float* x, float* out,
                           const std::string& p, int B, int T, int ksize, int dil, const int32_t* lens, const char* sfx, int32_t* range) {
   const int D = e->c.d_model, M = B * T;
@@ -994,9 +1012,15 @@
   STG(gemm(s, x, WT(e, p + ".glu.wn" + sfx), nullptr, h, g));
   STG(sopro_dwconv_f32(h, F(e, p + ".dw.w"), F(e, p + ".dw.b"), x, x1, lens, B, T, D, ksize, dil, left, 1, s));
   G f1; f1.M = M; f1.N = 4 * D; f1.K = D; f1.bias = F(e, p + ".ff1.b"); f1.epi = SOPRO_EPI_GELU; f1.rms_eps = RMS_EPS; f1.range_events = range;
-  STG(gemm(s, x1, WT(e, p + ".ff1.wn" + sfx), nullptr, u, f1));
   G f2; f2.M = M; f2.N = D; f2.K = 4 * D; f2.bias = F(e, p + ".ff2.b"); f2.epi = SOPRO_EPI_RES; f2.R = x1; f2.sk = sk; f2.range_events = range;
-  return gemm(s, u, WT(e, p + ".ff2.w" + sfx), nullptr, out, f2);
+  const Wt &w1 = WT(e, p + ".ff1.wn" + sfx), &w2 = WT(e, p + ".ff2.w" + sfx);
+  if ((nar_split_flow() & 1) && sfx[0] == 0 && e->c.precision == 0 && w1.f16 && w2.f16 && w1.packed && w2.packed && rows128(u, 4 * D) &&
+      ksplit_of(f2, w2) <= 1) {
+    f1.c_mode = 9;
+    f2.a_fmt = 3;
+  }
+  STG(gemm(s, x1, w1, nullptr, u, f1));
+  return gemm(s, u, w2, nullptr, out, f2);
 }
 static int ssm_block_seq(sopro_engine* e, hipStream_t s, const NarWs& w, const float* x, float* out, const std::string& p, int B, int T,
                          int ksize, int dil, const int32_t* lens, const char* sfx) {
@@ -1044,12 +1068,16 @@
     }
     STG(norm(s, xa, xb, F(e, "nar.norm.weight"), M, D, RMS_EPS));
     G pz; pz.M = M; pz.N = HD; pz.K = D; pz.bias = F(e, "nar.pre.b"); pz.range_events = w.range;
-    STG(gemm(s, xb, WT(e, std::string("nar.pre.w") + sfx), nullptr, w.z, pz));
+    const Wt &wz = WT(e, std::string("nar.pre.w") + sfx), &wh = WT(e, std::string("nar.heads.") + stage_names[sid] + ".w" + sfx);
+    const bool z_split = (nar_split_flow() & 2) && !safe && c.precision == 0 && wz.f16 && wh.f16 && wz.packed && wh.packed && rows128(w.z, HD);
+    if (z_split) pz.c_mode = 9;
+    STG(gemm(s, xb, wz, nullptr, w.z, pz));
     const int nh = c.stage_n_cb[sid];
     const std::string hk = std::string("nar.heads.") + stage_names[sid];
     G hg; hg.M = M; hg.N = nh * V; hg.K = HD; hg.bias = F(e, hk + ".b"); hg.c_mode = 5; hg.C2 = w.part; hg.ldc2 = (int64_t)nh_max * (V / 64);
     hg.range_events = w.range;
-    STG(gemm(s, w.z, WT(e, hk + ".w" + sfx), nullptr, nullptr, hg));
+    if (z_split) hg.a_fmt = 3;
+    STG(gemm(s, w.z, wh, nullptr, nullptr, hg));
     STG(sopro_argmax_partials_i32(w.part, (int64_t)nh_max * (V / 64), tokens + c.stage_first_cb[sid], Q, nh, V / 64, V, M, s));
   }
   if (io->range_out) STG(sopro_copy2d_u32(io->range_out, 1, w.range, 1, 1, 1, s));
diff --git a/sopro_amd/hip.py b/sopro_amd/hip.py
--- a/sopro_amd/hip.py
+++ b/sopro_amd/hip.py
@@ -146,6 +146,8 @@
     "sopro_copy2d_u32": (C.c_int, [_p, _i64, _p, _i64, _i32, _i32, _p]),
     "sopro_pack_w_f16x2": (C.c_int, [_p, _i64, _i32, _i32, _f32, _p, _p]),
     "sopro_f16x3_a_scale": (C.c_float, []),
+    "sopro_split_rows_f16": (C.c_int, [_p, _i64, _p, _i32, _i32, _p, _p]),
+    "sopro_nar_set_split_flow": (C.c_int, [_i32]),
     "sopro_gemm_f16x3": (C.c_int, [_p, _p, _p, _p]),
     "sopro_packed_w_bytes": (C.c_int64, [_i32, _i32, _i32]),
     "sopro_packed_w_rows_bytes": (C.c_int64, [_i32, _i32]),
@@ -447,10 +449,13 @@
     if (a16 or c16) and not (packed and W.pieces == 1 and not W.f16):
         raise SoproHipError("bf16 rows (a_format 2, c_mode 6 / 7 / 8) belong to the one-pass (pieces = 1) path")
     if packed and W.f16:
-        if a_split or c_mode not in (0, 5):
-            raise SoproHipError("split-form operands belong to the bf16 three-pass (pieces = 2) path")
+        if c_mode not in (0, 5, 9):
+            raise SoproHipError("the f16 three-pass path writes fp32 rows (c_mode 0), arg-max partials (5) or split-form fp16 rows (9)")
         if c_mode == 5:
             x.c_mode, x.C2, x.ldc2 = 5, ptr(C2) + 4 * c2_off, (-(-N // 64) if ldc2 is None else ldc2)
+        elif c_mode == 9:
+            x.c_mode = 9
+        x.a_format = 3 if a_split else 0
         x.acc_scale = W.acc_scale
         x.range_events = ptr(range_events, torch.int32)
         _check(load().sopro_gemm_f16x3(C.byref(g), ptr(W.data, torch.int32), C.byref(x), _stream()), "sopro_gemm_f16x3")
@@ -841,6 +846,23 @@
     else:
         _check(load().sopro_seanet_uptail_f32(ptr(x) + 4 * x_off, x_seg_stride, ptr(wu), ptr(bu), ptr(w1), ptr(b1), ptr(w2), ptr(b2), ptr(wf), bf,
                                               ptr(wav), wav_seg_stride, B, T, passes, _stream()), "sopro_seanet_uptail_f32")
+
+
+def split_rows_f16(src: torch.Tensor, dst: Optional[torch.Tensor] = None, *, rows: Optional[int] = None, cols: Optional[int] = None,
+                   ld: Optional[int] = None, range_events: Optional[torch.Tensor] = None) -> torch.Tensor:
+    if src.dim() != 2 and (rows is None or cols is None):
+        raise SoproHipError("split_rows_f16: give rows / cols for a tensor that is not 2-D")
+    rows = src.shape[0] if rows is None else rows
+    cols = src.shape[1] if cols is None else cols
+    ld = (src.stride(0) if src.dim() == 2 else cols) if ld is None else ld
+    if dst is None:
+        dst = torch.empty_like(src)
+    _check(load().sopro_split_rows_f16(ptr(src), ld, ptr(dst), rows, cols, ptr(range_events, torch.int32), _stream()), "sopro_split_rows_f16")
+    return dst
+
+
+def nar_set_split_flow(mask: int) -> None:
+    _check(load().sopro_nar_set_split_flow(int(mask)), "sopro_nar_set_split_flow")
 
 
 def fill_u32(t: torch.Tensor, value: int = 0) -> None:
```

After: 27410 audio-s/s. Within noise of the previous version (-0.4%).
